# pityka/lamp

Measured on AMD Instinct MI355X. Metric: training-step samples/sec, higher is better.
Workload: dtype bf16; 1 GPU; example-cifar100 Cnn.resnet(100) training step (fwd+backprop+AdamW), synthetic CIFAR batch; per_gpu_batch=2048, global_batch=2048, parallelism=single, optimizer=AdamW lr 1e-3 wd 0 beta2 0.95 mixedPrecision

## Files before the change

### include/lamp_hip.h

```cpp
#ifndef LAMP_HIP_H
#define LAMP_HIP_H

#include <stddef.h>
#include <stdint.h>

#ifdef __cplusplus
extern "C" {
#endif

#define LAMP_MAX_DIMS 8

typedef struct lamp_tensor lamp_tensor;
typedef struct lamp_stream lamp_stream;
typedef struct lamp_comm lamp_comm;
typedef struct lamp_graph lamp_graph;

#define LAMP_U8 0
#define LAMP_I8 1
#define LAMP_I16 2
#define LAMP_I32 3
#define LAMP_I64 4
#define LAMP_F16 5
#define LAMP_F32 6
#define LAMP_F64 7
// ... 263 lines not shown
                      const lamp_tensor* inRowptr, const lamp_tensor* inPerm, const lamp_tensor* outRowptr, const lamp_tensor* outPerm);
int lamp_gat_long_row(int64_t* out);

int lamp_convolution(lamp_tensor** out, const lamp_tensor* x, const lamp_tensor* w, const lamp_tensor* bias_or_null,
                     const int64_t* stride, const int64_t* padding, const int64_t* dilation, int nspatial,
                     int transposed, const int64_t* output_padding, int64_t groups);
int lamp_convolution_backward(lamp_tensor* out3[3], const lamp_tensor* grad_out, const lamp_tensor* x,
                              const lamp_tensor* w, const int64_t* stride, const int64_t* padding,
                              const int64_t* dilation, int nspatial, int transposed,
                              const int64_t* output_padding, int64_t groups, const uint8_t mask[3]);
int lamp_convolution_backward_input_add(lamp_tensor** out, const lamp_tensor* grad_out, const lamp_tensor* x,
                                        const lamp_tensor* w, const int64_t* stride, const int64_t* padding,
                                        const int64_t* dilation, int nspatial, const int64_t* output_padding,
                                        int64_t groups, const lamp_tensor* addend);
int lamp_convolution_backward_input_pair(lamp_tensor** out, const lamp_tensor* x, const lamp_tensor* grad_out_a, const lamp_tensor* w_a,
                                         const int64_t* stride_a, const int64_t* padding_a, const int64_t* dilation_a,
                                         const lamp_tensor* grad_out_b, const lamp_tensor* w_b, const int64_t* stride_b,
                                         const int64_t* padding_b, const int64_t* dilation_b, int nspatial, int64_t groups,
                                         const lamp_tensor* addend_or_null);
int lamp_convolution_backward_weight_pair(lamp_tensor* out2[2], const lamp_tensor* x, const lamp_tensor* grad_out_a, const lamp_tensor* w_a,
                                          const int64_t* stride_a, const int64_t* padding_a, const int64_t* dilation_a,
                                          const lamp_tensor* grad_out_b, const lamp_tensor* w_b, const int64_t* stride_b,
                                          const int64_t* padding_b, const int64_t* dilation_b, int nspatial, int64_t groups);
int lamp_convolution_pair(lamp_tensor* out2[2], const lamp_tensor* x, const lamp_tensor* w_a, const lamp_tensor* bias_a_or_null,
                          const int64_t* stride_a, const int64_t* padding_a, const int64_t* dilation_a, const lamp_tensor* w_b,
                          const lamp_tensor* bias_b_or_null, const int64_t* stride_b, const int64_t* padding_b,
                          const int64_t* dilation_b, int nspatial, int64_t groups);
int lamp_convolution_chain_pair(lamp_tensor* out3[3], const lamp_tensor* x, const lamp_tensor* w, const lamp_tensor* bias_or_null,
                                const int64_t* stride, const int64_t* padding, const int64_t* dilation, const lamp_tensor* w_a,
                                const lamp_tensor* bias_a_or_null, const int64_t* stride_a, const int64_t* padding_a,
                                const int64_t* dilation_a, const lamp_tensor* w_b, const lamp_tensor* bias_b_or_null,
                                const int64_t* stride_b, const int64_t* padding_b, const int64_t* dilation_b, int nspatial,
                                int64_t groups);
int lamp_avg_pool2d(lamp_tensor** out, const lamp_tensor* x, int64_t kernel, int64_t stride, int64_t padding,
                    int ceil_mode, int count_include_pad);
int lamp_avg_pool2d_backward(lamp_tensor** out, const lamp_tensor* grad_out, const lamp_tensor* x, int64_t kernel,
                             int64_t stride, int64_t padding, int ceil_mode, int count_include_pad);
int lamp_max_pool2d_with_indices(lamp_tensor** out, lamp_tensor** indices, const lamp_tensor* x, int64_t kernel,
                                 int64_t stride, int64_t padding, int64_t dilation, int ceil_mode);
int lamp_max_pool2d_with_indices_backward(lamp_tensor** out, const lamp_tensor* grad_out, const lamp_tensor* x,
                                          int64_t kernel, int64_t stride, int64_t padding, int64_t dilation,
                                          int ceil_mode, const lamp_tensor* indices);
int lamp_max_pool1d_with_indices(lamp_tensor** out, lamp_tensor** indices, const lamp_tensor* x, int64_t kernel,
                                 int64_t stride, int64_t padding, int64_t dilation, int ceil_mode);
int lamp_max_pool1d_with_indices_backward(lamp_tensor** out, const lamp_tensor* grad_out, const lamp_tensor* x,
                                          int64_t kernel, int64_t stride, int64_t padding, int64_t dilation,
                                          int ceil_mode, const lamp_tensor* indices);

int lamp_native_batch_norm(lamp_tensor* out3[3] , const lamp_tensor* x,
                           const lamp_tensor* weight_or_null, const lamp_tensor* bias_or_null,
                           lamp_tensor* running_mean_or_null, lamp_tensor* running_var_or_null, int training,
                           double momentum, double eps);
int lamp_native_batch_norm_backward(lamp_tensor* out3[3] , const lamp_tensor* grad_out,
                                    const lamp_tensor* x, const lamp_tensor* weight_or_null,
                                    const lamp_tensor* running_mean_or_null, const lamp_tensor* running_var_or_null,
                                    const lamp_tensor* save_mean_or_null, const lamp_tensor* save_invstd_or_null,
                                    int training, double eps, const uint8_t mask[3]);
int lamp_native_batch_norm_relu(lamp_tensor* out3[3] , const lamp_tensor* x,
                                const lamp_tensor* weight_or_null, const lamp_tensor* bias_or_null,
                                lamp_tensor* running_mean_or_null, lamp_tensor* running_var_or_null, int training,
                                double momentum, double eps);
int lamp_native_batch_norm_relu_backward(lamp_tensor* out3[3] , const lamp_tensor* grad_out,
                                         const lamp_tensor* x, const lamp_tensor* weight_or_null, const lamp_tensor* bias_or_null,
                                         const lamp_tensor* running_mean_or_null, const lamp_tensor* running_var_or_null,
                                         const lamp_tensor* save_mean_or_null, const lamp_tensor* save_invstd_or_null,
                                         int training, double eps, const uint8_t mask[3]);
// ... 185 lines not shown
```

### jni/LampNative.java

```java
package aten;

public final class LampNative {
  static { System.loadLibrary("lampjni"); }
  private LampNative() {}
  public static native String lamp_last_error();
  public static native String lamp_version();
  public static native void lamp_tensor_release_all(long[] tensors);
  public static native byte[] lamp_comm_get_unique_id();
  public static native long lamp_comm_init_rank(int nranks, byte[] id, int rank);
  public static native long[] lamp_tensors_from_file(String path, long offset, long length, boolean pin, long[] types, long[] offsets, long[] lengths);
  public static native long[] lamp_tensor_trace_list();
  public static native long[] lamp_tensor_sizes(long t);
  public static native long[] lamp_tensor_strides(long t);
  public static native boolean copyFromDoubleArray(long t, double[] a);
  public static native boolean copyToDoubleArray(long t, double[] a);
  public static native boolean copyFromFloatArray(long t, float[] a);
  public static native boolean copyToFloatArray(long t, float[] a);
  public static native boolean copyFromLongArray(long t, long[] a);
  public static native boolean copyToLongArray(long t, long[] a);
  public static native boolean copyFromIntArray(long t, int[] a);
  public static native boolean copyToIntArray(long t, int[] a);
  public static native boolean copyFromShortArray(long t, short[] a);
  public static native boolean copyToShortArray(long t, short[] a);
  public static native boolean copyFromByteArray(long t, byte[] a);
// ... 196 lines not shown
  public static native long lamp_bmm(long a, long b);
  public static native void lamp_bmm_out(long out, long a, long b);
  public static native long lamp_matmul(long a, long b);
  public static native long lamp_addmm(long self, long a, long b, double beta, double alpha);
  public static native void lamp_addmm_out(long out, long self, long a, long b, double beta, double alpha);
  public static native long lamp_baddbmm(long self, long a, long b, double beta, double alpha);
  public static native void lamp_addmm_out_transposed1(long out, long self, long a, long b, double beta, double alpha);
  public static native void lamp_addmm_out_transposed2(long out, long self, long a, long b, double beta, double alpha);
  public static native void lamp_baddbmm_out_transposed1(long out, long self, long a, long b, double beta, double alpha);
  public static native void lamp_baddbmm_out_transposed2(long out, long self, long a, long b, double beta, double alpha);
  public static native long lamp_linear_bias(long x, long w, long bias_or_null);
  public static native void lamp_lstm_cell_forward(long gates, long c_prev, long h_out, long c_out);
  public static native void lamp_lstm_cell_backward(long dgates, long dc_prev, long gates, long c_prev, long c, long dout_or_null, long dh_or_null, long dc_or_null);
  public static native void lamp_gru_gates_forward(long gates, long h_prev, long rh_out);
  public static native void lamp_gru_output_forward(long gates, long h_prev, long h_out);
  public static native void lamp_gru_output_backward(long dgates, long dh_prev, long gates, long h_prev, long dout_or_null, long dh_or_null);
  public static native void lamp_gru_gates_backward(long dgates, long dh_prev, long gates, long h_prev, long drh);
  public static native void lamp_rnn_cell_forward(long gates, long h_out);
  public static native void lamp_rnn_cell_backward(long dgates, long h, long dout_or_null, long dh_or_null);
  public static native long[] lamp_gcn_adjacency(long edgeI, long edgeJ, long numNodes, int dtype);
  public static native long lamp_gcn_aggregate(long x, long rowptr, long col, long dinv);
  public static native long lamp_gcn_long_row();
  public static native long[] lamp_graph_edge_csr(long index, long numNodes);
  public static native long[] lamp_gat_forward(long score, long value, long edgeI, long inRowptr, long inPerm);
  public static native long[] lamp_gat_backward(long dout, long out, long lse, long score, long value, long edgeI, long edgeJ, long inRowptr, long inPerm, long outRowptr, long outPerm);
  public static native long lamp_gat_long_row();
  public static native long lamp_convolution(long x, long w, long bias_or_null, long[] stride, long[] padding, long[] dilation, int transposed, long[] output_padding, long groups);
  public static native long[] lamp_convolution_backward(long grad_out, long x, long w, long[] stride, long[] padding, long[] dilation, int transposed, long[] output_padding, long groups, boolean[] mask);
  public static native long lamp_convolution_backward_input_add(long grad_out, long x, long w, long[] stride, long[] padding, long[] dilation, long[] output_padding, long groups, long addend);
  public static native long lamp_convolution_backward_input_pair(long x, long grad_out_a, long w_a, long[] stride_a, long[] padding_a, long[] dilation_a, long grad_out_b, long w_b, long[] stride_b, long[] padding_b, long[] dilation_b, long groups, long addend_or_null);
  public static native long[] lamp_convolution_backward_weight_pair(long x, long grad_out_a, long w_a, long[] stride_a, long[] padding_a, long[] dilation_a, long grad_out_b, long w_b, long[] stride_b, long[] padding_b, long[] dilation_b, long groups);
  public static native long[] lamp_convolution_pair(long x, long w_a, long bias_a_or_null, long[] stride_a, long[] padding_a, long[] dilation_a, long w_b, long bias_b_or_null, long[] stride_b, long[] padding_b, long[] dilation_b, long groups);
  public static native long[] lamp_convolution_chain_pair(long x, long w, long bias_or_null, long[] stride, long[] padding, long[] dilation, long w_a, long bias_a_or_null, long[] stride_a, long[] padding_a, long[] dilation_a, long w_b, long bias_b_or_null, long[] stride_b, long[] padding_b, long[] dilation_b, long groups);
  public static native long lamp_avg_pool2d(long x, long kernel, long stride, long padding, int ceil_mode, int count_include_pad);
  public static native long lamp_avg_pool2d_backward(long grad_out, long x, long kernel, long stride, long padding, int ceil_mode, int count_include_pad);
  public static native long[] lamp_max_pool2d_with_indices(long x, long kernel, long stride, long padding, long dilation, int ceil_mode);
  public static native long lamp_max_pool2d_with_indices_backward(long grad_out, long x, long kernel, long stride, long padding, long dilation, int ceil_mode, long indices);
  public static native long[] lamp_max_pool1d_with_indices(long x, long kernel, long stride, long padding, long dilation, int ceil_mode);
  public static native long lamp_max_pool1d_with_indices_backward(long grad_out, long x, long kernel, long stride, long padding, long dilation, int ceil_mode, long indices);
  public static native long[] lamp_native_batch_norm(long x, long weight_or_null, long bias_or_null, long running_mean_or_null, long running_var_or_null, int training, double momentum, double eps);
  public static native long[] lamp_native_batch_norm_backward(long grad_out, long x, long weight_or_null, long running_mean_or_null, long running_var_or_null, long save_mean_or_null, long save_invstd_or_null, int training, double eps, boolean[] mask);
  public static native long[] lamp_native_batch_norm_relu(long x, long weight_or_null, long bias_or_null, long running_mean_or_null, long running_var_or_null, int training, double momentum, double eps);
  public static native long[] lamp_native_batch_norm_relu_backward(long grad_out, long x, long weight_or_null, long bias_or_null, long running_mean_or_null, long running_var_or_null, long save_mean_or_null, long save_invstd_or_null, int training, double eps, boolean[] mask);
  public static native long[] lamp_native_batch_norm_add_relu(long x, long addend, long weight_or_null, long bias_or_null, long running_mean_or_null, long running_var_or_null, int training, double momentum, double eps);
  public static native long[] lamp_native_batch_norm_add_relu_backward(long grad_out, long x, long addend, long weight_or_null, long bias_or_null, long running_mean_or_null, long running_var_or_null, long save_mean_or_null, long save_invstd_or_null, int training, double eps, boolean[] mask);
  public static native long[] lamp_native_batch_norm2_add_relu(long x, long weight, long bias, long running_mean, long running_var, long x2, long weight2, long bias2, long running_mean2, long running_var2, double momentum, double momentum2, double eps, double eps2);
  public static native long[] lamp_native_batch_norm2_add_relu_pool_log_softmax(long x, long weight, long bias, long running_mean, long running_var, long x2, long weight2, long bias2, long running_mean2, long running_var2, double momentum, double momentum2, double eps, double eps2);
  public static native long[] lamp_native_batch_norm2_add_relu_backward(long grad_out, long x, long weight, long bias, long save_mean, long save_invstd, long x2, long weight2, long bias2, long save_mean2, long save_invstd2, double eps, double eps2, boolean[] mask);
  public static native long[] lamp_batch_norm_affine(long x, long weight, long bias, long running_mean, long running_var, double momentum, double eps);
  public static native int lamp_convolution_bn_relu_input_folds(long x, long w, long[] stride, long[] padding, long[] dilation, long groups);
  public static native long lamp_convolution_bn_relu_input(long x, long affine, long w, long bias_or_null, long[] stride, long[] padding, long[] dilation, long groups);
  public static native long[] lamp_convolution_bn_relu_input_backward(long grad_out, long x, long affine, long w, long[] stride, long[] padding, long[] dilation, long groups, boolean[] mask);
  public static native long[] lamp_native_layer_norm(long x, long[] normalized_shape, long weight_or_null, long bias_or_null, double eps);
  public static native long[] lamp_native_layer_norm_backward(long grad_out, long x, long[] normalized_shape, long mean, long rstd, long weight_or_null, long bias_or_null, boolean[] mask);
  public static native long lamp_log_softmax(long x, long dim);
  public static native long lamp_log_softmax_backward_data(long grad_out, long output, long dim);
  public static native long lamp_global_avg_pool_log_softmax(long x);
  public static native long lamp_global_avg_pool_log_softmax_backward(long grad, long output, long x);
  public static native long lamp_global_avg_pool_log_softmax_nll_backward(long grad_loss, long target, long weight_or_null, long reduction, long ignore_index, long total_weight, long output, long x);
  public static native long lamp_softmax(long x, long dim);
  public static native long[] lamp_nll_loss_forward(long x, long target, long weight_or_null, long reduction, long ignore_index);
  public static native long[] lamp_nll_loss_forward_accumulate_(long x, long target, long weight_or_null, long reduction, long ignore_index, long acc, double scale);
  public static native long[] lamp_nll_loss_forward_pooled_gradient_(long x, long target, long weight_or_null, long reduction, long ignore_index, long acc_or_null, double scale, long plane_elems);
  public static native long lamp_nll_loss_backward(long grad_out, long x, long target, long weight_or_null, long reduction, long ignore_index, long total_weight);
  public static native long lamp_mse_loss(long x, long target, long reduction);
  public static native long lamp_mse_loss_backward(long grad_out, long x, long target, long reduction);
// ... 77 lines not shown
```

### jni/aten_jni.c

```c
#ifdef LAMP_JNI_SYNTAX_CHECK
#include "jni_syntax_check.h"
#else
#include <jni.h>
#endif
#include <stdint.h>
#include <stddef.h>
#include "lamp_hip.h"

#define H(x) ((void*)(intptr_t)(x))

#define LAMP_JNI_MAX_OUTS 4096

static void lamp_throw(JNIEnv* env) {
  jclass ex = (*env)->FindClass(env, "java/lang/RuntimeException");
  if (ex) (*env)->ThrowNew(env, ex, lamp_last_error());
}
static void lamp_throw_msg(JNIEnv* env, const char* msg) {
  jclass ex = (*env)->FindClass(env, "java/lang/RuntimeException");
  if (ex) (*env)->ThrowNew(env, ex, msg);
}

#define COPY_NATIVES(JT, JNAME, GET, REL)                                                                                              \
  JNIEXPORT jboolean JNICALL Java_aten_LampNative_copyFrom##JNAME##Array(JNIEnv* env, jclass cls, jlong t, JT##Array a) {              \
    (void)cls;                                                                                                                         \
// ... 1980 lines not shown
  (void)stride_a_n;
  jsize padding_a_n = (*env)->GetArrayLength(env, padding_a);
  jlong* padding_a_e = (*env)->GetLongArrayElements(env, padding_a, NULL);
  (void)padding_a_n;
  jsize dilation_a_n = (*env)->GetArrayLength(env, dilation_a);
  jlong* dilation_a_e = (*env)->GetLongArrayElements(env, dilation_a, NULL);
  (void)dilation_a_n;
  jsize stride_b_n = (*env)->GetArrayLength(env, stride_b);
  jlong* stride_b_e = (*env)->GetLongArrayElements(env, stride_b, NULL);
  (void)stride_b_n;
  jsize padding_b_n = (*env)->GetArrayLength(env, padding_b);
  jlong* padding_b_e = (*env)->GetLongArrayElements(env, padding_b, NULL);
  (void)padding_b_n;
  jsize dilation_b_n = (*env)->GetArrayLength(env, dilation_b);
  jlong* dilation_b_e = (*env)->GetLongArrayElements(env, dilation_b, NULL);
  void* out3_o[3] = {0};
  const int rc_ = lamp_convolution_chain_pair((void*)out3_o, H(x), H(w), H(bias_or_null), (const int64_t*)stride_e, (const int64_t*)padding_e, (const int64_t*)dilation_e, H(w_a), H(bias_a_or_null), (const int64_t*)stride_a_e, (const int64_t*)padding_a_e, (const int64_t*)dilation_a_e, H(w_b), H(bias_b_or_null), (const int64_t*)stride_b_e, (const int64_t*)padding_b_e, (const int64_t*)dilation_b_e, (int)dilation_b_n, (int64_t)groups);
  (*env)->ReleaseLongArrayElements(env, stride, stride_e, JNI_ABORT);
  (*env)->ReleaseLongArrayElements(env, padding, padding_e, JNI_ABORT);
  (*env)->ReleaseLongArrayElements(env, dilation, dilation_e, JNI_ABORT);
  (*env)->ReleaseLongArrayElements(env, stride_a, stride_a_e, JNI_ABORT);
  (*env)->ReleaseLongArrayElements(env, padding_a, padding_a_e, JNI_ABORT);
  (*env)->ReleaseLongArrayElements(env, dilation_a, dilation_a_e, JNI_ABORT);
  (*env)->ReleaseLongArrayElements(env, stride_b, stride_b_e, JNI_ABORT);
  (*env)->ReleaseLongArrayElements(env, padding_b, padding_b_e, JNI_ABORT);
  (*env)->ReleaseLongArrayElements(env, dilation_b, dilation_b_e, JNI_ABORT);
  if (rc_ != 0) { lamp_throw(env); return NULL; }
  jlong r_[3] = {(jlong)(intptr_t)out3_o[0], (jlong)(intptr_t)out3_o[1], (jlong)(intptr_t)out3_o[2]};
  jlongArray a_ = (*env)->NewLongArray(env, 3);
  if (a_) (*env)->SetLongArrayRegion(env, a_, 0, 3, r_);
  return a_;
}

JNIEXPORT jlong JNICALL Java_aten_LampNative_lamp_1avg_1pool2d(JNIEnv* env, jclass cls, jlong x, jlong kernel, jlong stride, jlong padding, jint ceil_mode, jint count_include_pad) {
  (void)cls;
  void* out_o = NULL;
  const int rc_ = lamp_avg_pool2d((void*)&out_o, H(x), (int64_t)kernel, (int64_t)stride, (int64_t)padding, (int)ceil_mode, (int)count_include_pad);
  if (rc_ != 0) { lamp_throw(env); return 0; }
  return (jlong)(intptr_t)out_o;
}

JNIEXPORT jlong JNICALL Java_aten_LampNative_lamp_1avg_1pool2d_1backward(JNIEnv* env, jclass cls, jlong grad_out, jlong x, jlong kernel, jlong stride, jlong padding, jint ceil_mode, jint count_include_pad) {
  (void)cls;
  void* out_o = NULL;
  const int rc_ = lamp_avg_pool2d_backward((void*)&out_o, H(grad_out), H(x), (int64_t)kernel, (int64_t)stride, (int64_t)padding, (int)ceil_mode, (int)count_include_pad);
  if (rc_ != 0) { lamp_throw(env); return 0; }
  return (jlong)(intptr_t)out_o;
}

JNIEXPORT jlongArray JNICALL Java_aten_LampNative_lamp_1max_1pool2d_1with_1indices(JNIEnv* env, jclass cls, jlong x, jlong kernel, jlong stride, jlong padding, jlong dilation, jint ceil_mode) {
  (void)cls;
  void* out_o = NULL;
  void* indices_o = NULL;
  const int rc_ = lamp_max_pool2d_with_indices((void*)&out_o, (void*)&indices_o, H(x), (int64_t)kernel, (int64_t)stride, (int64_t)padding, (int64_t)dilation, (int)ceil_mode);
  if (rc_ != 0) { lamp_throw(env); return NULL; }
  jlong r_[2] = {(jlong)(intptr_t)out_o, (jlong)(intptr_t)indices_o};
  jlongArray a_ = (*env)->NewLongArray(env, 2);
  if (a_) (*env)->SetLongArrayRegion(env, a_, 0, 2, r_);
  return a_;
}

JNIEXPORT jlong JNICALL Java_aten_LampNative_lamp_1max_1pool2d_1with_1indices_1backward(JNIEnv* env, jclass cls, jlong grad_out, jlong x, jlong kernel, jlong stride, jlong padding, jlong dilation, jint ceil_mode, jlong indices) {
  (void)cls;
  void* out_o = NULL;
  const int rc_ = lamp_max_pool2d_with_indices_backward((void*)&out_o, H(grad_out), H(x), (int64_t)kernel, (int64_t)stride, (int64_t)padding, (int64_t)dilation, (int)ceil_mode, H(indices));
  if (rc_ != 0) { lamp_throw(env); return 0; }
// ... 1078 lines not shown
```

### lamp_amd/csrc/core/host_staging.cpp

```cpp
#include "host_staging.h"

namespace S = lamp::staging;

extern "C" {

int lamp_abs__dev(lamp_tensor** out, const lamp_tensor* a);
int lamp_abs(lamp_tensor** out, const lamp_tensor* a) { return S::call(lamp_abs__dev, S::Out{out}, S::In{a}); }
int lamp_abs___dev(lamp_tensor* a);
int lamp_abs_(lamp_tensor* a) { return S::call(lamp_abs___dev, S::InOut{a}); }
int lamp_acos__dev(lamp_tensor** out, const lamp_tensor* a);
int lamp_acos(lamp_tensor** out, const lamp_tensor* a) { return S::call(lamp_acos__dev, S::Out{out}, S::In{a}); }
int lamp_acos___dev(lamp_tensor* a);
int lamp_acos_(lamp_tensor* a) { return S::call(lamp_acos___dev, S::InOut{a}); }
int lamp_adamw_step___dev(lamp_tensor* const* params, lamp_tensor* const* grads, lamp_tensor* const* m, lamp_tensor* const* v, lamp_tensor* const* master_or_null, int n, const double* lr, const double* weight_decay, const double* beta1, const double* beta2, double eps, double schedule_factor, int64_t step_count, int debias);
int lamp_adamw_step_(lamp_tensor* const* params, lamp_tensor* const* grads, lamp_tensor* const* m, lamp_tensor* const* v, lamp_tensor* const* master_or_null, int n, const double* lr, const double* weight_decay, const double* beta1, const double* beta2, double eps, double schedule_factor, int64_t step_count, int debias) { return S::call(lamp_adamw_step___dev, S::Arr{params, n, false}, S::Arr{grads, n, true}, S::Arr{m, n, false}, S::Arr{v, n, false}, S::Arr{master_or_null, n, false}, n, lr, weight_decay, beta1, beta2, eps, schedule_factor, step_count, debias); }
int lamp_add__dev(lamp_tensor** out, const lamp_tensor* a, const lamp_tensor* b, double alpha);
int lamp_add(lamp_tensor** out, const lamp_tensor* a, const lamp_tensor* b, double alpha) { return S::call(lamp_add__dev, S::Out{out}, S::In{a}, S::In{b}, alpha); }
int lamp_add___dev(lamp_tensor* self, const lamp_tensor* b, double alpha);
int lamp_add_(lamp_tensor* self, const lamp_tensor* b, double alpha) { return S::call(lamp_add___dev, S::InOut{self}, S::In{b}, alpha); }
int lamp_add_out__dev(lamp_tensor* out, const lamp_tensor* a, const lamp_tensor* b, double alpha);
int lamp_add_out(lamp_tensor* out, const lamp_tensor* a, const lamp_tensor* b, double alpha) { return S::call(lamp_add_out__dev, S::InOut{out}, S::In{a}, S::In{b}, alpha); }
int lamp_add_scalar__dev(lamp_tensor** out, const lamp_tensor* a, double b, double alpha);
int lamp_add_scalar(lamp_tensor** out, const lamp_tensor* a, double b, double alpha) { return S::call(lamp_add_scalar__dev, S::Out{out}, S::In{a}, b, alpha); }
int lamp_add_scalar___dev(lamp_tensor* self, double b, double alpha);
// ... 26 lines not shown
int lamp_atan2(lamp_tensor** out, const lamp_tensor* a, const lamp_tensor* b) { return S::call(lamp_atan2__dev, S::Out{out}, S::In{a}, S::In{b}); }
int lamp_atan___dev(lamp_tensor* a);
int lamp_atan_(lamp_tensor* a) { return S::call(lamp_atan___dev, S::InOut{a}); }
int lamp_avg_pool2d__dev(lamp_tensor** out, const lamp_tensor* x, int64_t kernel, int64_t stride, int64_t padding, int ceil_mode, int count_include_pad);
int lamp_avg_pool2d(lamp_tensor** out, const lamp_tensor* x, int64_t kernel, int64_t stride, int64_t padding, int ceil_mode, int count_include_pad) { return S::call(lamp_avg_pool2d__dev, S::Out{out}, S::In{x}, kernel, stride, padding, ceil_mode, count_include_pad); }
int lamp_avg_pool2d_backward__dev(lamp_tensor** out, const lamp_tensor* grad_out, const lamp_tensor* x, int64_t kernel, int64_t stride, int64_t padding, int ceil_mode, int count_include_pad);
int lamp_avg_pool2d_backward(lamp_tensor** out, const lamp_tensor* grad_out, const lamp_tensor* x, int64_t kernel, int64_t stride, int64_t padding, int ceil_mode, int count_include_pad) { return S::call(lamp_avg_pool2d_backward__dev, S::Out{out}, S::In{grad_out}, S::In{x}, kernel, stride, padding, ceil_mode, count_include_pad); }
int lamp_baddbmm__dev(lamp_tensor** out, const lamp_tensor* self, const lamp_tensor* a, const lamp_tensor* b, double beta, double alpha);
int lamp_baddbmm(lamp_tensor** out, const lamp_tensor* self, const lamp_tensor* a, const lamp_tensor* b, double beta, double alpha) { return S::call(lamp_baddbmm__dev, S::Out{out}, S::In{self}, S::In{a}, S::In{b}, beta, alpha); }
int lamp_baddbmm_out_transposed1__dev(lamp_tensor* out, const lamp_tensor* self, const lamp_tensor* a, const lamp_tensor* b, double beta, double alpha);
int lamp_baddbmm_out_transposed1(lamp_tensor* out, const lamp_tensor* self, const lamp_tensor* a, const lamp_tensor* b, double beta, double alpha) { return S::call(lamp_baddbmm_out_transposed1__dev, S::InOut{out}, S::In{self}, S::In{a}, S::In{b}, beta, alpha); }
int lamp_baddbmm_out_transposed2__dev(lamp_tensor* out, const lamp_tensor* self, const lamp_tensor* a, const lamp_tensor* b, double beta, double alpha);
int lamp_baddbmm_out_transposed2(lamp_tensor* out, const lamp_tensor* self, const lamp_tensor* a, const lamp_tensor* b, double beta, double alpha) { return S::call(lamp_baddbmm_out_transposed2__dev, S::InOut{out}, S::In{self}, S::In{a}, S::In{b}, beta, alpha); }
int lamp_batch_norm_affine__dev(lamp_tensor* out3[3], const lamp_tensor* x, const lamp_tensor* weight, const lamp_tensor* bias, lamp_tensor* running_mean, lamp_tensor* running_var, double momentum, double eps);
int lamp_batch_norm_affine(lamp_tensor* out3[3], const lamp_tensor* x, const lamp_tensor* weight, const lamp_tensor* bias, lamp_tensor* running_mean, lamp_tensor* running_var, double momentum, double eps) { return S::call(lamp_batch_norm_affine__dev, S::OutK<3>{out3}, S::In{x}, S::In{weight}, S::In{bias}, S::InOut{running_mean}, S::InOut{running_var}, momentum, eps); }
int lamp_binary_cross_entropy_with_logits__dev(lamp_tensor** out, const lamp_tensor* x, const lamp_tensor* target, const lamp_tensor* pos_weight_or_null, int64_t reduction);
int lamp_binary_cross_entropy_with_logits(lamp_tensor** out, const lamp_tensor* x, const lamp_tensor* target, const lamp_tensor* pos_weight_or_null, int64_t reduction) { return S::call(lamp_binary_cross_entropy_with_logits__dev, S::Out{out}, S::In{x}, S::In{target}, S::In{pos_weight_or_null}, reduction); }
int lamp_bincount__dev(lamp_tensor** out, const lamp_tensor* a, const lamp_tensor* weights_or_null, int64_t minlength);
int lamp_bincount(lamp_tensor** out, const lamp_tensor* a, const lamp_tensor* weights_or_null, int64_t minlength) { return S::call(lamp_bincount__dev, S::Out{out}, S::In{a}, S::In{weights_or_null}, minlength); }
int lamp_bmm__dev(lamp_tensor** out, const lamp_tensor* a, const lamp_tensor* b);
int lamp_bmm(lamp_tensor** out, const lamp_tensor* a, const lamp_tensor* b) { return S::call(lamp_bmm__dev, S::Out{out}, S::In{a}, S::In{b}); }
int lamp_bmm_out__dev(lamp_tensor* out, const lamp_tensor* a, const lamp_tensor* b);
int lamp_bmm_out(lamp_tensor* out, const lamp_tensor* a, const lamp_tensor* b) { return S::call(lamp_bmm_out__dev, S::InOut{out}, S::In{a}, S::In{b}); }
int lamp_cartesian_prod__dev(lamp_tensor** out, lamp_tensor* const* tensors, int n);
int lamp_cartesian_prod(lamp_tensor** out, lamp_tensor* const* tensors, int n) { return S::call(lamp_cartesian_prod__dev, S::Out{out}, S::Arr{tensors, n, false}, n); }
int lamp_ceil__dev(lamp_tensor** out, const lamp_tensor* a);
int lamp_ceil(lamp_tensor** out, const lamp_tensor* a) { return S::call(lamp_ceil__dev, S::Out{out}, S::In{a}); }
int lamp_ceil___dev(lamp_tensor* a);
int lamp_ceil_(lamp_tensor* a) { return S::call(lamp_ceil___dev, S::InOut{a}); }
int lamp_convolution__dev(lamp_tensor** out, const lamp_tensor* x, const lamp_tensor* w, const lamp_tensor* bias_or_null, const int64_t* stride, const int64_t* padding, const int64_t* dilation, int nspatial, int transposed, const int64_t* output_padding, int64_t groups);
int lamp_convolution(lamp_tensor** out, const lamp_tensor* x, const lamp_tensor* w, const lamp_tensor* bias_or_null, const int64_t* stride, const int64_t* padding, const int64_t* dilation, int nspatial, int transposed, const int64_t* output_padding, int64_t groups) { return S::call(lamp_convolution__dev, S::Out{out}, S::In{x}, S::In{w}, S::In{bias_or_null}, stride, padding, dilation, nspatial, transposed, output_padding, groups); }
int lamp_convolution_backward__dev(lamp_tensor* out3[3], const lamp_tensor* grad_out, const lamp_tensor* x, const lamp_tensor* w, const int64_t* stride, const int64_t* padding, const int64_t* dilation, int nspatial, int transposed, const int64_t* output_padding, int64_t groups, const uint8_t mask[3]);
int lamp_convolution_backward(lamp_tensor* out3[3], const lamp_tensor* grad_out, const lamp_tensor* x, const lamp_tensor* w, const int64_t* stride, const int64_t* padding, const int64_t* dilation, int nspatial, int transposed, const int64_t* output_padding, int64_t groups, const uint8_t mask[3]) { return S::call(lamp_convolution_backward__dev, S::OutK<3>{out3}, S::In{grad_out}, S::In{x}, S::In{w}, stride, padding, dilation, nspatial, transposed, output_padding, groups, mask); }
int lamp_convolution_backward_input_add__dev(lamp_tensor** out, const lamp_tensor* grad_out, const lamp_tensor* x, const lamp_tensor* w, const int64_t* stride, const int64_t* padding, const int64_t* dilation, int nspatial, const int64_t* output_padding, int64_t groups, const lamp_tensor* addend);
int lamp_convolution_backward_input_add(lamp_tensor** out, const lamp_tensor* grad_out, const lamp_tensor* x, const lamp_tensor* w, const int64_t* stride, const int64_t* padding, const int64_t* dilation, int nspatial, const int64_t* output_padding, int64_t groups, const lamp_tensor* addend) { return S::call(lamp_convolution_backward_input_add__dev, S::Out{out}, S::In{grad_out}, S::In{x}, S::In{w}, stride, padding, dilation, nspatial, output_padding, groups, S::In{addend}); }
int lamp_convolution_backward_input_pair__dev(lamp_tensor** out, const lamp_tensor* x, const lamp_tensor* grad_out_a, const lamp_tensor* w_a, const int64_t* stride_a, const int64_t* padding_a, const int64_t* dilation_a, const lamp_tensor* grad_out_b, const lamp_tensor* w_b, const int64_t* stride_b, const int64_t* padding_b, const int64_t* dilation_b, int nspatial, int64_t groups, const lamp_tensor* addend_or_null);
int lamp_convolution_backward_input_pair(lamp_tensor** out, const lamp_tensor* x, const lamp_tensor* grad_out_a, const lamp_tensor* w_a, const int64_t* stride_a, const int64_t* padding_a, const int64_t* dilation_a, const lamp_tensor* grad_out_b, const lamp_tensor* w_b, const int64_t* stride_b, const int64_t* padding_b, const int64_t* dilation_b, int nspatial, int64_t groups, const lamp_tensor* addend_or_null) { return S::call(lamp_convolution_backward_input_pair__dev, S::Out{out}, S::In{x}, S::In{grad_out_a}, S::In{w_a}, stride_a, padding_a, dilation_a, S::In{grad_out_b}, S::In{w_b}, stride_b, padding_b, dilation_b, nspatial, groups, S::In{addend_or_null}); }
int lamp_convolution_backward_weight_pair__dev(lamp_tensor* out2[2], const lamp_tensor* x, const lamp_tensor* grad_out_a, const lamp_tensor* w_a, const int64_t* stride_a, const int64_t* padding_a, const int64_t* dilation_a, const lamp_tensor* grad_out_b, const lamp_tensor* w_b, const int64_t* stride_b, const int64_t* padding_b, const int64_t* dilation_b, int nspatial, int64_t groups);
int lamp_convolution_backward_weight_pair(lamp_tensor* out2[2], const lamp_tensor* x, const lamp_tensor* grad_out_a, const lamp_tensor* w_a, const int64_t* stride_a, const int64_t* padding_a, const int64_t* dilation_a, const lamp_tensor* grad_out_b, const lamp_tensor* w_b, const int64_t* stride_b, const int64_t* padding_b, const int64_t* dilation_b, int nspatial, int64_t groups) { return S::call(lamp_convolution_backward_weight_pair__dev, S::OutK<2>{out2}, S::In{x}, S::In{grad_out_a}, S::In{w_a}, stride_a, padding_a, dilation_a, S::In{grad_out_b}, S::In{w_b}, stride_b, padding_b, dilation_b, nspatial, groups); }
int lamp_convolution_bn_relu_input__dev(lamp_tensor** out, const lamp_tensor* x, const lamp_tensor* affine, const lamp_tensor* w, const lamp_tensor* bias_or_null, const int64_t* stride, const int64_t* padding, const int64_t* dilation, int nspatial, int64_t groups);
int lamp_convolution_bn_relu_input(lamp_tensor** out, const lamp_tensor* x, const lamp_tensor* affine, const lamp_tensor* w, const lamp_tensor* bias_or_null, const int64_t* stride, const int64_t* padding, const int64_t* dilation, int nspatial, int64_t groups) { return S::call(lamp_convolution_bn_relu_input__dev, S::Out{out}, S::In{x}, S::In{affine}, S::In{w}, S::In{bias_or_null}, stride, padding, dilation, nspatial, groups); }
int lamp_convolution_bn_relu_input_backward__dev(lamp_tensor* out3[3], const lamp_tensor* grad_out, const lamp_tensor* x, const lamp_tensor* affine, const lamp_tensor* w, const int64_t* stride, const int64_t* padding, const int64_t* dilation, int nspatial, int64_t groups, const uint8_t mask[3]);
int lamp_convolution_bn_relu_input_backward(lamp_tensor* out3[3], const lamp_tensor* grad_out, const lamp_tensor* x, const lamp_tensor* affine, const lamp_tensor* w, const int64_t* stride, const int64_t* padding, const int64_t* dilation, int nspatial, int64_t groups, const uint8_t mask[3]) { return S::call(lamp_convolution_bn_relu_input_backward__dev, S::OutK<3>{out3}, S::In{grad_out}, S::In{x}, S::In{affine}, S::In{w}, stride, padding, dilation, nspatial, groups, mask); }
int lamp_convolution_bn_relu_input_folds__dev(int* out, const lamp_tensor* x, const lamp_tensor* w, const int64_t* stride, const int64_t* padding, const int64_t* dilation, int nspatial, int64_t groups);
int lamp_convolution_bn_relu_input_folds(int* out, const lamp_tensor* x, const lamp_tensor* w, const int64_t* stride, const int64_t* padding, const int64_t* dilation, int nspatial, int64_t groups) { return S::call(lamp_convolution_bn_relu_input_folds__dev, out, S::In{x}, S::In{w}, stride, padding, dilation, nspatial, groups); }
int lamp_convolution_chain_pair__dev(lamp_tensor* out3[3], const lamp_tensor* x, const lamp_tensor* w, const lamp_tensor* bias_or_null, const int64_t* stride, const int64_t* padding, const int64_t* dilation, const lamp_tensor* w_a, const lamp_tensor* bias_a_or_null, const int64_t* stride_a, const int64_t* padding_a, const int64_t* dilation_a, const lamp_tensor* w_b, const lamp_tensor* bias_b_or_null, const int64_t* stride_b, const int64_t* padding_b, const int64_t* dilation_b, int nspatial, int64_t groups);
int lamp_convolution_chain_pair(lamp_tensor* out3[3], const lamp_tensor* x, const lamp_tensor* w, const lamp_tensor* bias_or_null, const int64_t* stride, const int64_t* padding, const int64_t* dilation, const lamp_tensor* w_a, const lamp_tensor* bias_a_or_null, const int64_t* stride_a, const int64_t* padding_a, const int64_t* dilation_a, const lamp_tensor* w_b, const lamp_tensor* bias_b_or_null, const int64_t* stride_b, const int64_t* padding_b, const int64_t* dilation_b, int nspatial, int64_t groups) { return S::call(lamp_convolution_chain_pair__dev, S::OutK<3>{out3}, S::In{x}, S::In{w}, S::In{bias_or_null}, stride, padding, dilation, S::In{w_a}, S::In{bias_a_or_null}, stride_a, padding_a, dilation_a, S::In{w_b}, S::In{bias_b_or_null}, stride_b, padding_b, dilation_b, nspatial, groups); }
int lamp_convolution_pair__dev(lamp_tensor* out2[2], const lamp_tensor* x, const lamp_tensor* w_a, const lamp_tensor* bias_a_or_null, const int64_t* stride_a, const int64_t* padding_a, const int64_t* dilation_a, const lamp_tensor* w_b, const lamp_tensor* bias_b_or_null, const int64_t* stride_b, const int64_t* padding_b, const int64_t* dilation_b, int nspatial, int64_t groups);
int lamp_convolution_pair(lamp_tensor* out2[2], const lamp_tensor* x, const lamp_tensor* w_a, const lamp_tensor* bias_a_or_null, const int64_t* stride_a, const int64_t* padding_a, const int64_t* dilation_a, const lamp_tensor* w_b, const lamp_tensor* bias_b_or_null, const int64_t* stride_b, const int64_t* padding_b, const int64_t* dilation_b, int nspatial, int64_t groups) { return S::call(lamp_convolution_pair__dev, S::OutK<2>{out2}, S::In{x}, S::In{w_a}, S::In{bias_a_or_null}, stride_a, padding_a, dilation_a, S::In{w_b}, S::In{bias_b_or_null}, stride_b, padding_b, dilation_b, nspatial, groups); }
int lamp_cos__dev(lamp_tensor** out, const lamp_tensor* a);
int lamp_cos(lamp_tensor** out, const lamp_tensor* a) { return S::call(lamp_cos__dev, S::Out{out}, S::In{a}); }
int lamp_cos___dev(lamp_tensor* a);
int lamp_cos_(lamp_tensor* a) { return S::call(lamp_cos___dev, S::InOut{a}); }
int lamp_count_ne__dev(lamp_tensor** out, const lamp_tensor* a, const lamp_tensor* b);
int lamp_count_ne(lamp_tensor** out, const lamp_tensor* a, const lamp_tensor* b) { return S::call(lamp_count_ne__dev, S::Out{out}, S::In{a}, S::In{b}); }
int lamp_cross__dev(lamp_tensor** out, const lamp_tensor* a, const lamp_tensor* b, int64_t dim);
int lamp_cross(lamp_tensor** out, const lamp_tensor* a, const lamp_tensor* b, int64_t dim) { return S::call(lamp_cross__dev, S::Out{out}, S::In{a}, S::In{b}, dim); }
int lamp_diag__dev(lamp_tensor** out, const lamp_tensor* a, int64_t diagonal);
int lamp_diag(lamp_tensor** out, const lamp_tensor* a, int64_t diagonal) { return S::call(lamp_diag__dev, S::Out{out}, S::In{a}, diagonal); }
int lamp_diagonal__dev(lamp_tensor** out, const lamp_tensor* a, int64_t offset, int64_t dim1, int64_t dim2);
int lamp_diagonal(lamp_tensor** out, const lamp_tensor* a, int64_t offset, int64_t dim1, int64_t dim2) { return S::call(lamp_diagonal__dev, S::Out{out}, S::In{a}, offset, dim1, dim2); }
int lamp_div__dev(lamp_tensor** out, const lamp_tensor* a, const lamp_tensor* b);
int lamp_div(lamp_tensor** out, const lamp_tensor* a, const lamp_tensor* b) { return S::call(lamp_div__dev, S::Out{out}, S::In{a}, S::In{b}); }
int lamp_div___dev(lamp_tensor* self, const lamp_tensor* b);
int lamp_div_(lamp_tensor* self, const lamp_tensor* b) { return S::call(lamp_div___dev, S::InOut{self}, S::In{b}); }
int lamp_div_out__dev(lamp_tensor* out, const lamp_tensor* a, const lamp_tensor* b);
// ... 379 lines not shown
```

### lamp_amd/csrc/core/switches.h

```cpp
#pragma once
#include <cstdint>

namespace lamp {

constexpr int64_t SW_NO_CLAMP = INT64_MIN;

#define LAMP_SWITCHES_ONCE(X)                                                                                                             \
                                                        \
  X(conv_sibling, "LAMP_CONV_SIBLING", BOOL, 1, 0, "a residual block's 3x3 and its sibling 1x1 of the same input as one forward launch") \
  X(conv_chain, "LAMP_CONV_CHAIN", BOOL, 1, 0, "a convolution directly in front of a residual block and the block's 3x3 + 1x1 as one forward call (0: two)") \
  X(fuse_bn_pair, "LAMP_FUSE_BN_PAIR", BOOL, 1, 0, "relu(bn(right) + bn(left)) at a block's end as one op (0: the chain)")                \
  X(fuse_pool_logsoftmax, "LAMP_FUSE_POOL_LOGSOFTMAX", BOOL, 1, 0, "average pool -> flatten -> log-softmax tail as one node")             \
  X(fuse_block_tail, "LAMP_FUSE_BLOCK_TAIL", BOOL, 1, 0, "the last residual block and the pooled log-softmax tail as one node")          \
  X(fuse_bn_conv, "LAMP_FUSE_BN_CONV", BOOL, 1, 0, "batch norm -> relu -> convolution: the convolution applies the norm while staging")  \
  X(fuse_loss_accumulate, "LAMP_FUSE_LOSS_ACCUMULATE", BOOL, 1, 0, "acc += n * loss inside the NLL loss kernel")                          \
  X(fuse_loss_backward, "LAMP_FUSE_LOSS_BACKWARD", BOOL, 1, 0, "the NLL loss backward goes straight to the pooled log-softmax node's input in one launch")                      \
  X(fuse_loss_tail, "LAMP_FUSE_LOSS_TAIL", BOOL, 1, 0, "the loss launch also writes the pooled log-softmax's input gradient per plane")  \
  X(conv_dgrad_accumulate, "LAMP_CONV_DGRAD_ACCUMULATE", BOOL, 1, 0, "a convolution's input gradient adds into the existing one in its epilogue") \
  X(conv_dgrad_pair, "LAMP_CONV_DGRAD_PAIR", BOOL, 1, 0, "input gradients of a block's 3x3 and sibling 1x1 from one launch")             \
  X(conv_wgrad_pair, "LAMP_CONV_WGRAD_PAIR", BOOL, 1, 0, "weight gradients of a block's 3x3 and sibling 1x1 from one launch")            \
  X(linear_bias_fused, "LAMP_LINEAR_BIAS_FUSED", BOOL, 1, 0, "a linear layer's bias in the GEMM epilogue (0: mm then add)")               \
  X(mult_add_fused, "LAMP_MULT_ADD_FUSED", BOOL, 1, 0, "x * scale + residual in one pass (0: mult then add)")                             \
  X(attention_as_written_for_cuda, "LAMP_ATTENTION_AS_WRITTEN_FOR_CUDA", BOOL, 0, 0, "multi-head attention as the reference's op chain instead of the fused kernels") \
  X(recurrent_fused, "LAMP_RECURRENT_FUSED", BOOL, 1, 0, "RNN / GRU / LSTM as one node per sequence with fused cell kernels (0: the fold over time steps)") \
  X(fuse_qkv, "LAMP_FUSE_QKV", BOOL, 1, 0, "self-attention's three projections as one product (0: three)")                                \
  X(host_stream_side, "LAMP_HOST_STREAM_SIDE", BOOL, 0, 0, "batch streams gather on a side stream instead of the consumer's")             \
                                                                           \
  X(pinned_cache_mb, "LAMP_PINNED_CACHE_MB", INT, 2048, 0, "upper bound of the cache of freed pinned host buffers, MiB")                  \
  X(pinned_gather_wgs, "LAMP_PINNED_GATHER_WGS", INT, 48, 1, "workgroups of a gather that reads pinned host memory")                      \
                                                                                                    \
  X(flash_attention, "LAMP_FLASH_ATTENTION", BOOL, 1, 0, "the flash attention kernels, forward and backward")                             \
  X(small_attention, "LAMP_SMALL_ATTENTION", BOOL, 1, 0, "the short-sequence attention kernels")                                          \
  X(knn_fused, "LAMP_KNN_FUSED", BOOL, 1, 0, "the fused distance + top-k nearest-neighbour kernel")                                       \
  X(knn_split, "LAMP_KNN_SPLIT", INT, -1, SW_NO_CLAMP, "f16-plane k-NN filter: 0 off, 1 where it pays, 2 forced; negative: the mode set through the API") \
  X(knn_split_planes, "LAMP_KNN_SPLIT_PLANES", INT, 0, SW_NO_CLAMP, "f16 planes per coordinate of that filter: 3, anything else 2")      \
  X(umap_pairs2, "LAMP_UMAP_PAIRS2", BOOL, 1, 0, "the UMAP loss's two-dimensional pair kernel")                                            \
                                                                                                             \
  X(gemm_shape_tags, "LAMP_GEMM_SHAPE_TAGS", BOOL, 0, 0, "profiling aid: one kernel-timer class per GEMM shape and layout")               \
  X(gemm_splitk, "LAMP_GEMM_SPLITK", BOOL, 1, 0, "split-K for products with few output tiles (bf16 and f32 / f64)")                       \
  X(gemm_tail_split, "LAMP_GEMM_TAIL_SPLIT", BOOL, 1, 0, "an almost empty last round of 256 x 256 tiles becomes a second, split-K product") \
  X(gemm_fp_split_wgs, "LAMP_GEMM_FP_SPLIT_WGS", INT, 512, 1, "workgroups an f32 / f64 split-K product aims at")                          \
                                                                                              \
  X(bn_fused_bwd, "LAMP_BN_FUSED_BWD", BOOL, 1, 0, "one-pass batch-norm backward (workgroups exchange their sums) where no mode is set through the API") \
// ... 45 lines not shown
```

### lamp_amd/csrc/host/autograd.h

```cpp
#pragma once
#include <cmath>
#include <functional>
#include <memory>
#include <string>
#include <vector>

#include "../core/tensor.h"

namespace lamp {
namespace host {

struct Box {
  lamp_tensor* h;
  explicit Box(lamp_tensor* h_) : h(h_) {}
  ~Box() { if (h) lamp_tensor_release(h); }
  Box(const Box&) = delete;
  Box& operator=(const Box&) = delete;
};
struct Ten {
  std::shared_ptr<Box> b;
  Ten() = default;
  explicit Ten(lamp_tensor* h) : b(h ? std::make_shared<Box>(h) : nullptr) {}
  lamp_tensor* h() const { return b ? b->h : nullptr; }
  bool defined() const { return b && b->h; }
// ... 64 lines not shown
inline Ten view(const Ten& a, const std::vector<int64_t>& s) { lamp_tensor* o = nullptr; HCALL(lamp_view(&o, a.h(), s.data(), (int)s.size())); return Ten(o); }
inline Ten reshape(const Ten& a, const std::vector<int64_t>& s) { lamp_tensor* o = nullptr; HCALL(lamp_reshape(&o, a.h(), s.data(), (int)s.size())); return Ten(o); }
inline Ten flatten(const Ten& a, int64_t s, int64_t e) { lamp_tensor* o = nullptr; HCALL(lamp_flatten(&o, a.h(), s, e)); return Ten(o); }
inline Ten transpose(const Ten& a, int64_t d0, int64_t d1) { lamp_tensor* o = nullptr; HCALL(lamp_transpose(&o, a.h(), d0, d1)); return Ten(o); }
inline Ten slice(const Ten& a, int64_t d, int64_t s, int64_t e, int64_t st) { lamp_tensor* o = nullptr; HCALL(lamp_slice(&o, a.h(), d, s, e, st)); return Ten(o); }
inline Ten select(const Ten& a, int64_t d, int64_t i) { lamp_tensor* o = nullptr; HCALL(lamp_select(&o, a.h(), d, i)); return Ten(o); }
inline Ten unbroadcast(const Ten& p, const std::vector<int64_t>& s) { lamp_tensor* o = nullptr; HCALL(lamp_unbroadcast(&o, p.h(), s.data(), (int)s.size())); return Ten(o); }
inline Ten sum_dims(const Ten& a, const std::vector<int64_t>& d, bool keep) { lamp_tensor* o = nullptr; HCALL(lamp_sum_dims(&o, a.h(), d.data(), (int)d.size(), keep)); return Ten(o); }
inline Ten mean_dims(const Ten& a, const std::vector<int64_t>& d, bool keep) { lamp_tensor* o = nullptr; HCALL(lamp_mean_dims(&o, a.h(), d.data(), (int)d.size(), keep)); return Ten(o); }
inline Ten norm2_dims(const Ten& a, const std::vector<int64_t>& d, bool keep) { lamp_tensor* o = nullptr; HCALL(lamp_norm2_dims(&o, a.h(), d.data(), (int)d.size(), keep)); return Ten(o); }
inline Ten zeros(const std::vector<int64_t>& s, int dtype, int device) { lamp_tensor* o = nullptr; HCALL(lamp_zeros(&o, s.data(), (int)s.size(), dtype, device)); return Ten(o); }
inline Ten ones(const std::vector<int64_t>& s, int dtype, int device) { lamp_tensor* o = nullptr; HCALL(lamp_ones(&o, s.data(), (int)s.size(), dtype, device)); return Ten(o); }
inline Ten scalar(double v, int dtype, int device) { lamp_tensor* o = nullptr; HCALL(lamp_scalar_tensor(&o, v, dtype, device)); return Ten(o); }
inline Ten normal(double mean, double std, const std::vector<int64_t>& s, int dtype, int device) { lamp_tensor* o = nullptr; HCALL(lamp_normal(&o, mean, std, s.data(), (int)s.size(), dtype, device)); return Ten(o); }
inline Ten cast(const Ten& a, int dtype) { lamp_tensor* o = nullptr; HCALL(lamp_cast(&o, a.h(), dtype)); return Ten(o); }
inline Ten index_select(const Ten& a, int64_t d, const Ten& idx) { lamp_tensor* o = nullptr; HCALL(lamp_index_select(&o, a.h(), d, idx.h())); return Ten(o); }
inline Ten index_add(const Ten& a, int64_t d, const Ten& idx, const Ten& src) { lamp_tensor* o = nullptr; HCALL(lamp_index_add(&o, a.h(), d, idx.h(), src.h())); return Ten(o); }
inline Ten where(const Ten& c, const Ten& a, const Ten& b) { lamp_tensor* o = nullptr; HCALL(lamp_where(&o, c.h(), a.h(), b.h())); return Ten(o); }
inline Ten lt_scalar(const Ten& a, double s) { lamp_tensor* o = nullptr; HCALL(lamp_lt_scalar(&o, a.h(), s)); return Ten(o); }
inline Ten le_scalar(const Ten& a, double s) { lamp_tensor* o = nullptr; HCALL(lamp_le_scalar(&o, a.h(), s)); return Ten(o); }
inline Ten cat(const std::vector<Ten>& ts, int64_t dim) {
  std::vector<lamp_tensor*> hs;
  for (auto& t : ts) hs.push_back(t.h());
  lamp_tensor* o = nullptr;
  HCALL(lamp_cat(&o, hs.data(), (int)hs.size(), dim));
  return Ten(o);
}
}

struct Variable;
using Var = std::shared_ptr<Variable>;
using Backward = std::function<void(const Ten& p, Variable& out)>;

struct Op {
  virtual ~Op() = default;
  std::vector<std::pair<Var, Backward>> params;
  const char* name = "op";
  std::function<void()> reset;
  std::function<void(const Ten& plane_grad)> pooled_input_grad;
};

struct Variable {
  std::shared_ptr<Op> op;
  Ten value;
  bool wants_grad = false;
  Ten grad;
  bool grad_shared = false;
  std::vector<std::function<void()>> pending;
  bool needsGrad() const { return wants_grad; }
  std::vector<int64_t> shape() const { return value.shape(); }
  void zeroGrad() { grad = Ten(); grad_shared = false; }
  Ten grad_tensor() {
    if (!wants_grad) return Ten();
    if (!grad.defined()) { grad = ops::zeros_like(value); grad_shared = false; }
    return grad;
  }
  Ten grad_inplace() {
    if (!grad.defined()) { grad = ops::zeros_like(value); grad_shared = false; }
    else if (grad_shared) { grad = ops::clone(grad); grad_shared = false; }
    return grad;
  }
  void accumulate(const Ten& t, bool fresh) {
    if (!grad.defined()) { grad = t; grad_shared = !fresh; return; }
    if (grad_shared) { grad = ops::add(grad, t); grad_shared = false; return; }
    ops::add_(grad, t);
  }
  void accumulate_scaled(const Ten& t, double alpha) {
    if (!grad.defined()) { grad = ops::mul_scalar(t, alpha); grad_shared = false; return; }
    if (grad_shared) { grad = ops::add(grad, t, alpha); grad_shared = false; return; }
    ops::add_(grad, t, alpha);
  }
  void subtract(const Ten& t) { accumulate_scaled(t, -1.0); }
// ... 26 lines not shown
```

### lamp_amd/csrc/host/ops.cpp

```cpp
#include "ops.h"
#include "../core/switches.h"
#include <cstring>
#include <map>
#include <tuple>

#include <unordered_set>

namespace lamp {
namespace host {

Var make_const(const Ten& t) {
  auto v = std::make_shared<Variable>();
  v->value = t;
  return v;
}
Var make_param(const Ten& t) {
  auto v = std::make_shared<Variable>();
  v->value = t;
  v->wants_grad = true;
  return v;
}
Var make_result(const std::shared_ptr<Op>& op, const Ten& value) {
  auto v = std::make_shared<Variable>();
  v->op = op;
// ... 628 lines not shown
        lamp_tensor* r3[3] = {nullptr, nullptr, nullptr};
        HCALL(lamp_scaled_dot_product_attention_bias_backward(r3, p.h(), qv.h(), kv.h(), vv.h(), out.h(), lse.h(), attentionBias.defined() ? attentionBias.h() : nullptr,
                                                              isCausal, 0.0));
        for (int i = 0; i < 3; i++) cache->g[i] = Ten(r3[i]);
        cache->p = p;
      }
      acc.accumulate(cache->g[which], true);
      cache->g[which] = Ten();
      if (!cache->g[0].defined() && !cache->g[1].defined() && !cache->g[2].defined()) cache->p = Ten();
    };
  };
  op->params.push_back({query, back(0)});
  op->params.push_back({key, back(1)});
  op->params.push_back({value, back(2)});
  return make_result(op, out);
}

struct ConvPairGrad {
  struct Side { Ten w; std::vector<int64_t> stride, padding, dilation; Ten p; Ten pw; Variable* wout = nullptr; };
  Side side[2];
  int64_t groups = 1;
  int waiting = -1;
  int wwaiting = -1;
};
static Var convolution_node(const Var& input, const Var& weight, const Var& bias, const std::vector<int64_t>& stride,
                            const std::vector<int64_t>& padding, const std::vector<int64_t>& dilation, bool transposed,
                            const std::vector<int64_t>& outputPadding, int64_t groups, const Ten* computed,
                            const std::shared_ptr<ConvPairGrad>& pair = nullptr, int pair_side = 0) {
  auto op = new_op("Convolution");
  const int ns = (int)stride.size();
  Ten iv = input->value, wv = weight->value;
  const bool fuse_accumulate = sw().conv_dgrad_accumulate;
  const bool fuse_pair = sw().conv_dgrad_pair;
  auto back = [=](int which) {
    std::function<void(const Ten&, Variable&)> single;
    single = [=](const Ten& p, Variable& out) {
      if (which == 0 && !transposed && fuse_accumulate && out.has_grad() && out.grad.h()->is_device() && p.h()->is_device() && out.grad.dtype() == p.dtype()) {
        lamp_tensor* r = nullptr;
        HCALL(lamp_convolution_backward_input_add(&r, p.h(), iv.h(), wv.h(), stride.data(), padding.data(), dilation.data(), ns,
                                                  outputPadding.data(), groups, out.grad.h()));
        out.grad = Ten(r);
        out.grad_shared = false;
        return;
      }
      lamp_tensor* o3[3] = {nullptr, nullptr, nullptr};
      uint8_t mask[3] = {(uint8_t)(which == 0), (uint8_t)(which == 1), (uint8_t)(which == 2)};
      HCALL(lamp_convolution_backward(o3, p.h(), iv.h(), wv.h(), stride.data(), padding.data(), dilation.data(), ns, transposed,
                                      outputPadding.data(), groups, mask));
      out.accumulate(Ten(o3[which]), true);
    };
    const bool fuse_wpair = sw().conv_wgrad_pair;
    if (which == 1 && pair && fuse_wpair && !transposed) {
      Variable* inp = input.get();
      return Backward([=](const Ten& p, Variable& out) {
        if (!p.h()->is_device() || tls_backprop_hooked || out.op) { single(p, out); return; }
        ConvPairGrad& st = *pair;
        if (st.wwaiting < 0) {
          st.wwaiting = pair_side;
          st.side[pair_side].pw = p;
          st.side[pair_side].wout = &out;
          inp->pending.push_back([=] {
            ConvPairGrad& s2 = *pair;
            if (s2.wwaiting != pair_side) return;
            const Ten held = s2.side[pair_side].pw;
            Variable* wo = s2.side[pair_side].wout;
            s2.side[pair_side].pw = Ten(); s2.side[pair_side].wout = nullptr; s2.wwaiting = -1;
// ... 8 lines not shown
        st.side[other].pw = Ten(); st.side[other].wout = nullptr; st.wwaiting = -1;
        const Ten& pa = pair_side == 0 ? p : po;
        const Ten& pb = pair_side == 0 ? po : p;
        lamp_tensor* o2[2] = {nullptr, nullptr};
        HCALL(lamp_convolution_backward_weight_pair(o2, iv.h(), pa.h(), st.side[0].w.h(), st.side[0].stride.data(), st.side[0].padding.data(),
                                                    st.side[0].dilation.data(), pb.h(), st.side[1].w.h(), st.side[1].stride.data(),
                                                    st.side[1].padding.data(), st.side[1].dilation.data(), ns, st.groups));
        const Ten da(o2[0]), db(o2[1]);
        (pair_side == 0 ? out : *wo).accumulate(da, true);
        (pair_side == 0 ? *wo : out).accumulate(db, true);
      });
    }
    if (which != 0 || !pair || !fuse_pair || transposed) return Backward(single);
    return Backward([=](const Ten& p, Variable& out) {
      if (!(p.h()->is_device() && fuse_accumulate)) { single(p, out); return; }
      ConvPairGrad& st = *pair;
      if (st.waiting < 0) {
        st.waiting = pair_side;
        st.side[pair_side].p = p;
        Variable* outp = &out;
        out.pending.push_back([=] {
          ConvPairGrad& s2 = *pair;
          if (s2.waiting != pair_side) return;
          const Ten held = s2.side[pair_side].p;
          s2.side[pair_side].p = Ten(); s2.waiting = -1;
          single(held, *outp);
        });
        return;
      }
      if (st.waiting == pair_side) { single(p, out); return; }
      const int other = st.waiting;
      const Ten po = st.side[other].p;
      st.side[other].p = Ten(); st.waiting = -1;
      const Ten& pa = pair_side == 0 ? p : po;
      const Ten& pb = pair_side == 0 ? po : p;
      const bool have = out.has_grad() && out.grad.h()->is_device() && out.grad.dtype() == p.dtype();
      if (out.has_grad() && !have) { single(po, out); single(p, out); return; }
      lamp_tensor* r = nullptr;
      HCALL(lamp_convolution_backward_input_pair(&r, iv.h(), pa.h(), st.side[0].w.h(), st.side[0].stride.data(), st.side[0].padding.data(),
                                                 st.side[0].dilation.data(), pb.h(), st.side[1].w.h(), st.side[1].stride.data(),
                                                 st.side[1].padding.data(), st.side[1].dilation.data(), ns, st.groups, have ? out.grad.h() : nullptr));
      out.grad = Ten(r);
      out.grad_shared = false;
    });
  };
  op->params.push_back({input, back(0)});
  op->params.push_back({weight, back(1)});
  op->params.push_back({bias, back(2)});
  if (pair) op->reset = [pair] {
    pair->waiting = pair->wwaiting = -1;
    for (auto& sd : pair->side) { sd.p = Ten(); sd.pw = Ten(); sd.wout = nullptr; }
  };
  if (computed) return make_result(op, *computed);
  lamp_tensor* o = nullptr;
  HCALL(lamp_convolution(&o, iv.h(), wv.h(), bias->value.h(), stride.data(), padding.data(), dilation.data(), ns, transposed,
                         outputPadding.data(), groups));
  return make_result(op, Ten(o));
}
Var convolution(const Var& input, const Var& weight, const Var& bias, const std::vector<int64_t>& stride,
                const std::vector<int64_t>& padding, const std::vector<int64_t>& dilation, bool transposed,
                const std::vector<int64_t>& outputPadding, int64_t groups) {
  return convolution_node(input, weight, bias, stride, padding, dilation, transposed, outputPadding, groups, nullptr);
}
static std::pair<Var, Var> convolution_pair_nodes(const Var& input, const Var& weight_a, const Var& bias_a, const std::vector<int64_t>& stride_a,
                                                  const std::vector<int64_t>& padding_a, const std::vector<int64_t>& dilation_a, const Var& weight_b,
                                                  const Var& bias_b, const std::vector<int64_t>& stride_b, const std::vector<int64_t>& padding_b,
                                                  const std::vector<int64_t>& dilation_b, int64_t groups, const Ten& ya, const Ten& yb);
std::pair<Var, Var> convolution_pair(const Var& input, const Var& weight_a, const Var& bias_a, const std::vector<int64_t>& stride_a,
                                     const std::vector<int64_t>& padding_a, const std::vector<int64_t>& dilation_a, const Var& weight_b,
                                     const Var& bias_b, const std::vector<int64_t>& stride_b, const std::vector<int64_t>& padding_b,
                                     const std::vector<int64_t>& dilation_b, int64_t groups) {
  const int ns = (int)stride_a.size();
  LAMP_CHECK(ns == (int)stride_b.size(), "convolution_pair: the two convolutions have different numbers of spatial dimensions");
  lamp_tensor* o2[2] = {nullptr, nullptr};
  HCALL(lamp_convolution_pair(o2, input->value.h(), weight_a->value.h(), bias_a->value.h(), stride_a.data(), padding_a.data(), dilation_a.data(),
                              weight_b->value.h(), bias_b->value.h(), stride_b.data(), padding_b.data(), dilation_b.data(), ns, groups));
  return convolution_pair_nodes(input, weight_a, bias_a, stride_a, padding_a, dilation_a, weight_b, bias_b, stride_b, padding_b, dilation_b, groups, Ten(o2[0]),
                                Ten(o2[1]));
}
static std::pair<Var, Var> convolution_pair_nodes(const Var& input, const Var& weight_a, const Var& bias_a, const std::vector<int64_t>& stride_a,
                                                  const std::vector<int64_t>& padding_a, const std::vector<int64_t>& dilation_a, const Var& weight_b,
// ... 418 lines not shown
```

### lamp_amd/csrc/kernels/abi_dev_names.h

```cpp
#pragma once
#define lamp_abs lamp_abs__dev
#define lamp_abs_ lamp_abs___dev
#define lamp_acos lamp_acos__dev
#define lamp_acos_ lamp_acos___dev
#define lamp_adamw_step_ lamp_adamw_step___dev
#define lamp_add lamp_add__dev
#define lamp_add_ lamp_add___dev
#define lamp_add_out lamp_add_out__dev
#define lamp_add_scalar lamp_add_scalar__dev
#define lamp_add_scalar_ lamp_add_scalar___dev
#define lamp_add_scaled_mixed_ lamp_add_scaled_mixed___dev
#define lamp_addcdiv_out lamp_addcdiv_out__dev
#define lamp_addcmul_out lamp_addcmul_out__dev
#define lamp_addmm lamp_addmm__dev
#define lamp_addmm_out lamp_addmm_out__dev
#define lamp_addmm_out_transposed1 lamp_addmm_out_transposed1__dev
#define lamp_addmm_out_transposed2 lamp_addmm_out_transposed2__dev
#define lamp_argmax lamp_argmax__dev
#define lamp_argsort lamp_argsort__dev
#define lamp_asin lamp_asin__dev
#define lamp_asin_ lamp_asin___dev
#define lamp_atan lamp_atan__dev
#define lamp_atan2 lamp_atan2__dev
#define lamp_atan_ lamp_atan___dev
#define lamp_avg_pool2d lamp_avg_pool2d__dev
#define lamp_avg_pool2d_backward lamp_avg_pool2d_backward__dev
#define lamp_baddbmm lamp_baddbmm__dev
#define lamp_baddbmm_out_transposed1 lamp_baddbmm_out_transposed1__dev
#define lamp_baddbmm_out_transposed2 lamp_baddbmm_out_transposed2__dev
#define lamp_batch_norm_affine lamp_batch_norm_affine__dev
#define lamp_binary_cross_entropy_with_logits lamp_binary_cross_entropy_with_logits__dev
#define lamp_bincount lamp_bincount__dev
#define lamp_bmm lamp_bmm__dev
#define lamp_bmm_out lamp_bmm_out__dev
#define lamp_cartesian_prod lamp_cartesian_prod__dev
#define lamp_ceil lamp_ceil__dev
#define lamp_ceil_ lamp_ceil___dev
#define lamp_convolution lamp_convolution__dev
#define lamp_convolution_backward lamp_convolution_backward__dev
#define lamp_convolution_backward_input_add lamp_convolution_backward_input_add__dev
#define lamp_convolution_backward_input_pair lamp_convolution_backward_input_pair__dev
#define lamp_convolution_backward_weight_pair lamp_convolution_backward_weight_pair__dev
#define lamp_convolution_bn_relu_input lamp_convolution_bn_relu_input__dev
#define lamp_convolution_bn_relu_input_backward lamp_convolution_bn_relu_input_backward__dev
#define lamp_convolution_bn_relu_input_folds lamp_convolution_bn_relu_input_folds__dev
#define lamp_convolution_chain_pair lamp_convolution_chain_pair__dev
#define lamp_convolution_pair lamp_convolution_pair__dev
#define lamp_cos lamp_cos__dev
#define lamp_cos_ lamp_cos___dev
#define lamp_count_ne lamp_count_ne__dev
#define lamp_cross lamp_cross__dev
#define lamp_diag lamp_diag__dev
#define lamp_diagonal lamp_diagonal__dev
#define lamp_div lamp_div__dev
#define lamp_div_ lamp_div___dev
#define lamp_div_out lamp_div_out__dev
#define lamp_div_scalar lamp_div_scalar__dev
#define lamp_dropout_ lamp_dropout___dev
#define lamp_embedding lamp_embedding__dev
#define lamp_embedding_backward lamp_embedding_backward__dev
#define lamp_eq lamp_eq__dev
#define lamp_eq_scalar lamp_eq_scalar__dev
#define lamp_exp lamp_exp__dev
#define lamp_exp_ lamp_exp___dev
#define lamp_expm1 lamp_expm1__dev
#define lamp_flatten_into_ lamp_flatten_into___dev
#define lamp_floor lamp_floor__dev
#define lamp_floor_ lamp_floor___dev
#define lamp_gat_backward lamp_gat_backward__dev
#define lamp_gat_forward lamp_gat_forward__dev
#define lamp_gather lamp_gather__dev
#define lamp_gcn_adjacency lamp_gcn_adjacency__dev
// ... 173 lines not shown
```

### lamp_amd/csrc/kernels/conv.hip

```cpp
#include "device_utils.h"
#include "../core/strided.h"
#include "../core/switches.h"
#include "conv_geom.h"
#include "conv_backends.h"

namespace lamp {

template <class T>
__global__ __launch_bounds__(256) void conv_fwd_direct_kernel(const T* __restrict__ x, const T* __restrict__ w, const T* __restrict__ bias,
                                                              T* __restrict__ y, ConvGeom g) {
  using A = acc_t<T>;
  const int64_t total = g.N * g.Cout * g.Ho * g.Wo;
  const int cin_g = (int)(g.Cin / g.groups), cout_g = (int)(g.Cout / g.groups);
  for (int64_t e = blockIdx.x * (int64_t)blockDim.x + threadIdx.x; e < total; e += (int64_t)gridDim.x * blockDim.x) {
    const int wo = (int)(e % g.Wo);
    const int ho = (int)((e / g.Wo) % g.Ho);
    const int co = (int)((e / (g.Wo * g.Ho)) % g.Cout);
    const int64_t n = e / (g.Wo * g.Ho * g.Cout);
    const int grp = co / cout_g;
    A acc = bias ? load_as<A>(bias[co]) : A(0);
    const T* wp = w + (int64_t)co * cin_g * g.kh * g.kw;
    for (int cl = 0; cl < cin_g; cl++) {
      const T* xp = x + ((n * g.Cin + grp * cin_g + cl) * g.H) * g.W;
      for (int r = 0; r < g.kh; r++) {
// ... 547 lines not shown
    LAMP_CHECK(gy->ndim == x->ndim && gy->sizes[0] == g.N && gy->sizes[1] == g.Cout && gy->sizes[gy->ndim - 1] == g.Wo && (nspatial == 1 || gy->sizes[2] == g.Ho),
               "convolution_backward_input_pair: the " << which << " grad_out " << gy->describe() << " does not match its forward output shape");
  };
  check_grad(grad_out_a, ga, "first"); check_grad(grad_out_b, gb, "second");
  if (x->dtype == kBF16 && nspatial == 2) {
    Hold wa(contiguous_filter(w_a)), wb(contiguous_filter(w_b)), gya(contiguous(grad_out_a)), gyb(contiguous(grad_out_b)), ac(addend ? contiguous(addend) : nullptr);
    hipStream_t st = current_stream(x->device());
    Hold dx(new_tensor(std::vector<int64_t>(x->sizes, x->sizes + x->ndim), x->dtype, x->device()));
    bool fused = false;
    if (narrow_conv_dgrad_pair(gya.get(), wa.get(), ga, gyb.get(), wb.get(), gb, dx.get(), st, ac.get(), &fused) ||
        igemm_conv_dgrad_pair(gya.get(), wa.get(), ga, gyb.get(), wb.get(), gb, dx.get(), st, ac.get(), &fused)) {
      if (ac.get() && !fused) {
        lamp_tensor* sum = nullptr;
        if (lamp_add(&sum, ac.get(), dx.get(), 1.0) != 0) throw Error(lamp_last_error());
        *out = sum;
      } else *out = dx.take();
      return 0;
    }
  }
  const uint8_t m3[3] = {1, 0, 0};
  lamp_tensor* part = nullptr;
  if (addend) {
    if (lamp_convolution_backward_input_add(&part, grad_out_b, x, w_b, stride_b, padding_b, dilation_b, nspatial, zero2, groups, addend) != 0) throw Error(lamp_last_error());
  } else {
    lamp_tensor* r3[3] = {nullptr, nullptr, nullptr};
    if (lamp_convolution_backward(r3, grad_out_b, x, w_b, stride_b, padding_b, dilation_b, nspatial, 0, zero2, groups, m3) != 0) throw Error(lamp_last_error());
    part = r3[0];
  }
  Hold ph(part);
  if (lamp_convolution_backward_input_add(out, grad_out_a, x, w_a, stride_a, padding_a, dilation_a, nspatial, zero2, groups, ph.get()) != 0) throw Error(lamp_last_error());
  LAMP_API_END
}

int lamp_convolution_backward_weight_pair(lamp_tensor* out2[2], const lamp_tensor* x, const lamp_tensor* grad_out_a, const lamp_tensor* w_a,
                                          const int64_t* stride_a, const int64_t* padding_a, const int64_t* dilation_a,
                                          const lamp_tensor* grad_out_b, const lamp_tensor* w_b, const int64_t* stride_b,
                                          const int64_t* padding_b, const int64_t* dilation_b, int nspatial, int64_t groups) {
  LAMP_API_BEGIN
  check_device_tensor(x, "input"); check_device_tensor(w_a, "first weight"); check_device_tensor(grad_out_a, "first grad_out");
  check_device_tensor(w_b, "second weight"); check_device_tensor(grad_out_b, "second grad_out");
  LAMP_CHECK(x->dtype == w_a->dtype && x->dtype == w_b->dtype && grad_out_a->dtype == x->dtype && grad_out_b->dtype == x->dtype,
             "convolution_backward_weight_pair: dtype mismatch");
  LAMP_CHECK(nspatial >= 1 && nspatial <= 2, "convolution_backward_weight_pair: 1 or 2 spatial dimensions");
  const int64_t zero2[2] = {0, 0};
  ConvGeom ga = make_geom(x, w_a, stride_a, padding_a, dilation_a, nspatial, 0, zero2, groups);
  ConvGeom gb = make_geom(x, w_b, stride_b, padding_b, dilation_b, nspatial, 0, zero2, groups);
  auto check_grad = [&](const lamp_tensor* gy, const ConvGeom& g, const char* which) {
    LAMP_CHECK(gy->ndim == x->ndim && gy->sizes[0] == g.N && gy->sizes[1] == g.Cout && gy->sizes[gy->ndim - 1] == g.Wo && (nspatial == 1 || gy->sizes[2] == g.Ho),
               "convolution_backward_weight_pair: the " << which << " grad_out " << gy->describe() << " does not match its forward output shape");
  };
  check_grad(grad_out_a, ga, "first"); check_grad(grad_out_b, gb, "second");
  if (x->dtype == kBF16 && nspatial == 2) {
    Hold xc(contiguous(x)), wa(contiguous_filter(w_a)), wb(contiguous_filter(w_b)), gya(contiguous(grad_out_a)), gyb(contiguous(grad_out_b));
    hipStream_t st = current_stream(x->device());
    Hold dwa(new_like(wa.get())), dwb(new_like(wb.get()));
    if (narrow_conv_wgrad_pair(gya.get(), gyb.get(), xc.get(), dwa.get(), dwb.get(), ga, gb, st) ||
        igemm_conv_wgrad_pair(gya.get(), gyb.get(), xc.get(), dwa.get(), dwb.get(), ga, gb, st)) {
      out2[0] = dwa.take(); out2[1] = dwb.take();
      return 0;
    }
  }
  const uint8_t m3[3] = {0, 1, 0};
  lamp_tensor* ra[3] = {nullptr, nullptr, nullptr};
  if (lamp_convolution_backward(ra, grad_out_a, x, w_a, stride_a, padding_a, dilation_a, nspatial, 0, zero2, groups, m3) != 0) throw Error(lamp_last_error());
  Hold ha(ra[1]);
  lamp_tensor* rb[3] = {nullptr, nullptr, nullptr};
// ... 7 lines not shown
```

### lamp_amd/csrc/kernels/conv_backends.h

```cpp
#pragma once
#include "../core/tensor.h"
#include "conv_geom.h"

namespace lamp {
struct NcvPackMany;

bool igemm_conv_fwd(const Tensor* x, const Tensor* w, const Tensor* bias, Tensor* y, const ConvGeom& g, hipStream_t st);
bool igemm_conv_fwd_pair(const Tensor* x, const Tensor* w, const Tensor* bias, Tensor* y, const ConvGeom& g, const Tensor* w1, const Tensor* bias1,
                         Tensor* y1, const ConvGeom& g1, hipStream_t st);
bool igemm_conv_dgrad(const Tensor* dy, const Tensor* w, Tensor* dx, const ConvGeom& g, hipStream_t st, const Tensor* addend = nullptr,
                      bool* addend_fused = nullptr);
bool igemm_conv_dgrad_pair(const Tensor* dy, const Tensor* w, const ConvGeom& g, const Tensor* dy1, const Tensor* w1, const ConvGeom& g1, Tensor* dx,
                           hipStream_t st, const Tensor* addend, bool* addend_fused);
bool igemm_conv_wgrad(const Tensor* dy, const Tensor* x, Tensor* dw, const ConvGeom& g, hipStream_t st, const Tensor* affine = nullptr);
bool igemm_conv_wgrad_pair(const Tensor* dy, const Tensor* dy1, const Tensor* x, Tensor* dw, Tensor* dw1, const ConvGeom& g, const ConvGeom& g1, hipStream_t st);
bool igemm_conv_folds_affine(const ConvGeom& g, int dtype);
bool igemm_conv_fwd_affine(const Tensor* x, const Tensor* affine, const Tensor* w, const Tensor* bias, Tensor* y, const ConvGeom& g, hipStream_t st);

bool igemm32_conv_fwd(const Tensor* x, const Tensor* w, const Tensor* bias, Tensor* y, const ConvGeom& g, hipStream_t st);
bool igemm32_conv_dgrad(const Tensor* dy, const Tensor* w, Tensor* dx, const ConvGeom& g, hipStream_t st, const Tensor* addend = nullptr,
                        bool* addend_fused = nullptr);
bool igemm32_conv_wgrad(const Tensor* dy, const Tensor* x, Tensor* dw, const ConvGeom& g, hipStream_t st);

bool narrow_conv_fwd(const Tensor* x, const Tensor* w, const Tensor* bias, Tensor* y, const ConvGeom& g, hipStream_t st);
bool narrow_conv_fwd_pair(const Tensor* x, const Tensor* w, const Tensor* bias, Tensor* y, const ConvGeom& g, const Tensor* w1, const Tensor* bias1,
                          Tensor* y1, const ConvGeom& g1, hipStream_t st);
bool narrow_conv_chain_pair(const Tensor* x, const Tensor* w0, const Tensor* bias0, Tensor* s, const ConvGeom& g0, const Tensor* w, const Tensor* bias,
                            Tensor* y, const ConvGeom& g, const Tensor* w1, const Tensor* bias1, Tensor* y1, const ConvGeom& g1, hipStream_t st);
bool narrow_conv_dgrad(const Tensor* dy, const Tensor* w, Tensor* dx, const ConvGeom& g, hipStream_t st, const Tensor* addend = nullptr,
                       bool* addend_fused = nullptr);
bool narrow_conv_dgrad_pair(const Tensor* dy, const Tensor* w, const ConvGeom& g, const Tensor* dy1, const Tensor* w1, const ConvGeom& g1, Tensor* dx,
                            hipStream_t st, const Tensor* addend, bool* addend_fused);
bool narrow_conv_wgrad(const Tensor* dy, const Tensor* x, Tensor* dw, const ConvGeom& g, hipStream_t st);
bool narrow_conv_wgrad_pair(const Tensor* dy, const Tensor* dy1, const Tensor* x, Tensor* dw, Tensor* dw1, const ConvGeom& g, const ConvGeom& g1, hipStream_t st);

bool small_conv_fwd(const Tensor* x, const Tensor* w, const Tensor* bias, Tensor* y, const ConvGeom& g, hipStream_t st);
bool small_conv_dgrad(const Tensor* dy, const Tensor* w, Tensor* dx, const ConvGeom& g, hipStream_t st, const Tensor* addend = nullptr,
                      bool* addend_fused = nullptr);
bool small_conv_wgrad(const Tensor* dy, const Tensor* x, Tensor* dw, const ConvGeom& g, hipStream_t st);

void conv_repack_cached(lamp_tensor* const* params, int n, hipStream_t st);
void igemm_repack_cached(lamp_tensor* const* params, int n, hipStream_t st);
void igemm32_repack_cached(lamp_tensor* const* params, int n, hipStream_t st);
void small_repack_cached(lamp_tensor* const* params, int n, hipStream_t st);
void narrow_repack_cached(lamp_tensor* const* params, int n, hipStream_t st, NcvPackMany* fill, int* fill_cnt);
void narrow_pack_launch(const NcvPackMany& a, int cnt, hipStream_t st);

}
```

### lamp_amd/csrc/kernels/conv_narrow.hip

```cpp
#include "device_utils.h"
#include "conv_geom.h"
#include "conv_backends.h"
#include "../core/pack_cache.h"
#include "wgrad_reduce.h"
#include <type_traits>
#include <vector>
#include "conv_narrow_pack.h"
#include "../core/switches.h"

namespace lamp {

typedef nv_s8 __attribute__((aligned(2))) nv_s8_u;
typedef float nv_f4 __attribute__((ext_vector_type(4)));

struct NcvGeom {
  int N, C, CO;
  int H, W;
  int Hs, Ws;
  int top, left, dil;
  int Ho, Wo;
  int sh, sw, wx;
  int kh;
  int kh_inv;
  int pf;
// ... 159 lines not shown
      }
    }
    koff[ks] = (c * q.Hs + r) * q.Ws * 2;
  });
}
struct NcvStatAcc { nv_f4 st1, st2; int tiles; };
__device__ __forceinline__ void ncv_stats_take(NcvStatAcc& s, unsigned a, unsigned b, unsigned c, unsigned d) {
  typedef unsigned int nv_u4 __attribute__((ext_vector_type(4)));
  const unsigned ones2 = 0x3f803f80u;
  const nv_bf8 ones = __builtin_bit_cast(nv_bf8, nv_u4{ones2, ones2, ones2, ones2});
  const nv_bf8 y = __builtin_bit_cast(nv_bf8, nv_u4{a, b, c, d});
  s.st1 = __builtin_amdgcn_mfma_f32_16x16x32_bf16(ones, y, s.st1, 0, 0, 0);
  s.st2 = __builtin_amdgcn_mfma_f32_16x16x32_bf16(y, y, s.st2, 0, 0, 0);
}
template <int VPT>
__device__ __forceinline__ void ncv_stats_leave(NcvStatAcc& s, float (*sst)[16][3], int lane, int wid) {
  const int j = lane & 15, r = j & 3;
  const float sq = r == 0 ? s.st2[0] : r == 1 ? s.st2[1] : r == 2 ? s.st2[2] : s.st2[3];
  if ((lane >> 4) == (j >> 2)) { sst[wid][j][0] = (float)(s.tiles * VPT); sst[wid][j][1] = s.st1[0]; sst[wid][j][2] = sq; }
  s.st1 = nv_f4{0.f, 0.f, 0.f, 0.f}; s.st2 = nv_f4{0.f, 0.f, 0.f, 0.f}; s.tiles = 0;
}
template <int NS>
__device__ __forceinline__ void ncv_stats_flush(float (*sst)[16][3], int lane, int wid, int nwaves, int CO, int co_a, float* __restrict__ stats,
                                                float* __restrict__ stats2, int part, int nparts) {
  if (wid == 0 && lane < (NS == 2 ? 8 : 16) && lane < CO) {
    float cnt = 0.f, sy = 0.f, sq = 0.f;
    for (int h = 0; h < NS; h++)
      for (int k = 0; k < nwaves; k++) { cnt += sst[k][lane + 8 * h][0]; sy += sst[k][lane + 8 * h][1]; sq += sst[k][lane + 8 * h][2]; }
    const float mean = sy / cnt;
    float* o = lane < co_a ? stats + ((int64_t)lane * nparts + part) * 3 : stats2 + ((int64_t)(lane - co_a) * nparts + part) * 3;
    o[0] = cnt; o[1] = mean; o[2] = fmaxf(sq - sy * mean, 0.f);
  }
}
template <int NK, int SW, int PH0, int NS, bool ADD, bool STATS, bool PAR, bool MIRROR>
__device__ __forceinline__ void ncv_super_tiles(const char* smem, const NcvGeom& q, const nv_bf8 (&wfr)[NK], const int (&koff)[NK], int a_off, float bv, int co,
                                                bf16_t* yc, const bf16_t* ap, NcvStatAcc& sa, unsigned short* mc, int mws, int lane, int wid, int nwaves) {
  constexpr int P = 8 / SW;
  constexpr int ND = P / NS;
  constexpr int NSEG = (PH0 + (ND - 1) * NS * SW + 7) < 16 ? 2 : 3;
  static_assert(!MIRROR || (P == 8 && !PAR), "the LDS copy takes whole 16-byte packets of plain tiles");
  const int ncg = q.Wo / P, TR = 16 / ncg;
  const int nsuper = q.Ho / TR;
  for (int st = wid; st < nsuper; st += nwaves) {
    constexpr int RS = PAR ? 2 : 1;
    const int h0 = PAR ? (st >> 1) * (2 * TR) + (st & 1) : st * TR;
    const char* base = smem + a_off + h0 * q.sh * q.Ws * 2;
    nv_f4 acc[ND];
#pragma unroll
    for (int d = 0; d < ND; d++) acc[d] = nv_f4{0.f, 0.f, 0.f, 0.f};
#ifdef NCV_SKIP
    if (NCV_SKIP & 1) { acc[0][0] = (float)lane; }
    else
#endif
    {
    auto kstep = [&](auto ksc) {
      constexpr int ks = decltype(ksc)::value;
      unsigned int sg[NSEG * 4 + 1];
#pragma unroll
      for (int e = 0; e < NSEG; e++) {
        const uint4 v = *reinterpret_cast<const uint4*>(base + koff[ks] + e * 16);
        sg[e * 4 + 0] = v.x; sg[e * 4 + 1] = v.y; sg[e * 4 + 2] = v.z; sg[e * 4 + 3] = v.w;
      }
      sg[NSEG * 4] = 0;
#pragma unroll
      for (int d = 0; d < ND; d++) {
        const int o = PH0 + d * NS * SW;
        const int dq = o >> 1;
        unsigned int f[4];
#pragma unroll
        for (int j = 0; j < 4; j++) f[j] = (o & 1) ? __builtin_amdgcn_alignbit(sg[dq + j + 1], sg[dq + j], 16) : sg[dq + j];
        typedef unsigned int u4v __attribute__((ext_vector_type(4)));
        const u4v fv = {f[0], f[1], f[2], f[3]};
        acc[d] = __builtin_amdgcn_mfma_f32_16x16x32_bf16(__builtin_bit_cast(nv_bf8, fv), wfr[ks], acc[d], 0, 0, 0);
// ... 10 lines not shown
    if (ADD && co < q.CO) {
#pragma unroll
      for (int k = 0; k < NROW; k++) {
        const int i = row0 + k, tr = i / ncg, cg = i - tr * ncg;
        const bf16_t* a = ap + (h0 + RS * tr) * q.Wo + cg * P;
        if (P == 8) addv[k] = *reinterpret_cast<const uint4*>(a);
        else { const uint2 t = *reinterpret_cast<const uint2*>(a); addv[k] = make_uint4(t.x, t.y, 0, 0); }
      }
    }
    if (STATS) sa.tiles++;
    if (NS == 1) {
      unsigned int prev[P / 2];
#pragma unroll
      for (int rr = 0; rr < 4; rr++) {
        const int i = (lane >> 4) * 4 + rr;
        const int tr = i / ncg, cg = i - tr * ncg;
        bf16_t* o = yc + (h0 + RS * tr) * q.Wo + cg * P;
        unsigned int pk[P / 2];
#pragma unroll
        for (int d = 0; d < P; d += 2) {
          const bf16_t lo(acc[d % ND][rr] + bv), hi(acc[(d + 1) % ND][rr] + bv);
          pk[d >> 1] = (unsigned)lo.bits | ((unsigned)hi.bits << 16);
        }
        if (ADD) {
#pragma unroll
          for (int j = 0; j < P / 2; j++) pk[j] = add_bf16x2(pk[j], (&addv[rr % NROW].x)[j]);
        }
        if (STATS) {
          if (P == 8) ncv_stats_take(sa, pk[0], pk[1], pk[2 % (P / 2)], pk[3 % (P / 2)]);
          else if (rr & 1) ncv_stats_take(sa, prev[0], prev[1], pk[0], pk[1]);
          else { prev[0] = pk[0]; prev[1] = pk[1]; }
        }
        if (co < q.CO NCV_STORE_COND) {
          if (P == 8) *reinterpret_cast<uint4*>(o) = make_uint4(pk[0], pk[1], pk[2 % (P / 2)], pk[3 % (P / 2)]);
          else *reinterpret_cast<uint2*>(o) = make_uint2(pk[0], pk[1]);
          if constexpr (MIRROR) *reinterpret_cast<uint4*>(mc + (h0 + tr) * mws + cg * 8) = make_uint4(pk[0], pk[1], pk[2 % (P / 2)], pk[3 % (P / 2)]);
        }
      }
    } else {
      const int sft = (lane >> 3) & 1;
      unsigned int keep[2][ND], got[2][ND];
#pragma unroll
      for (int h = 0; h < 2; h++)
#pragma unroll
        for (int d = 0; d < ND; d++) {
          const bf16_t mine(acc[d][sft * 2 + h] + bv), theirs(acc[d][(1 - sft) * 2 + h] + bv);
          keep[h][d] = mine.bits;
          got[h][d] = (unsigned)__shfl_xor((int)theirs.bits, 8, 64);
        }
      unsigned int prev[ND];
#pragma unroll
      for (int h = 0; h < 2; h++) {
        const int i = (lane >> 4) * 4 + sft * 2 + h;
        const int tr = i / ncg, cg = i - tr * ncg;
        bf16_t* o = yc + (h0 + RS * tr) * q.Wo + cg * P;
        unsigned int pk[ND];
#pragma unroll
        for (int d = 0; d < ND; d++) {
          const unsigned int even = sft ? got[h][d] : keep[h][d], odd = sft ? keep[h][d] : got[h][d];
          pk[d] = even | (odd << 16);
        }
        if (ADD) {
#pragma unroll
          for (int d = 0; d < ND; d++) pk[d] = add_bf16x2(pk[d], (&addv[h % NROW].x)[d]);
        }
        if (STATS) {
          if (P == 8) ncv_stats_take(sa, pk[0], pk[1], pk[2 % ND], pk[3 % ND]);
          else if (h) ncv_stats_take(sa, prev[0], prev[1], pk[0], pk[1]);
          else { prev[0] = pk[0]; prev[1] = pk[1]; }
        }
        if (co < q.CO NCV_STORE_COND) {
          if (P == 8) *reinterpret_cast<uint4*>(o) = make_uint4(pk[0], pk[1], pk[2 % ND], pk[3 % ND]);
          else *reinterpret_cast<uint2*>(o) = make_uint2(pk[0], pk[1]);
          if constexpr (MIRROR) *reinterpret_cast<uint4*>(mc + (h0 + tr) * mws + cg * 8) = make_uint4(pk[0], pk[1], pk[2 % ND], pk[3 % ND]);
        }
      }
    }
  }
}

template <int NK, int SW, int PH0, int NS, bool ADD, bool STATS, bool PAR = false>
__global__ __launch_bounds__(256, (STATS && NK <= 5) ? 3 : 1) void ncv_fwd2_kernel(const bf16_t* __restrict__ src, const nv_bf8* __restrict__ wpk, const bf16_t* __restrict__ bias,
                                                       bf16_t* dst, NcvGeom q, const bf16_t* add, bf16_t* dst2, const bf16_t* __restrict__ bias2, int co_a,
                                                       float* __restrict__ stats, float* __restrict__ stats2, int stats_per_wg,
                                                       const bf16_t* __restrict__ src2) {
  __shared__ float sst[STATS ? 2 : 1][4][16][3];
  extern __shared__ __attribute__((aligned(16))) char smem[];
  unsigned short* xs = reinterpret_cast<unsigned short*>(smem);
  NCV_STAMP_AT(0);
  constexpr int P = 8 / SW;
  const int tid = threadIdx.x, lane = tid & 63, wid = tid >> 6, nthreads = blockDim.x, nwaves = nthreads >> 6;
  const int co = NS == 2 ? (lane & 7) : (lane & 15);
  const int ncg = q.Wo / P;
  const int64_t img_in = (int64_t)q.C1 * q.H * q.W, img_in2 = (int64_t)(q.C - q.C1) * q.H * q.W;
  NcvPre pre;
  const NcvPlan plan = ncv_stage_plan(q, tid, nthreads);
  if (q.pf && (int)blockIdx.x < q.N) ncv_stage_load(pre, plan, src + blockIdx.x * img_in, src2 + blockIdx.x * img_in2);
  nv_bf8 wfr[NK];
  int koff[NK];
  ncv_frag_setup<NK, PAR>(q, wpk, lane, wfr, koff);
  const float bv = co < co_a ? (bias ? (float)bias[co] : 0.f) : ((bias2 && co < q.CO) ? (float)bias2[co - co_a] : 0.f);
#ifdef NCV_STAMP
  __builtin_amdgcn_s_waitcnt(0);
  NCV_STAMP_AT(1);
#endif
  const int HoWo = q.Ho * q.Wo;
  const int img_elems = q.C * q.Hs * q.Ws;
  for (int o = tid * 8; o < img_elems; o += nthreads * 8) *reinterpret_cast<uint4*>(xs + o) = make_uint4(0, 0, 0, 0);
  const int a_tr = (lane & 15) / ncg, a_cg = (lane & 15) - a_tr * ncg;
  const int a_off = ((PAR ? 2 : 1) * a_tr * q.sh * q.Ws + a_cg * 8 + (q.wx - PH0)) * 2;
  constexpr int VPT = 16 * P / NS;
  NcvStatAcc sa{nv_f4{0.f, 0.f, 0.f, 0.f}, nv_f4{0.f, 0.f, 0.f, 0.f}, 0};
  int it = 0;
  for (int n = blockIdx.x; n < q.N; n += gridDim.x, it++) {
    __syncthreads();
    NCV_STAMP_ONCE(2);
    if (STATS && !stats_per_wg && it > 0) ncv_stats_flush<NS>(sst[(it - 1) & 1], lane, wid, nwaves, q.CO, co_a, stats, stats2, n - (int)gridDim.x, q.N);
#if defined(NCV_SKIP) && (NCV_SKIP & 4)
    if (n < 0)
#endif
    {
    if (q.pf) ncv_stage_store(xs, pre, plan, q.dil);
    else ncv_stage(xs, src + n * img_in, q, tid, nthreads);
    }
    __syncthreads();
    NCV_STAMP_ONCE(3);
#if defined(NCV_SKIP) && (NCV_SKIP & 4)
    if (n < 0)
#endif
    if (q.pf && n + (int)gridDim.x < q.N)
      ncv_stage_load(pre, plan, src + (n + (int)gridDim.x) * img_in, src2 + (n + (int)gridDim.x) * img_in2);
    bf16_t* yc = co < co_a ? dst + ((int64_t)n * co_a + co) * HoWo : dst2 + ((int64_t)n * (q.CO - co_a) + (co - co_a)) * HoWo;
    const bf16_t* ap = ADD ? add + (int64_t)n * q.CO * HoWo + co * HoWo : nullptr;
    ncv_super_tiles<NK, SW, PH0, NS, ADD, STATS, PAR, false>(smem, q, wfr, koff, a_off, bv, co, yc, ap, sa, nullptr, 0, lane, wid, nwaves);
    if (STATS && !stats_per_wg) ncv_stats_leave<VPT>(sa, sst[it & 1], lane, wid);
    NCV_STAMP_ONCE(4);
  }
  if (STATS && it > 0) {
    if (stats_per_wg) ncv_stats_leave<VPT>(sa, sst[0], lane, wid);
    __syncthreads();
    if (stats_per_wg) ncv_stats_flush<NS>(sst[0], lane, wid, nwaves, q.CO, co_a, stats, stats2, (int)blockIdx.x, (int)gridDim.x);
    else ncv_stats_flush<NS>(sst[(it - 1) & 1], lane, wid, nwaves, q.CO, co_a, stats, stats2, (int)blockIdx.x + (it - 1) * (int)gridDim.x, q.N);
  }
#ifdef NCV_STAMP
  NCV_STAMP_AT(5);
  __builtin_amdgcn_s_waitcnt(0);
  NCV_STAMP_AT(6);
#endif
}

constexpr int NCV_CHAIN_PF = 2;
template <int NK0, int PH00, int NK1, int PH01, bool STATS>
__global__ __launch_bounds__(256, NK1 <= 5 ? 3 : 1) void ncv_chain_kernel(const bf16_t* __restrict__ x, const nv_bf8* __restrict__ wpk0, const bf16_t* __restrict__ bias0,
                                                                          bf16_t* s, NcvGeom q0, const nv_bf8* __restrict__ wpk1, const bf16_t* __restrict__ bias1,
                                                                          const bf16_t* __restrict__ bias1b, bf16_t* ya, bf16_t* yb, int co_a, NcvGeom q1,
                                                                          float* __restrict__ stats, float* __restrict__ stats2, int stats_per_wg) {
  __shared__ float sst[STATS ? 2 : 1][4][16][3];
  extern __shared__ __attribute__((aligned(16))) char smem[];
  const int img0 = q0.C * q0.Hs * q0.Ws, img1 = q1.C * q1.Hs * q1.Ws;
  unsigned short* xs0 = reinterpret_cast<unsigned short*>(smem);
  unsigned short* xs1 = xs0 + img0;
  const int tid = threadIdx.x, lane = tid & 63, wid = tid >> 6;
  const int co0 = lane & 7, co1 = lane & 15;
  const int64_t img_in = (int64_t)q0.C * q0.H * q0.W;
  NcvPreT<NCV_CHAIN_PF> pre;
  const NcvPlanT<NCV_CHAIN_PF> plan = ncv_stage_plan<NCV_CHAIN_PF>(q0, tid, 256);
  if ((int)blockIdx.x < q0.N) ncv_stage_load(pre, plan, x + blockIdx.x * img_in, x);
  nv_bf8 wfr1[NK1];
  int koff1[NK1];
  ncv_frag_setup<NK1, false>(q1, wpk1, lane, wfr1, koff1);
  const float bv0 = (bias0 && co0 < q0.CO) ? (float)bias0[co0] : 0.f;
  const float bv1 = co1 < co_a ? (bias1 ? (float)bias1[co1] : 0.f) : ((bias1b && co1 < q1.CO) ? (float)bias1b[co1 - co_a] : 0.f);
  for (int o = tid * 8; o < img0 + img1; o += 256 * 8) *reinterpret_cast<uint4*>(xs0 + o) = make_uint4(0, 0, 0, 0);
  const int ncg0 = q0.Wo / 8, ncg1 = q1.Wo / 4;
  const int a_tr0 = (lane & 15) / ncg0, a_cg0 = (lane & 15) - a_tr0 * ncg0;
  const int a_off0 = (a_tr0 * q0.sh * q0.Ws + a_cg0 * 8 + (q0.wx - PH00)) * 2;
  const int a_tr1 = (lane & 15) / ncg1, a_cg1 = (lane & 15) - a_tr1 * ncg1;
  const int a_off1 = (a_tr1 * q1.sh * q1.Ws + a_cg1 * 8 + (q1.wx - PH01)) * 2;
  const int HoWo0 = q0.Ho * q0.Wo, HoWo1 = q1.Ho * q1.Wo;
  unsigned short* mc = xs1 + (co0 * q1.Hs + q1.top) * q1.Ws + q1.left;
  constexpr int VPT = 16 * 4;
  NcvStatAcc sa{nv_f4{0.f, 0.f, 0.f, 0.f}, nv_f4{0.f, 0.f, 0.f, 0.f}, 0}, none = sa;
  int it = 0;
  for (int n = blockIdx.x; n < q0.N; n += gridDim.x, it++) {
    __syncthreads();
    if (STATS && !stats_per_wg && it > 0) ncv_stats_flush<1>(sst[(it - 1) & 1], lane, wid, 4, q1.CO, co_a, stats, stats2, n - (int)gridDim.x, q1.N);
    ncv_stage_store(xs0, pre, plan, 1);
    __syncthreads();
    if (n + (int)gridDim.x < q0.N) ncv_stage_load(pre, plan, x + (n + (int)gridDim.x) * img_in, x);
    nv_bf8 wfr0[NK0];
    int koff0[NK0];
    int lane0 = lane;
    asm volatile("" : "+v"(lane0));
    ncv_frag_setup<NK0, false>(q0, wpk0, lane0, wfr0, koff0);
    ncv_super_tiles<NK0, 1, PH00, 2, false, false, false, true>(smem, q0, wfr0, koff0, a_off0, bv0, co0, s + ((int64_t)n * q0.CO + co0) * HoWo0, nullptr, none,
                                                                mc, q1.Ws, lane, wid, 4);
    __syncthreads();
    bf16_t* yc = co1 < co_a ? ya + ((int64_t)n * co_a + co1) * HoWo1 : yb + ((int64_t)n * (q1.CO - co_a) + (co1 - co_a)) * HoWo1;
    ncv_super_tiles<NK1, 2, PH01, 1, false, STATS, false, false>(reinterpret_cast<const char*>(xs1), q1, wfr1, koff1, a_off1, bv1, co1, yc, nullptr, sa, nullptr, 0,
                                                                 lane, wid, 4);
    if (STATS && !stats_per_wg) ncv_stats_leave<VPT>(sa, sst[it & 1], lane, wid);
  }
  if (STATS && it > 0) {
    if (stats_per_wg) ncv_stats_leave<VPT>(sa, sst[0], lane, wid);
    __syncthreads();
    if (stats_per_wg) ncv_stats_flush<1>(sst[0], lane, wid, 4, q1.CO, co_a, stats, stats2, (int)blockIdx.x, (int)gridDim.x);
    else ncv_stats_flush<1>(sst[(it - 1) & 1], lane, wid, 4, q1.CO, co_a, stats, stats2, (int)blockIdx.x + (it - 1) * (int)gridDim.x, q1.N);
  }
}
#ifdef NCV_STAMP
extern "C" int lamp_debug_ncv_stamps(unsigned long long* out) { return hipMemcpyFromSymbol(out, HIP_SYMBOL(ncv_stamps), sizeof(ncv_stamps)) == hipSuccess ? 0 : 1; }
#endif

struct NcvWGeom {
  int N, Cin, Cout, H, W, Ho, Wo;
  int kh, kw, ph, pw;
  int Hs, Ws;
  int ncol;
  int IG;
  int Cout2;
};
constexpr int NCV_OFF2 = 4;

template <int NT, int SW>
__global__ __launch_bounds__(256) void ncv_wgrad_kernel(const bf16_t* __restrict__ dy, const bf16_t* __restrict__ x, float* __restrict__ partial, NcvWGeom q,
                                                        int images_per_block) {
  extern __shared__ __attribute__((aligned(16))) char smem[];
  const int tid = threadIdx.x, lane = tid & 63, wid = tid >> 6;
  const int HoWo = q.Ho * q.Wo;
  const int ximg = q.Cin * q.Hs * q.Ws * (SW == 2 ? 2 : 1);
  unsigned short* xs = reinterpret_cast<unsigned short*>(smem);
  unsigned short* ds = xs + q.IG * ximg;
// ... 49 lines not shown
    __syncthreads();
    const int nchunks = ig * chunks_per_img;
    for (int ch = wid; ch < nchunks; ch += 4) {
      const int pg = ch * 32 + (lane >> 4) * 8;
      const int im = pg / HoWo, pp = pg - im * HoWo;
      const int ho = pp / q.Wo, wo0 = pp - ho * q.Wo;
      const nv_s8 a = *reinterpret_cast<const nv_s8*>(ds + (im * 16 + (lane & 15)) * HoWo + pp);
      const char* xb = reinterpret_cast<const char*>(xs + im * ximg) +
                       (SW == 1 ? (ho * q.Ws + wo0) * 2 : ((ho * 2) * 2 * q.Ws + wo0) * 2);
#pragma unroll
      for (int nt = 0; nt < NT; nt++) {
        const nv_s8 b = *reinterpret_cast<const nv_s8_u*>(xb + coff[nt]);
        acc[nt] = __builtin_amdgcn_mfma_f32_16x16x32_bf16(__builtin_bit_cast(nv_bf8, a), __builtin_bit_cast(nv_bf8, b), acc[nt], 0, 0, 0);
      }
    }
  }
#pragma unroll
  for (int nt = 0; nt < NT; nt++)
#pragma unroll
    for (int rr = 0; rr < 4; rr++) red[(wid * 16 + (lane >> 4) * 4 + rr) * (NT * 16) + nt * 16 + (lane & 15)] = acc[nt][rr];
  __syncthreads();
  const int O = q.Cout * q.ncol;
  for (int i = tid; i < O; i += 256) {
    const int co = i / q.ncol, cidx = i - co * q.ncol;
    float a = 0.f;
#pragma unroll
    for (int w = 0; w < 4; w++) a += red[(w * 16 + co) * (NT * 16) + cidx];
    partial[(int64_t)blockIdx.x * O + i] = a;
  }
}

constexpr int NCV_OFFA = 8;
constexpr int NCV_WPF = 6;
template <int KW, int PW, int SW, int NPT>
__global__ __launch_bounds__(256) void ncv_wgrad2_kernel(const bf16_t* __restrict__ dy, const bf16_t* __restrict__ x, float* __restrict__ partial, NcvWGeom q,
                                                         int images_per_block, const bf16_t* __restrict__ dy2, float* __restrict__ partial2) {
  extern __shared__ __attribute__((aligned(16))) char smem[];
  const int tid = threadIdx.x, lane = tid & 63, wid = tid >> 6;
  const int HoWo = q.Ho * q.Wo;
  const int ximg = q.Cin * q.Hs * q.Ws * (SW == 2 ? 2 : 1);
  unsigned short* xs = reinterpret_cast<unsigned short*>(smem);
  unsigned short* ds = xs + q.IG * ximg;
  constexpr int NCOLT = NPT * KW * 16;
  float* red = reinterpret_cast<float*>(ds + q.IG * 16 * HoWo);
  {
    const int tot = q.IG * (ximg + 16 * HoWo);
    for (int o = tid * 8; o < tot; o += 256 * 8) *reinterpret_cast<uint4*>(xs + o) = make_uint4(0, 0, 0, 0);
  }
  const int npairs = q.Cin * q.kh;
  int poff[NPT];
#pragma unroll
  for (int pt = 0; pt < NPT; pt++) {
    int pair = pt * 16 + (lane & 15);
    if (pair >= npairs) pair = 0;
    const int ci = pair / q.kh, r = pair - ci * q.kh;
    poff[pt] = (SW == 1 ? (ci * q.Hs + r) * q.Ws : (ci * q.Hs + r) * 2 * q.Ws) * 2;
  }
  nv_f4 acc[NPT][KW];
#pragma unroll
  for (int pt = 0; pt < NPT; pt++)
#pragma unroll
    for (int s = 0; s < KW; s++) acc[pt][s] = nv_f4{0.f, 0.f, 0.f, 0.f};

  const int64_t n0 = (int64_t)blockIdx.x * images_per_block, n1 = min<int64_t>(n0 + images_per_block, q.N);
  const int chunks_per_img = HoWo >> 5;
  const int xpk = (q.Cin * q.H * q.W) >> 3, dpk = (q.Cout * HoWo) >> 3, dpk2 = (q.Cout2 * HoWo) >> 3, per = xpk + dpk + dpk2;
  const int rc = q.W >> 3;
  const bool pf = q.IG * per <= NCV_WPF * 256;
  uint4 pre[NCV_WPF];
  int p_src[NCV_WPF], p_dst[NCV_WPF], p_im[NCV_WPF];
#pragma unroll
  for (int k = 0; k < NCV_WPF; k++) {
    const int idx = tid + k * 256;
    const int im = idx / per, j = idx - im * per;
    p_im[k] = (pf && im < q.IG) ? im : -1;
    if (j < xpk) {
      const int b = j % rc, a = (j / rc) % q.H, c = j / (rc * q.H);
      p_src[k] = im * q.Cin * q.H * q.W + j * 8;
      p_dst[k] = im * ximg + (SW == 1 ? (c * q.Hs + q.ph + a) * q.Ws + NCV_OFFA + b * 8 : ((c * q.Hs + q.ph + a) * 2) * q.Ws + NCV_OFFA + b * 4);
    } else if (j < xpk + dpk) {
      p_src[k] = -(im * q.Cout * HoWo + (j - xpk) * 8) - 1;
      p_dst[k] = q.IG * ximg + im * 16 * HoWo + (j - xpk) * 8;
    } else {
      p_src[k] = -(im * q.Cout2 * HoWo + (j - xpk - dpk) * 8) - 1 - (1 << 30);
      p_dst[k] = q.IG * ximg + im * 16 * HoWo + q.Cout * HoWo + (j - xpk - dpk) * 8;
    }
  }
  auto pre_load = [&](int64_t nb, int ig) {
    const bf16_t* xg = x + nb * q.Cin * q.H * q.W;
    const bf16_t* dg = dy + nb * q.Cout * HoWo;
    const bf16_t* dg2 = dy2 + nb * q.Cout2 * HoWo;
#pragma unroll
    for (int k = 0; k < NCV_WPF; k++)
      if (p_im[k] >= 0 && p_im[k] < ig) {
        const bf16_t* sp = p_src[k] >= 0 ? xg + p_src[k] : p_src[k] >= -(1 << 30) ? dg + (-p_src[k] - 1) : dg2 + (-p_src[k] - 1 - (1 << 30));
        pre[k] = *reinterpret_cast<const uint4*>(sp);
      }
  };
  auto stage_x = [&](unsigned short* dst, const uint4 v) {
    if (SW == 1) {
      *reinterpret_cast<uint4*>(dst) = v;
    } else {
      uint2 ev, od;
      ev.x = (v.x & 0xffffu) | (v.y << 16); ev.y = (v.z & 0xffffu) | (v.w << 16);
      od.x = (v.x >> 16) | (v.y & 0xffff0000u); od.y = (v.z >> 16) | (v.w & 0xffff0000u);
      *reinterpret_cast<uint2*>(dst) = ev;
      *reinterpret_cast<uint2*>(dst + q.Ws) = od;
    }
  };
  auto pre_store = [&](int ig) {
#pragma unroll
    for (int k = 0; k < NCV_WPF; k++) {
      if (p_im[k] < 0 || p_im[k] >= ig) continue;
      const uint4 v = pre[k];
      if (SW == 1 || p_src[k] < 0) *reinterpret_cast<uint4*>(xs + p_dst[k]) = v;
      else stage_x(xs + p_dst[k], v);
    }
  };
  auto x_dst = [&](unsigned short* xi, int j) {
    const int b = j % rc, a = (j / rc) % q.H, c = j / (rc * q.H);
    return xi + (SW == 1 ? (c * q.Hs + q.ph + a) * q.Ws + NCV_OFFA + b * 8 : ((c * q.Hs + q.ph + a) * 2) * q.Ws + NCV_OFFA + b * 4);
  };

  if (pf && n0 < n1) pre_load(n0, (int)min<int64_t>(q.IG, n1 - n0));
  for (int64_t nb = n0; nb < n1; nb += q.IG) {
    const int ig = (int)min<int64_t>(q.IG, n1 - nb);
    __syncthreads();
#if defined(NCV_WSKIP) && (NCV_WSKIP & 4)
    if (nb < 0)
#endif
    if (pf) pre_store(ig);
    else for (int im = 0; im < ig; im++) {
      const bf16_t* xp = x + (nb + im) * q.Cin * q.H * q.W;
      unsigned short* xi = xs + im * ximg;
      for (int i = tid; i < xpk; i += 256) stage_x(x_dst(xi, i), *reinterpret_cast<const uint4*>(xp + i * 8));
      const bf16_t* dp = dy + (nb + im) * q.Cout * HoWo;
      unsigned short* di = ds + im * 16 * HoWo;
      for (int i = tid; i < dpk; i += 256) *reinterpret_cast<uint4*>(di + i * 8) = *reinterpret_cast<const uint4*>(dp + i * 8);
      const bf16_t* dp2 = dy2 + (nb + im) * q.Cout2 * HoWo;
      for (int i = tid; i < dpk2; i += 256) *reinterpret_cast<uint4*>(di + q.Cout * HoWo + i * 8) = *reinterpret_cast<const uint4*>(dp2 + i * 8);
    }
    __syncthreads();
#if defined(NCV_WSKIP) && (NCV_WSKIP & 4)
    if (nb < 0)
#endif
    if (pf && nb + q.IG < n1) pre_load(nb + q.IG, (int)min<int64_t>(q.IG, n1 - nb - q.IG));
    const int nchunks = ig * chunks_per_img;
#if defined(NCV_WSKIP) && (NCV_WSKIP & 1)
    if (nb < 0)
#endif
    for (int ch = wid; ch < nchunks; ch += 4) {
      const int pg = ch * 32 + (lane >> 4) * 8;
      const int im = pg / HoWo, pp = pg - im * HoWo;
      const int ho = pp / q.Wo, wo0 = pp - ho * q.Wo;
      const nv_s8 a = *reinterpret_cast<const nv_s8*>(ds + (im * 16 + (lane & 15)) * HoWo + pp);
      const nv_bf8 af = __builtin_bit_cast(nv_bf8, a);
      const char* xb = reinterpret_cast<const char*>(xs + im * ximg) +
                       (SW == 1 ? (ho * q.Ws + wo0 + NCV_OFFA - 8) * 2 : ((ho * 2) * 2 * q.Ws + wo0 + NCV_OFFA - 8) * 2);
#pragma unroll
      for (int pt = 0; pt < NPT; pt++) {
        const char* rowp = xb + poff[pt];
        if (SW == 1) {
          constexpr bool need_m = PW > 0, need_p = (KW - 1 - PW) > 0;
          unsigned int sg[13];
          const uint4 z = make_uint4(0, 0, 0, 0);
          const uint4 v0 = need_m ? *reinterpret_cast<const uint4*>(rowp) : z;
          const uint4 v1 = *reinterpret_cast<const uint4*>(rowp + 16);
          const uint4 v2 = need_p ? *reinterpret_cast<const uint4*>(rowp + 32) : z;
          sg[0] = v0.x; sg[1] = v0.y; sg[2] = v0.z; sg[3] = v0.w; sg[4] = v1.x; sg[5] = v1.y; sg[6] = v1.z; sg[7] = v1.w;
          sg[8] = v2.x; sg[9] = v2.y; sg[10] = v2.z; sg[11] = v2.w; sg[12] = 0;
#pragma unroll
          for (int s = 0; s < KW; s++) {
            const int o = 8 + s - PW;
            const int dq = o >> 1;
            typedef unsigned int u4v __attribute__((ext_vector_type(4)));
            u4v f;
#pragma unroll
            for (int j = 0; j < 4; j++) f[j] = (o & 1) ? __builtin_amdgcn_alignbit(sg[dq + j + 1], sg[dq + j], 16) : sg[dq + j];
            acc[pt][s] = __builtin_amdgcn_mfma_f32_16x16x32_bf16(af, __builtin_bit_cast(nv_bf8, f), acc[pt][s], 0, 0, 0);
          }
        } else {
          unsigned int sg[2][9];
#pragma unroll
          for (int par = 0; par < 2; par++) {
            const uint4 v0 = *reinterpret_cast<const uint4*>(rowp + par * q.Ws * 2);
            const uint4 v1 = *reinterpret_cast<const uint4*>(rowp + par * q.Ws * 2 + 16);
            sg[par][0] = v0.x; sg[par][1] = v0.y; sg[par][2] = v0.z; sg[par][3] = v0.w;
            sg[par][4] = v1.x; sg[par][5] = v1.y; sg[par][6] = v1.z; sg[par][7] = v1.w; sg[par][8] = 0;
          }
#pragma unroll
          for (int s = 0; s < KW; s++) {
            const int t = s - PW, par = t & 1, half = (t - par) >> 1;
            const int o = 8 + half, dq = o >> 1;
            typedef unsigned int u4v __attribute__((ext_vector_type(4)));
            u4v f;
#pragma unroll
            for (int j = 0; j < 4; j++) f[j] = (o & 1) ? __builtin_amdgcn_alignbit(sg[par][dq + j + 1], sg[par][dq + j], 16) : sg[par][dq + j];
            acc[pt][s] = __builtin_amdgcn_mfma_f32_16x16x32_bf16(af, __builtin_bit_cast(nv_bf8, f), acc[pt][s], 0, 0, 0);
          }
        }
      }
    }
  }
#pragma unroll
  for (int pt = 0; pt < NPT; pt++)
#pragma unroll
    for (int s = 0; s < KW; s++)
#pragma unroll
      for (int rr = 0; rr < 4; rr++) red[(wid * 16 + (lane >> 4) * 4 + rr) * NCOLT + (pt * KW + s) * 16 + (lane & 15)] = acc[pt][s][rr];
  __syncthreads();
  const int O = q.Cout * q.ncol;
  for (int i = tid; i < O; i += 256) {
    const int co = i / q.ncol, cidx = i - co * q.ncol;
    const int pair = cidx / KW, s = cidx - pair * KW;
    const int col = ((pair >> 4) * KW + s) * 16 + (pair & 15);
    float a = 0.f;
#pragma unroll
    for (int w = 0; w < 4; w++) a += red[(w * 16 + co) * NCOLT + col];
    partial[(int64_t)blockIdx.x * O + i] = a;
  }
  const int O2 = q.Cout2 * q.Cin;
  for (int i = tid; i < O2; i += 256) {
    const int co2 = i / q.Cin, ci = i - co2 * q.Cin;
    const int pair = ci * q.kh + (q.kh >> 1), s = KW >> 1;
    const int col = ((pair >> 4) * KW + s) * 16 + (pair & 15);
    float a = 0.f;
#pragma unroll
    for (int w = 0; w < 4; w++) a += red[(w * 16 + q.Cout + co2) * NCOLT + col];
    partial2[(int64_t)blockIdx.x * O2 + i] = a;
  }
}


static inline int round_up(int v, int m) { return (v + m - 1) / m * m; }

static bool ncv_common(const ConvGeom& g, int dtype) {
  if (dtype != kBF16) return false;
  if (g.groups != 1 || g.transposed || g.dh != 1 || g.dw != 1) return false;
  if (g.Cin > 16 || g.Cout > 16 || g.N < 1) return false;
  if (g.sh != g.sw || g.sh < 1 || g.sh > 2) return false;
  if (g.kw > 8 || g.ph > g.kh - 1 || g.pw > g.kw - 1 || g.pw > 8) return false;
  return true;
}

template <int NK>
static void ncv_launch(const bf16_t* src, const nv_bf8* wpk, const bf16_t* bias, bf16_t* dst, const NcvGeom& q, int blocks, size_t lds, hipStream_t st) {
  hipLaunchKernelGGL((ncv_fwd_kernel<NK>), dim3(blocks), dim3(256), lds, st, src, wpk, bias, dst, q);
}

static PackCache g_ncv_packs;
constexpr int64_t NCV_PACK_ELEMS = (int64_t)NCV_NKMAX * 64 * 8;
enum { NCV_T_COUT, NCV_T_CIN, NCV_T_KH, NCV_T_KW, NCV_T_DGRAD, NCV_T_NS, NCV_T_SW, NCV_T_COUT2 };

void narrow_pack_launch(const NcvPackMany& a, int cnt, hipStream_t st) {
  hipLaunchKernelGGL(ncv_pack_kernel, dim3((NCV_NKMAX * 64 + 255) / 256, (unsigned)cnt), dim3(256), 0, st, a);
  LAMP_LAUNCH_CHECK();
}

static Tensor* ncv_packed_weights(const Tensor* w, const NcvW& wq, hipStream_t st, const Tensor* w2 = nullptr) {
  const bool cacheable = PackCache::cacheable(w, w2);
  const PackKey key{w->st->uid, w->offset, {wq.Cout, wq.Cin, wq.kh, wq.kw, wq.dgrad, wq.ns + 16 * wq.nke, wq.sw, w2 ? wq.Cout2 : 0}, st,
                    w2 ? w2->st->uid : 0, w2 ? w2->offset : 0};
  const uint64_t ver = PackCache::version_of(w), ver2 = PackCache::version_of(w2);
// ... 311 lines not shown
    bf16_t* y1p = y1->ptr<bf16_t>();
    int co_a = (int)g.Cout;
    void* args[] = {(void*)&xp, (void*)&wpk0, (void*)&b0p, (void*)&sp, (void*)&q0, (void*)&wpk1, (void*)&bp, (void*)&b1p, (void*)&yp, (void*)&y1p,
                    (void*)&co_a, (void*)&q1, (void*)&statp, (void*)&stat2p, (void*)&stats_per_wg};
    HIP_CHECK(hipLaunchKernel(kfn, dim3(blocks), dim3(256), args, lds, st));
    LAMP_LAUNCH_CHECK();
  }
  if (statt.get()) conv_stats_publish(y, statt.get(), parts, 0);
  if (statt2.get()) conv_stats_publish(y1, statt2.get(), parts);
  return true;
}
bool narrow_conv_dgrad(const Tensor* dy, const Tensor* w, Tensor* dx, const ConvGeom& g, hipStream_t st, const Tensor* addend, bool* addend_fused) {
  return ncv_run(dy, w, nullptr, dx, g, true, st, addend, addend_fused);
}
bool narrow_conv_dgrad_pair(const Tensor* dy, const Tensor* w, const ConvGeom& g, const Tensor* dy1, const Tensor* w1, const ConvGeom& g1, Tensor* dx,
                            hipStream_t st, const Tensor* addend, bool* addend_fused) {
  if (addend_fused) *addend_fused = false;
  const bool on = sw().conv_dgrad_pair;
  if (!on || dy->dtype != kBF16 || dy1->dtype != kBF16) return false;
  if (g.kh != 3 || g.kw != 3 || g.ph != 1 || g.pw != 1 || g1.kh != 1 || g1.kw != 1 || g1.ph != 0 || g1.pw != 0) return false;
  if (g.sh != g1.sh || g.sw != g1.sw || g.Ho != g1.Ho || g.Wo != g1.Wo || g.H != g1.H || g.W != g1.W || g.Cin != g1.Cin || g.N != g1.N) return false;
  if (g.groups != 1 || g1.groups != 1 || g.dh != 1 || g.dw != 1 || g1.dh != 1 || g1.dw != 1 || g1.Cout > 16) return false;
  const NcvSecondGrad sg{dy1, w1};
  return ncv_run(dy, w, nullptr, dx, g, true, st, addend, addend_fused, nullptr, &sg);
}

template <int NT, int SW>
static void ncv_wg_launch(const bf16_t* dy, const bf16_t* x, float* partial, const NcvWGeom& q, int ipb, int blocks, size_t lds, hipStream_t st) {
  static bool attr = false;
  allow_big_lds((const void*)ncv_wgrad_kernel<NT, SW>);
  hipLaunchKernelGGL((ncv_wgrad_kernel<NT, SW>), dim3(blocks), dim3(256), lds, st, dy, x, partial, q, ipb);
}

struct NcvSecondWgrad { const Tensor* dy; Tensor* dw; };
static bool ncv_wgrad_run(const Tensor* dy, const Tensor* x, Tensor* dw, const ConvGeom& g, hipStream_t st, const NcvSecondWgrad* second) {
  if (!ncv_common(g, x->dtype)) return false;
  if (g.W % 8 != 0 || g.Wo % 8 != 0 || (g.Ho * g.Wo) % 32 != 0) return false;
  const int cout2 = second ? (int)second->dy->sizes[1] : 0;
  if (second && (g.Cout + cout2 > 16 || g.kh != 3 || g.kw != 3 || g.ph != 1 || g.pw != 1)) return false;
  NcvWGeom q;
  q.N = (int)g.N; q.Cin = (int)g.Cin; q.Cout = (int)g.Cout; q.H = (int)g.H; q.W = (int)g.W; q.Ho = (int)g.Ho; q.Wo = (int)g.Wo;
  q.kh = g.kh; q.kw = g.kw; q.ph = g.ph; q.pw = g.pw; q.Cout2 = cout2;
  q.ncol = (int)g.Cin * g.kh * g.kw;
  const int SW = g.sh;
  q.Hs = std::max((int)g.H + 2 * g.ph, ((int)g.Ho - 1) * g.sh + g.kh);
  if (SW == 1) q.Ws = round_up(std::max(NCV_LEFT + (int)g.W, (int)g.Wo - 1 + g.kw - 1 - g.pw + NCV_LEFT + 1), 8);
  else {
    const int half_max = (g.kw - 1 - g.pw) >> 1;
    q.Ws = round_up(std::max((int)g.W / 2, (int)g.Wo + half_max) + NCV_OFF2 + 1, 8);
  }
  const int HoWo = (int)(g.Ho * g.Wo);
  q.IG = std::max(1, 256 / HoWo);
  const int npt = (int)((g.Cin * g.kh + 15) / 16);
  const bool aligned = g.kh == g.kw && npt <= 3 &&
                       ((g.kw == 5 && g.pw == 2 && SW == 1) || (g.kw == 3 && g.pw == 1) || (g.kw == 1 && g.pw == 0));
  if (aligned) {
    if (SW == 1) q.Ws = round_up(NCV_OFFA + std::max((int)g.W, (int)g.Wo + 8) + 8, 8);
    else q.Ws = round_up(NCV_OFFA + std::max((int)g.W / 2, (int)g.Wo) + 8, 8);
    const int ximg2 = q.Cin * q.Hs * q.Ws * (SW == 2 ? 2 : 1);
    const int ncolt = npt * g.kw * 16;
    const size_t lds2 = (size_t)q.IG * (ximg2 + 16 * HoWo) * 2 + (size_t)4 * 16 * ncolt * 4;
    if (lds2 <= 150 * 1024) {
      const int O = q.Cout * q.ncol;
      const void* kfn = nullptr;
#define NCV_WG2(KWv, PWv, SWv, NPTv) kfn = (const void*)ncv_wgrad2_kernel<KWv, PWv, SWv, NPTv>
#define NCV_WG2_NPT(KWv, PWv, SWv) do { if (npt == 1) NCV_WG2(KWv, PWv, SWv, 1); else if (npt == 2) NCV_WG2(KWv, PWv, SWv, 2); else NCV_WG2(KWv, PWv, SWv, 3); } while (0)
      if (g.kw == 5) NCV_WG2_NPT(5, 2, 1);
      else if (g.kw == 3 && SW == 1) NCV_WG2_NPT(3, 1, 1);
      else if (g.kw == 3) NCV_WG2_NPT(3, 1, 2);
      else if (SW == 1) NCV_WG2_NPT(1, 0, 1);
      else NCV_WG2_NPT(1, 0, 2);
#undef NCV_WG2_NPT
#undef NCV_WG2
      allow_big_lds(kfn);
      const int per_cu = std::min((int)std::max<size_t>(1, std::min<size_t>(4, (size_t)(150 * 1024) / lds2)), kernel_occupancy(kfn, 256, lds2));
      const int64_t rounds = (g.N + q.IG - 1) / q.IG;
      const int nb = (int)std::min<int64_t>(rounds, (int64_t)num_cus() * per_cu);
      const int ipb = (int)((rounds + nb - 1) / nb) * q.IG;
      const int nblocks = (int)((g.N + ipb - 1) / ipb);
      int64_t ps[1] = {(int64_t)nblocks * O};
      Hold partial(new_tensor(ps, 1, kF32, dy->device()));
      const int O2 = cout2 * q.Cin;
      Hold partial2;
      if (second) { int64_t ps2[1] = {(int64_t)nblocks * O2}; partial2 = Hold(new_tensor(ps2, 1, kF32, dy->device())); }
      {
        const double sec_fl = second ? 2.0 * (double)g.N * cout2 * (double)g.Ho * g.Wo * (double)g.Cin : 0.0;
        const double sec_by = second ? ((double)g.N * cout2 * g.Ho * g.Wo + (double)cout2 * g.Cin) * 2.0 : 0.0;
        KernelTimer kt("conv_wgrad_narrow", conv_flops(g) + sec_fl, conv_bytes(g, 2) + sec_by, st);
        const bf16_t* dp = dy->ptr<bf16_t>(); const bf16_t* xp = x->ptr<bf16_t>(); float* pp = partial->ptr<float>();
        const bf16_t* dp2 = second ? second->dy->ptr<bf16_t>() : (const bf16_t*)nullptr;
        float* pp2 = second ? partial2->ptr<float>() : (float*)nullptr;
        int ipb_arg = ipb;
        void* args[] = {(void*)&dp, (void*)&xp, (void*)&pp, (void*)&q, (void*)&ipb_arg, (void*)&dp2, (void*)&pp2};
        HIP_CHECK(hipLaunchKernel(kfn, dim3(nblocks), dim3(256), args, lds2, st));
        LAMP_LAUNCH_CHECK();
      }
      WgradReduceArgs ra{};
      ra.kind = 1; ra.O = O; ra.nsplit = nblocks; ra.blocks = (int)(((int64_t)O * 64 + 255) / 256);
      wgrad_reduce_enqueue(ra, partial.get(), dw, st);
      if (second) {
        WgradReduceArgs rb{};
        rb.kind = 1; rb.O = O2; rb.nsplit = nblocks; rb.blocks = (int)(((int64_t)O2 * 64 + 255) / 256);
        wgrad_reduce_enqueue(rb, partial2.get(), second->dw, st);
      }
      return true;
    }
    if (second) return false;
    if (SW == 1) q.Ws = round_up(std::max(NCV_LEFT + (int)g.W, (int)g.Wo - 1 + g.kw - 1 - g.pw + NCV_LEFT + 1), 8);
    else { const int half_max = (g.kw - 1 - g.pw) >> 1; q.Ws = round_up(std::max((int)g.W / 2, (int)g.Wo + half_max) + NCV_OFF2 + 1, 8); }
  }
  if (second) return false;
  const int nt_real = (q.ncol + 15) / 16;
  static const int nt_opts[] = {1, 2, 4, 5, 9};
  int NT = 0;
  for (int o : nt_opts) if (o >= nt_real) { NT = o; break; }
  if (!NT) return false;
  const int ximg = q.Cin * q.Hs * q.Ws * (SW == 2 ? 2 : 1);
  if ((q.IG * (ximg + 16 * HoWo)) % 8 != 0) return false;
  const size_t lds = (size_t)q.IG * (ximg + 16 * HoWo) * 2 + (size_t)4 * 16 * NT * 16 * 4;
  if (lds > 150 * 1024) return false;
  const int O = q.Cout * q.ncol;
  const int per_cu = (int)std::max<size_t>(1, std::min<size_t>(4, (size_t)(150 * 1024) / lds));
  const int64_t rounds = (g.N + q.IG - 1) / q.IG;
  const int nb = (int)std::min<int64_t>(rounds, (int64_t)num_cus() * per_cu);
  const int ipb = (int)((rounds + nb - 1) / nb) * q.IG;
  const int nblocks = (int)((g.N + ipb - 1) / ipb);
  int64_t ps[1] = {(int64_t)nblocks * O};
  Hold partial(new_tensor(ps, 1, kF32, dy->device()));
  {
    KernelTimer kt("conv_wgrad_narrow", conv_flops(g), conv_bytes(g, 2), st);
    const bf16_t* dp = dy->ptr<bf16_t>(); const bf16_t* xp = x->ptr<bf16_t>(); float* pp = partial->ptr<float>();
#define NCV_WG(NTv)                                                                                          \
  do {                                                                                                       \
    if (SW == 1) ncv_wg_launch<NTv, 1>(dp, xp, pp, q, ipb, nblocks, lds, st);                                \
    else ncv_wg_launch<NTv, 2>(dp, xp, pp, q, ipb, nblocks, lds, st);                                        \
  } while (0)
    switch (NT) {
      case 1: NCV_WG(1); break;
      case 2: NCV_WG(2); break;
      case 4: NCV_WG(4); break;
      case 5: NCV_WG(5); break;
      default: NCV_WG(9); break;
    }
#undef NCV_WG
    LAMP_LAUNCH_CHECK();
  }
  WgradReduceArgs ra{};
  ra.kind = 1; ra.O = O; ra.nsplit = nblocks; ra.blocks = (int)(((int64_t)O * 64 + 255) / 256);
  wgrad_reduce_enqueue(ra, partial.get(), dw, st);
  return true;
}

bool narrow_conv_wgrad(const Tensor* dy, const Tensor* x, Tensor* dw, const ConvGeom& g, hipStream_t st) { return ncv_wgrad_run(dy, x, dw, g, st, nullptr); }
bool narrow_conv_wgrad_pair(const Tensor* dy, const Tensor* dy1, const Tensor* x, Tensor* dw, Tensor* dw1, const ConvGeom& g, const ConvGeom& g1, hipStream_t st) {
  const bool on = sw().conv_wgrad_pair;
  if (!on || x->dtype != kBF16 || dy->dtype != kBF16 || dy1->dtype != kBF16) return false;
  if (g1.kh != 1 || g1.kw != 1 || g1.ph != 0 || g1.pw != 0) return false;
  if (g.sh != g1.sh || g.sw != g1.sw || g.Ho != g1.Ho || g.Wo != g1.Wo || g.H != g1.H || g.W != g1.W || g.Cin != g1.Cin || g.N != g1.N) return false;
  if (g.groups != 1 || g1.groups != 1 || g.dh != 1 || g.dw != 1 || g1.dh != 1 || g1.dw != 1) return false;
  const NcvSecondWgrad sw{dy1, dw1};
  return ncv_wgrad_run(dy, x, dw, g, st, &sw);
}

}
```

Baseline: 2.239 million samples/s.

## Fuse block's paired input gradient with preceding conv's weight gradient in one kernel

```diff
diff --git a/include/lamp_hip.h b/include/lamp_hip.h
--- a/include/lamp_hip.h
+++ b/include/lamp_hip.h
@@ -319,6 +319,12 @@
                                 const int64_t* dilation_a, const lamp_tensor* w_b, const lamp_tensor* bias_b_or_null,
                                 const int64_t* stride_b, const int64_t* padding_b, const int64_t* dilation_b, int nspatial,
                                 int64_t groups);
+int lamp_convolution_backward_chain_pair(lamp_tensor** out_dw0, const lamp_tensor* x, const lamp_tensor* w, const int64_t* stride,
+                                         const int64_t* padding, const int64_t* dilation, const lamp_tensor* grad_a,
+                                         const lamp_tensor* w_a, const int64_t* stride_a, const int64_t* padding_a,
+                                         const int64_t* dilation_a, const lamp_tensor* grad_b, const lamp_tensor* w_b,
+                                         const int64_t* stride_b, const int64_t* padding_b, const int64_t* dilation_b, int nspatial,
+                                         int64_t groups);
 int lamp_avg_pool2d(lamp_tensor** out, const lamp_tensor* x, int64_t kernel, int64_t stride, int64_t padding,
                     int ceil_mode, int count_include_pad);
 int lamp_avg_pool2d_backward(lamp_tensor** out, const lamp_tensor* grad_out, const lamp_tensor* x, int64_t kernel,
diff --git a/jni/LampNative.java b/jni/LampNative.java
--- a/jni/LampNative.java
+++ b/jni/LampNative.java
@@ -252,6 +252,7 @@
   public static native long[] lamp_convolution_backward_weight_pair(long x, long grad_out_a, long w_a, long[] stride_a, long[] padding_a, long[] dilation_a, long grad_out_b, long w_b, long[] stride_b, long[] padding_b, long[] dilation_b, long groups);
   public static native long[] lamp_convolution_pair(long x, long w_a, long bias_a_or_null, long[] stride_a, long[] padding_a, long[] dilation_a, long w_b, long bias_b_or_null, long[] stride_b, long[] padding_b, long[] dilation_b, long groups);
   public static native long[] lamp_convolution_chain_pair(long x, long w, long bias_or_null, long[] stride, long[] padding, long[] dilation, long w_a, long bias_a_or_null, long[] stride_a, long[] padding_a, long[] dilation_a, long w_b, long bias_b_or_null, long[] stride_b, long[] padding_b, long[] dilation_b, long groups);
+  public static native long lamp_convolution_backward_chain_pair(long x, long w, long[] stride, long[] padding, long[] dilation, long grad_a, long w_a, long[] stride_a, long[] padding_a, long[] dilation_a, long grad_b, long w_b, long[] stride_b, long[] padding_b, long[] dilation_b, long groups);
   public static native long lamp_avg_pool2d(long x, long kernel, long stride, long padding, int ceil_mode, int count_include_pad);
   public static native long lamp_avg_pool2d_backward(long grad_out, long x, long kernel, long stride, long padding, int ceil_mode, int count_include_pad);
   public static native long[] lamp_max_pool2d_with_indices(long x, long kernel, long stride, long padding, long dilation, int ceil_mode);
diff --git a/jni/aten_jni.c b/jni/aten_jni.c
--- a/jni/aten_jni.c
+++ b/jni/aten_jni.c
@@ -2036,6 +2036,49 @@
   return a_;
 }
 
+JNIEXPORT jlong JNICALL Java_aten_LampNative_lamp_1convolution_1backward_1chain_1pair(JNIEnv* env, jclass cls, jlong x, jlong w, jlongArray stride, jlongArray padding, jlongArray dilation, jlong grad_a, jlong w_a, jlongArray stride_a, jlongArray padding_a, jlongArray dilation_a, jlong grad_b, jlong w_b, jlongArray stride_b, jlongArray padding_b, jlongArray dilation_b, jlong groups) {
+  (void)cls;
+  jsize stride_n = (*env)->GetArrayLength(env, stride);
+  jlong* stride_e = (*env)->GetLongArrayElements(env, stride, NULL);
+  (void)stride_n;
+  jsize padding_n = (*env)->GetArrayLength(env, padding);
+  jlong* padding_e = (*env)->GetLongArrayElements(env, padding, NULL);
+  (void)padding_n;
+  jsize dilation_n = (*env)->GetArrayLength(env, dilation);
+  jlong* dilation_e = (*env)->GetLongArrayElements(env, dilation, NULL);
+  (void)dilation_n;
+  jsize stride_a_n = (*env)->GetArrayLength(env, stride_a);
+  jlong* stride_a_e = (*env)->GetLongArrayElements(env, stride_a, NULL);
+  (void)stride_a_n;
+  jsize padding_a_n = (*env)->GetArrayLength(env, padding_a);
+  jlong* padding_a_e = (*env)->GetLongArrayElements(env, padding_a, NULL);
+  (void)padding_a_n;
+  jsize dilation_a_n = (*env)->GetArrayLength(env, dilation_a);
+  jlong* dilation_a_e = (*env)->GetLongArrayElements(env, dilation_a, NULL);
+  (void)dilation_a_n;
+  jsize stride_b_n = (*env)->GetArrayLength(env, stride_b);
+  jlong* stride_b_e = (*env)->GetLongArrayElements(env, stride_b, NULL);
+  (void)stride_b_n;
+  jsize padding_b_n = (*env)->GetArrayLength(env, padding_b);
+  jlong* padding_b_e = (*env)->GetLongArrayElements(env, padding_b, NULL);
+  (void)padding_b_n;
+  jsize dilation_b_n = (*env)->GetArrayLength(env, dilation_b);
+  jlong* dilation_b_e = (*env)->GetLongArrayElements(env, dilation_b, NULL);
+  void* out_dw0_o = NULL;
+  const int rc_ = lamp_convolution_backward_chain_pair((void*)&out_dw0_o, H(x), H(w), (const int64_t*)stride_e, (const int64_t*)padding_e, (const int64_t*)dilation_e, H(grad_a), H(w_a), (const int64_t*)stride_a_e, (const int64_t*)padding_a_e, (const int64_t*)dilation_a_e, H(grad_b), H(w_b), (const int64_t*)stride_b_e, (const int64_t*)padding_b_e, (const int64_t*)dilation_b_e, (int)dilation_b_n, (int64_t)groups);
+  (*env)->ReleaseLongArrayElements(env, stride, stride_e, JNI_ABORT);
+  (*env)->ReleaseLongArrayElements(env, padding, padding_e, JNI_ABORT);
+  (*env)->ReleaseLongArrayElements(env, dilation, dilation_e, JNI_ABORT);
+  (*env)->ReleaseLongArrayElements(env, stride_a, stride_a_e, JNI_ABORT);
+  (*env)->ReleaseLongArrayElements(env, padding_a, padding_a_e, JNI_ABORT);
+  (*env)->ReleaseLongArrayElements(env, dilation_a, dilation_a_e, JNI_ABORT);
+  (*env)->ReleaseLongArrayElements(env, stride_b, stride_b_e, JNI_ABORT);
+  (*env)->ReleaseLongArrayElements(env, padding_b, padding_b_e, JNI_ABORT);
+  (*env)->ReleaseLongArrayElements(env, dilation_b, dilation_b_e, JNI_ABORT);
+  if (rc_ != 0) { lamp_throw(env); return 0; }
+  return (jlong)(intptr_t)out_dw0_o;
+}
+
 JNIEXPORT jlong JNICALL Java_aten_LampNative_lamp_1avg_1pool2d(JNIEnv* env, jclass cls, jlong x, jlong kernel, jlong stride, jlong padding, jint ceil_mode, jint count_include_pad) {
   (void)cls;
   void* out_o = NULL;
diff --git a/lamp_amd/csrc/core/host_staging.cpp b/lamp_amd/csrc/core/host_staging.cpp
--- a/lamp_amd/csrc/core/host_staging.cpp
+++ b/lamp_amd/csrc/core/host_staging.cpp
@@ -82,6 +82,8 @@
 int lamp_convolution(lamp_tensor** out, const lamp_tensor* x, const lamp_tensor* w, const lamp_tensor* bias_or_null, const int64_t* stride, const int64_t* padding, const int64_t* dilation, int nspatial, int transposed, const int64_t* output_padding, int64_t groups) { return S::call(lamp_convolution__dev, S::Out{out}, S::In{x}, S::In{w}, S::In{bias_or_null}, stride, padding, dilation, nspatial, transposed, output_padding, groups); }
 int lamp_convolution_backward__dev(lamp_tensor* out3[3], const lamp_tensor* grad_out, const lamp_tensor* x, const lamp_tensor* w, const int64_t* stride, const int64_t* padding, const int64_t* dilation, int nspatial, int transposed, const int64_t* output_padding, int64_t groups, const uint8_t mask[3]);
 int lamp_convolution_backward(lamp_tensor* out3[3], const lamp_tensor* grad_out, const lamp_tensor* x, const lamp_tensor* w, const int64_t* stride, const int64_t* padding, const int64_t* dilation, int nspatial, int transposed, const int64_t* output_padding, int64_t groups, const uint8_t mask[3]) { return S::call(lamp_convolution_backward__dev, S::OutK<3>{out3}, S::In{grad_out}, S::In{x}, S::In{w}, stride, padding, dilation, nspatial, transposed, output_padding, groups, mask); }
+int lamp_convolution_backward_chain_pair__dev(lamp_tensor** out_dw0, const lamp_tensor* x, const lamp_tensor* w, const int64_t* stride, const int64_t* padding, const int64_t* dilation, const lamp_tensor* grad_a, const lamp_tensor* w_a, const int64_t* stride_a, const int64_t* padding_a, const int64_t* dilation_a, const lamp_tensor* grad_b, const lamp_tensor* w_b, const int64_t* stride_b, const int64_t* padding_b, const int64_t* dilation_b, int nspatial, int64_t groups);
+int lamp_convolution_backward_chain_pair(lamp_tensor** out_dw0, const lamp_tensor* x, const lamp_tensor* w, const int64_t* stride, const int64_t* padding, const int64_t* dilation, const lamp_tensor* grad_a, const lamp_tensor* w_a, const int64_t* stride_a, const int64_t* padding_a, const int64_t* dilation_a, const lamp_tensor* grad_b, const lamp_tensor* w_b, const int64_t* stride_b, const int64_t* padding_b, const int64_t* dilation_b, int nspatial, int64_t groups) { return S::call(lamp_convolution_backward_chain_pair__dev, S::Out{out_dw0}, S::In{x}, S::In{w}, stride, padding, dilation, S::In{grad_a}, S::In{w_a}, stride_a, padding_a, dilation_a, S::In{grad_b}, S::In{w_b}, stride_b, padding_b, dilation_b, nspatial, groups); }
 int lamp_convolution_backward_input_add__dev(lamp_tensor** out, const lamp_tensor* grad_out, const lamp_tensor* x, const lamp_tensor* w, const int64_t* stride, const int64_t* padding, const int64_t* dilation, int nspatial, const int64_t* output_padding, int64_t groups, const lamp_tensor* addend);
 int lamp_convolution_backward_input_add(lamp_tensor** out, const lamp_tensor* grad_out, const lamp_tensor* x, const lamp_tensor* w, const int64_t* stride, const int64_t* padding, const int64_t* dilation, int nspatial, const int64_t* output_padding, int64_t groups, const lamp_tensor* addend) { return S::call(lamp_convolution_backward_input_add__dev, S::Out{out}, S::In{grad_out}, S::In{x}, S::In{w}, stride, padding, dilation, nspatial, output_padding, groups, S::In{addend}); }
 int lamp_convolution_backward_input_pair__dev(lamp_tensor** out, const lamp_tensor* x, const lamp_tensor* grad_out_a, const lamp_tensor* w_a, const int64_t* stride_a, const int64_t* padding_a, const int64_t* dilation_a, const lamp_tensor* grad_out_b, const lamp_tensor* w_b, const int64_t* stride_b, const int64_t* padding_b, const int64_t* dilation_b, int nspatial, int64_t groups, const lamp_tensor* addend_or_null);
diff --git a/lamp_amd/csrc/core/switches.h b/lamp_amd/csrc/core/switches.h
--- a/lamp_amd/csrc/core/switches.h
+++ b/lamp_amd/csrc/core/switches.h
@@ -9,6 +9,7 @@
                                                         \
   X(conv_sibling, "LAMP_CONV_SIBLING", BOOL, 1, 0, "a residual block's 3x3 and its sibling 1x1 of the same input as one forward launch") \
   X(conv_chain, "LAMP_CONV_CHAIN", BOOL, 1, 0, "a convolution directly in front of a residual block and the block's 3x3 + 1x1 as one forward call (0: two)") \
+  X(conv_chain_bwd, "LAMP_CONV_CHAIN_BWD", BOOL, 1, 0, "a block's paired input gradient and the weight gradient of the convolution in front of it as one call where nothing else needs the gradient between them (0: two)") \
   X(fuse_bn_pair, "LAMP_FUSE_BN_PAIR", BOOL, 1, 0, "relu(bn(right) + bn(left)) at a block's end as one op (0: the chain)")                \
   X(fuse_pool_logsoftmax, "LAMP_FUSE_POOL_LOGSOFTMAX", BOOL, 1, 0, "average pool -> flatten -> log-softmax tail as one node")             \
   X(fuse_block_tail, "LAMP_FUSE_BLOCK_TAIL", BOOL, 1, 0, "the last residual block and the pooled log-softmax tail as one node")          \
diff --git a/lamp_amd/csrc/host/autograd.h b/lamp_amd/csrc/host/autograd.h
--- a/lamp_amd/csrc/host/autograd.h
+++ b/lamp_amd/csrc/host/autograd.h
@@ -120,12 +120,18 @@
 using Var = std::shared_ptr<Variable>;
 using Backward = std::function<void(const Ten& p, Variable& out)>;
 
+struct PairOutputGrads {
+  Ten p[2], w[2];
+  std::vector<int64_t> stride[2], padding[2], dilation[2];
+  int64_t groups = 1;
+};
 struct Op {
   virtual ~Op() = default;
   std::vector<std::pair<Var, Backward>> params;
   const char* name = "op";
   std::function<void()> reset;
   std::function<void(const Ten& plane_grad)> pooled_input_grad;
+  std::function<bool(const PairOutputGrads& pair)> chain_pair_grad;
 };
 
 struct Variable {
diff --git a/lamp_amd/csrc/host/ops.cpp b/lamp_amd/csrc/host/ops.cpp
--- a/lamp_amd/csrc/host/ops.cpp
+++ b/lamp_amd/csrc/host/ops.cpp
@@ -684,6 +684,7 @@
   Ten iv = input->value, wv = weight->value;
   const bool fuse_accumulate = sw().conv_dgrad_accumulate;
   const bool fuse_pair = sw().conv_dgrad_pair;
+  const bool fuse_chain_bwd = sw().conv_chain_bwd && fuse_pair;
   auto back = [=](int which) {
     std::function<void(const Ten&, Variable&)> single;
     single = [=](const Ten& p, Variable& out) {
@@ -758,21 +759,53 @@
       const int other = st.waiting;
       const Ten po = st.side[other].p;
       st.side[other].p = Ten(); st.waiting = -1;
-      const Ten& pa = pair_side == 0 ? p : po;
-      const Ten& pb = pair_side == 0 ? po : p;
-      const bool have = out.has_grad() && out.grad.h()->is_device() && out.grad.dtype() == p.dtype();
-      if (out.has_grad() && !have) { single(po, out); single(p, out); return; }
-      lamp_tensor* r = nullptr;
-      HCALL(lamp_convolution_backward_input_pair(&r, iv.h(), pa.h(), st.side[0].w.h(), st.side[0].stride.data(), st.side[0].padding.data(),
-                                                 st.side[0].dilation.data(), pb.h(), st.side[1].w.h(), st.side[1].stride.data(),
-                                                 st.side[1].padding.data(), st.side[1].dilation.data(), ns, st.groups, have ? out.grad.h() : nullptr));
-      out.grad = Ten(r);
-      out.grad_shared = false;
+      auto both = [=](const Ten& p, const Ten& po, Variable& out) {
+        const ConvPairGrad& st = *pair;
+        const Ten& pa = pair_side == 0 ? p : po;
+        const Ten& pb = pair_side == 0 ? po : p;
+        const bool have = out.has_grad() && out.grad.h()->is_device() && out.grad.dtype() == p.dtype();
+        if (out.has_grad() && !have) { single(po, out); single(p, out); return; }
+        lamp_tensor* r = nullptr;
+        HCALL(lamp_convolution_backward_input_pair(&r, iv.h(), pa.h(), st.side[0].w.h(), st.side[0].stride.data(), st.side[0].padding.data(),
+                                                   st.side[0].dilation.data(), pb.h(), st.side[1].w.h(), st.side[1].stride.data(),
+                                                   st.side[1].padding.data(), st.side[1].dilation.data(), ns, st.groups, have ? out.grad.h() : nullptr));
+        out.grad = Ten(r);
+        out.grad_shared = false;
+      };
+      if (fuse_chain_bwd && out.op && out.op->chain_pair_grad) {
+        Variable* outp = &out;
+        out.pending.push_back([=] {
+          if (!outp->has_grad()) {
+            const ConvPairGrad& s2 = *pair;
+            PairOutputGrads g;
+            g.p[0] = pair_side == 0 ? p : po; g.p[1] = pair_side == 0 ? po : p;
+            for (int i = 0; i < 2; i++) { g.w[i] = s2.side[i].w; g.stride[i] = s2.side[i].stride; g.padding[i] = s2.side[i].padding; g.dilation[i] = s2.side[i].dilation; }
+            g.groups = s2.groups;
+            if (outp->op->chain_pair_grad(g)) return;
+          }
+          both(p, po, *outp);
+        });
+        return;
+      }
+      both(p, po, out);
     });
   };
   op->params.push_back({input, back(0)});
   op->params.push_back({weight, back(1)});
   op->params.push_back({bias, back(2)});
+  if (fuse_chain_bwd && !transposed && !input->needsGrad() && weight->needsGrad() && !weight->op && !bias->needsGrad() && iv.h()->is_device() &&
+      wv.h()->is_device() && iv.dtype() == kBF16 && wv.dtype() == kBF16) {
+    Variable* wvar = weight.get();
+    op->chain_pair_grad = [=](const PairOutputGrads& g) {
+      if (g.groups != groups || !g.p[0].h()->is_device() || !g.p[1].h()->is_device()) return false;
+      lamp_tensor* r = nullptr;
+      HCALL(lamp_convolution_backward_chain_pair(&r, iv.h(), wv.h(), stride.data(), padding.data(), dilation.data(), g.p[0].h(), g.w[0].h(), g.stride[0].data(),
+                                                 g.padding[0].data(), g.dilation[0].data(), g.p[1].h(), g.w[1].h(), g.stride[1].data(), g.padding[1].data(),
+                                                 g.dilation[1].data(), ns, groups));
+      wvar->accumulate(Ten(r), true);
+      return true;
+    };
+  }
   if (pair) op->reset = [pair] {
     pair->waiting = pair->wwaiting = -1;
     for (auto& sd : pair->side) { sd.p = Ten(); sd.pw = Ten(); sd.wout = nullptr; }
diff --git a/lamp_amd/csrc/kernels/abi_dev_names.h b/lamp_amd/csrc/kernels/abi_dev_names.h
--- a/lamp_amd/csrc/kernels/abi_dev_names.h
+++ b/lamp_amd/csrc/kernels/abi_dev_names.h
@@ -38,6 +38,7 @@
 #define lamp_ceil_ lamp_ceil___dev
 #define lamp_convolution lamp_convolution__dev
 #define lamp_convolution_backward lamp_convolution_backward__dev
+#define lamp_convolution_backward_chain_pair lamp_convolution_backward_chain_pair__dev
 #define lamp_convolution_backward_input_add lamp_convolution_backward_input_add__dev
 #define lamp_convolution_backward_input_pair lamp_convolution_backward_input_pair__dev
 #define lamp_convolution_backward_weight_pair lamp_convolution_backward_weight_pair__dev
diff --git a/lamp_amd/csrc/kernels/conv.hip b/lamp_amd/csrc/kernels/conv.hip
--- a/lamp_amd/csrc/kernels/conv.hip
+++ b/lamp_amd/csrc/kernels/conv.hip
@@ -603,6 +603,51 @@
   LAMP_API_END
 }
 
+int lamp_convolution_backward_chain_pair(lamp_tensor** out_dw0, const lamp_tensor* x, const lamp_tensor* w, const int64_t* stride, const int64_t* padding,
+                                         const int64_t* dilation, const lamp_tensor* grad_a, const lamp_tensor* w_a, const int64_t* stride_a,
+                                         const int64_t* padding_a, const int64_t* dilation_a, const lamp_tensor* grad_b, const lamp_tensor* w_b,
+                                         const int64_t* stride_b, const int64_t* padding_b, const int64_t* dilation_b, int nspatial, int64_t groups) {
+  LAMP_API_BEGIN
+  *out_dw0 = nullptr;
+  check_device_tensor(x, "input"); check_device_tensor(w, "weight"); check_device_tensor(grad_a, "first grad_out"); check_device_tensor(w_a, "first weight");
+  check_device_tensor(grad_b, "second grad_out"); check_device_tensor(w_b, "second weight");
+  const int64_t zero2[2] = {0, 0};
+  ConvGeom g0 = make_geom(x, w, stride, padding, dilation, nspatial, 0, zero2, groups);
+  LAMP_CHECK(g0.Ho > 0 && g0.Wo > 0, "convolution_backward_chain_pair: the first convolution has an empty output");
+  std::vector<int64_t> sshape = {g0.N, g0.Cout};
+  if (nspatial == 2) sshape.push_back(g0.Ho);
+  sshape.push_back(g0.Wo);
+  Hold s(new_tensor(sshape, x->dtype, x->device()));
+  if (nspatial == 2 && x->ndim == 4 && x->dtype == kBF16 && w->dtype == kBF16 && w_a->dtype == kBF16 && w_b->dtype == kBF16 && grad_a->dtype == kBF16 &&
+      grad_b->dtype == kBF16 && w_a->ndim == 4 && w_b->ndim == 4 && grad_a->ndim == 4 && grad_b->ndim == 4) {
+    if (w_a->sizes[1] * groups == g0.Cout && w_b->sizes[1] * groups == g0.Cout) {
+      ConvGeom ga = make_geom(s.get(), w_a, stride_a, padding_a, dilation_a, nspatial, 0, zero2, groups);
+      ConvGeom gb = make_geom(s.get(), w_b, stride_b, padding_b, dilation_b, nspatial, 0, zero2, groups);
+      auto grad_ok = [&](const lamp_tensor* gy, const ConvGeom& g) { return gy->sizes[0] == g.N && gy->sizes[1] == g.Cout && gy->sizes[2] == g.Ho && gy->sizes[3] == g.Wo; };
+      if (grad_ok(grad_a, ga) && grad_ok(grad_b, gb)) {
+        Hold xc(contiguous(x)), wa(contiguous_filter(w_a)), wb(contiguous_filter(w_b)), gya(contiguous(grad_a)), gyb(contiguous(grad_b));
+        Hold w0(contiguous_filter(w));
+        Hold dw(new_like(w0.get()));
+        hipStream_t st = current_stream(x->device());
+        if (narrow_conv_chain_bwd(xc.get(), g0, gya.get(), wa.get(), ga, gyb.get(), wb.get(), gb, dw.get(), st)) {
+          *out_dw0 = dw.take();
+          return 0;
+        }
+      }
+    }
+  }
+  lamp_tensor* ds = nullptr;
+  if (lamp_convolution_backward_input_pair(&ds, s.get(), grad_a, w_a, stride_a, padding_a, dilation_a, grad_b, w_b, stride_b, padding_b, dilation_b, nspatial, groups,
+                                           nullptr) != 0)
+    throw Error(lamp_last_error());
+  Hold hds(ds);
+  const uint8_t m3[3] = {0, 1, 0};
+  lamp_tensor* r3[3] = {nullptr, nullptr, nullptr};
+  if (lamp_convolution_backward(r3, hds.get(), x, w, stride, padding, dilation, nspatial, 0, zero2, groups, m3) != 0) throw Error(lamp_last_error());
+  *out_dw0 = r3[1];
+  LAMP_API_END
+}
+
 int lamp_convolution_backward_weight_pair(lamp_tensor* out2[2], const lamp_tensor* x, const lamp_tensor* grad_out_a, const lamp_tensor* w_a,
                                           const int64_t* stride_a, const int64_t* padding_a, const int64_t* dilation_a,
                                           const lamp_tensor* grad_out_b, const lamp_tensor* w_b, const int64_t* stride_b,
diff --git a/lamp_amd/csrc/kernels/conv_backends.h b/lamp_amd/csrc/kernels/conv_backends.h
--- a/lamp_amd/csrc/kernels/conv_backends.h
+++ b/lamp_amd/csrc/kernels/conv_backends.h
@@ -27,6 +27,8 @@
                           Tensor* y1, const ConvGeom& g1, hipStream_t st);
 bool narrow_conv_chain_pair(const Tensor* x, const Tensor* w0, const Tensor* bias0, Tensor* s, const ConvGeom& g0, const Tensor* w, const Tensor* bias,
                             Tensor* y, const ConvGeom& g, const Tensor* w1, const Tensor* bias1, Tensor* y1, const ConvGeom& g1, hipStream_t st);
+bool narrow_conv_chain_bwd(const Tensor* x, const ConvGeom& g0, const Tensor* dy, const Tensor* w, const ConvGeom& g, const Tensor* dy1, const Tensor* w1,
+                           const ConvGeom& g1, Tensor* dw0, hipStream_t st);
 bool narrow_conv_dgrad(const Tensor* dy, const Tensor* w, Tensor* dx, const ConvGeom& g, hipStream_t st, const Tensor* addend = nullptr,
                        bool* addend_fused = nullptr);
 bool narrow_conv_dgrad_pair(const Tensor* dy, const Tensor* w, const ConvGeom& g, const Tensor* dy1, const Tensor* w1, const ConvGeom& g1, Tensor* dx,
diff --git a/lamp_amd/csrc/kernels/conv_narrow.hip b/lamp_amd/csrc/kernels/conv_narrow.hip
--- a/lamp_amd/csrc/kernels/conv_narrow.hip
+++ b/lamp_amd/csrc/kernels/conv_narrow.hip
@@ -215,13 +215,13 @@
     o[0] = cnt; o[1] = mean; o[2] = fmaxf(sq - sy * mean, 0.f);
   }
 }
-template <int NK, int SW, int PH0, int NS, bool ADD, bool STATS, bool PAR, bool MIRROR>
+template <int NK, int SW, int PH0, int NS, bool ADD, bool STATS, bool PAR, int MIRROR>
 __device__ __forceinline__ void ncv_super_tiles(const char* smem, const NcvGeom& q, const nv_bf8 (&wfr)[NK], const int (&koff)[NK], int a_off, float bv, int co,
                                                 bf16_t* yc, const bf16_t* ap, NcvStatAcc& sa, unsigned short* mc, int mws, int lane, int wid, int nwaves) {
   constexpr int P = 8 / SW;
   constexpr int ND = P / NS;
   constexpr int NSEG = (PH0 + (ND - 1) * NS * SW + 7) < 16 ? 2 : 3;
-  static_assert(!MIRROR || (P == 8 && !PAR), "the LDS copy takes whole 16-byte packets of plain tiles");
+  static_assert(!MIRROR || P == 8, "the LDS copy takes whole 16-byte packets");
   const int ncg = q.Wo / P, TR = 16 / ncg;
   const int nsuper = q.Ho / TR;
   for (int st = wid; st < nsuper; st += nwaves) {
@@ -298,9 +298,11 @@
           else { prev[0] = pk[0]; prev[1] = pk[1]; }
         }
         if (co < q.CO NCV_STORE_COND) {
-          if (P == 8) *reinterpret_cast<uint4*>(o) = make_uint4(pk[0], pk[1], pk[2 % (P / 2)], pk[3 % (P / 2)]);
-          else *reinterpret_cast<uint2*>(o) = make_uint2(pk[0], pk[1]);
-          if constexpr (MIRROR) *reinterpret_cast<uint4*>(mc + (h0 + tr) * mws + cg * 8) = make_uint4(pk[0], pk[1], pk[2 % (P / 2)], pk[3 % (P / 2)]);
+          if constexpr (MIRROR != 2) {
+            if (P == 8) *reinterpret_cast<uint4*>(o) = make_uint4(pk[0], pk[1], pk[2 % (P / 2)], pk[3 % (P / 2)]);
+            else *reinterpret_cast<uint2*>(o) = make_uint2(pk[0], pk[1]);
+          }
+          if constexpr (MIRROR != 0) *reinterpret_cast<uint4*>(mc + (h0 + RS * tr) * mws + cg * 8) = make_uint4(pk[0], pk[1], pk[2 % (P / 2)], pk[3 % (P / 2)]);
         }
       }
     } else {
@@ -336,9 +338,11 @@
           else { prev[0] = pk[0]; prev[1] = pk[1]; }
         }
         if (co < q.CO NCV_STORE_COND) {
-          if (P == 8) *reinterpret_cast<uint4*>(o) = make_uint4(pk[0], pk[1], pk[2 % ND], pk[3 % ND]);
-          else *reinterpret_cast<uint2*>(o) = make_uint2(pk[0], pk[1]);
-          if constexpr (MIRROR) *reinterpret_cast<uint4*>(mc + (h0 + tr) * mws + cg * 8) = make_uint4(pk[0], pk[1], pk[2 % ND], pk[3 % ND]);
+          if constexpr (MIRROR != 2) {
+            if (P == 8) *reinterpret_cast<uint4*>(o) = make_uint4(pk[0], pk[1], pk[2 % ND], pk[3 % ND]);
+            else *reinterpret_cast<uint2*>(o) = make_uint2(pk[0], pk[1]);
+          }
+          if constexpr (MIRROR != 0) *reinterpret_cast<uint4*>(mc + (h0 + RS * tr) * mws + cg * 8) = make_uint4(pk[0], pk[1], pk[2 % ND], pk[3 % ND]);
         }
       }
     }
@@ -398,7 +402,7 @@
       ncv_stage_load(pre, plan, src + (n + (int)gridDim.x) * img_in, src2 + (n + (int)gridDim.x) * img_in2);
     bf16_t* yc = co < co_a ? dst + ((int64_t)n * co_a + co) * HoWo : dst2 + ((int64_t)n * (q.CO - co_a) + (co - co_a)) * HoWo;
     const bf16_t* ap = ADD ? add + (int64_t)n * q.CO * HoWo + co * HoWo : nullptr;
-    ncv_super_tiles<NK, SW, PH0, NS, ADD, STATS, PAR, false>(smem, q, wfr, koff, a_off, bv, co, yc, ap, sa, nullptr, 0, lane, wid, nwaves);
+    ncv_super_tiles<NK, SW, PH0, NS, ADD, STATS, PAR, 0>(smem, q, wfr, koff, a_off, bv, co, yc, ap, sa, nullptr, 0, lane, wid, nwaves);
     if (STATS && !stats_per_wg) ncv_stats_leave<VPT>(sa, sst[it & 1], lane, wid);
     NCV_STAMP_ONCE(4);
   }
@@ -459,11 +463,11 @@
     int lane0 = lane;
     asm volatile("" : "+v"(lane0));
     ncv_frag_setup<NK0, false>(q0, wpk0, lane0, wfr0, koff0);
-    ncv_super_tiles<NK0, 1, PH00, 2, false, false, false, true>(smem, q0, wfr0, koff0, a_off0, bv0, co0, s + ((int64_t)n * q0.CO + co0) * HoWo0, nullptr, none,
+    ncv_super_tiles<NK0, 1, PH00, 2, false, false, false, 1>(smem, q0, wfr0, koff0, a_off0, bv0, co0, s + ((int64_t)n * q0.CO + co0) * HoWo0, nullptr, none,
                                                                 mc, q1.Ws, lane, wid, 4);
     __syncthreads();
     bf16_t* yc = co1 < co_a ? ya + ((int64_t)n * co_a + co1) * HoWo1 : yb + ((int64_t)n * (q1.CO - co_a) + (co1 - co_a)) * HoWo1;
-    ncv_super_tiles<NK1, 2, PH01, 1, false, STATS, false, false>(reinterpret_cast<const char*>(xs1), q1, wfr1, koff1, a_off1, bv1, co1, yc, nullptr, sa, nullptr, 0,
+    ncv_super_tiles<NK1, 2, PH01, 1, false, STATS, false, 0>(reinterpret_cast<const char*>(xs1), q1, wfr1, koff1, a_off1, bv1, co1, yc, nullptr, sa, nullptr, 0,
                                                                  lane, wid, 4);
     if (STATS && !stats_per_wg) ncv_stats_leave<VPT>(sa, sst[it & 1], lane, wid);
   }
@@ -579,6 +583,113 @@
 
 constexpr int NCV_OFFA = 8;
 constexpr int NCV_WPF = 6;
+template <int SW>
+__device__ __forceinline__ int ncv_wg_x_dst(const NcvWGeom& q, int j) {
+  const int rc = q.W >> 3;
+  const int b = j % rc, a = (j / rc) % q.H, c = j / (rc * q.H);
+  return SW == 1 ? (c * q.Hs + q.ph + a) * q.Ws + NCV_OFFA + b * 8 : ((c * q.Hs + q.ph + a) * 2) * q.Ws + NCV_OFFA + b * 4;
+}
+template <int SW, int NPT>
+__device__ __forceinline__ void ncv_wg_pair_rows(const NcvWGeom& q, int lane, int (&poff)[NPT]) {
+  const int npairs = q.Cin * q.kh;
+#pragma unroll
+  for (int pt = 0; pt < NPT; pt++) {
+    int pair = pt * 16 + (lane & 15);
+    if (pair >= npairs) pair = 0;
+    const int ci = pair / q.kh, r = pair - ci * q.kh;
+    poff[pt] = (SW == 1 ? (ci * q.Hs + r) * q.Ws : (ci * q.Hs + r) * 2 * q.Ws) * 2;
+  }
+}
+template <int KW, int PW, int SW, int NPT>
+__device__ __forceinline__ void ncv_wg_chunks(const unsigned short* xs, int ximg, const unsigned short* arow, int a_img, const NcvWGeom& q, const int (&poff)[NPT],
+                                              nv_f4 (&acc)[NPT][KW], int nchunks, int lane, int wid) {
+  const int HoWo = q.Ho * q.Wo;
+  for (int ch = wid; ch < nchunks; ch += 4) {
+    const int pg = ch * 32 + (lane >> 4) * 8;
+    const int im = pg / HoWo, pp = pg - im * HoWo;
+    const int ho = pp / q.Wo, wo0 = pp - ho * q.Wo;
+    const nv_s8 a = *reinterpret_cast<const nv_s8*>(arow + im * a_img + pp);
+    const nv_bf8 af = __builtin_bit_cast(nv_bf8, a);
+    const char* xb = reinterpret_cast<const char*>(xs + im * ximg) +
+                     (SW == 1 ? (ho * q.Ws + wo0 + NCV_OFFA - 8) * 2 : ((ho * 2) * 2 * q.Ws + wo0 + NCV_OFFA - 8) * 2);
+#pragma unroll
+    for (int pt = 0; pt < NPT; pt++) {
+      const char* rowp = xb + poff[pt];
+      if (SW == 1) {
+        constexpr bool need_m = PW > 0, need_p = (KW - 1 - PW) > 0;
+        unsigned int sg[13];
+        const uint4 z = make_uint4(0, 0, 0, 0);
+        const uint4 v0 = need_m ? *reinterpret_cast<const uint4*>(rowp) : z;
+        const uint4 v1 = *reinterpret_cast<const uint4*>(rowp + 16);
+        const uint4 v2 = need_p ? *reinterpret_cast<const uint4*>(rowp + 32) : z;
+        sg[0] = v0.x; sg[1] = v0.y; sg[2] = v0.z; sg[3] = v0.w; sg[4] = v1.x; sg[5] = v1.y; sg[6] = v1.z; sg[7] = v1.w;
+        sg[8] = v2.x; sg[9] = v2.y; sg[10] = v2.z; sg[11] = v2.w; sg[12] = 0;
+#pragma unroll
+        for (int s = 0; s < KW; s++) {
+          const int o = 8 + s - PW;
+          const int dq = o >> 1;
+          typedef unsigned int u4v __attribute__((ext_vector_type(4)));
+          u4v f;
+#pragma unroll
+          for (int j = 0; j < 4; j++) f[j] = (o & 1) ? __builtin_amdgcn_alignbit(sg[dq + j + 1], sg[dq + j], 16) : sg[dq + j];
+          acc[pt][s] = __builtin_amdgcn_mfma_f32_16x16x32_bf16(af, __builtin_bit_cast(nv_bf8, f), acc[pt][s], 0, 0, 0);
+        }
+      } else {
+        unsigned int sg[2][9];
+#pragma unroll
+        for (int par = 0; par < 2; par++) {
+          const uint4 v0 = *reinterpret_cast<const uint4*>(rowp + par * q.Ws * 2);
+          const uint4 v1 = *reinterpret_cast<const uint4*>(rowp + par * q.Ws * 2 + 16);
+          sg[par][0] = v0.x; sg[par][1] = v0.y; sg[par][2] = v0.z; sg[par][3] = v0.w;
+          sg[par][4] = v1.x; sg[par][5] = v1.y; sg[par][6] = v1.z; sg[par][7] = v1.w; sg[par][8] = 0;
+        }
+#pragma unroll
+        for (int s = 0; s < KW; s++) {
+          const int t = s - PW, par = t & 1, half = (t - par) >> 1;
+          const int o = 8 + half, dq = o >> 1;
+          typedef unsigned int u4v __attribute__((ext_vector_type(4)));
+          u4v f;
+#pragma unroll
+          for (int j = 0; j < 4; j++) f[j] = (o & 1) ? __builtin_amdgcn_alignbit(sg[par][dq + j + 1], sg[par][dq + j], 16) : sg[par][dq + j];
+          acc[pt][s] = __builtin_amdgcn_mfma_f32_16x16x32_bf16(af, __builtin_bit_cast(nv_bf8, f), acc[pt][s], 0, 0, 0);
+        }
+      }
+    }
+  }
+}
+template <int KW, int NPT>
+__device__ __forceinline__ void ncv_wg_leave(float* red, const nv_f4 (&acc)[NPT][KW], const NcvWGeom& q, float* __restrict__ partial, float* __restrict__ partial2,
+                                             int tid, int lane, int wid) {
+  constexpr int NCOLT = NPT * KW * 16;
+#pragma unroll
+  for (int pt = 0; pt < NPT; pt++)
+#pragma unroll
+    for (int s = 0; s < KW; s++)
+#pragma unroll
+      for (int rr = 0; rr < 4; rr++) red[(wid * 16 + (lane >> 4) * 4 + rr) * NCOLT + (pt * KW + s) * 16 + (lane & 15)] = acc[pt][s][rr];
+  __syncthreads();
+  const int O = q.Cout * q.ncol;
+  for (int i = tid; i < O; i += 256) {
+    const int co = i / q.ncol, cidx = i - co * q.ncol;
+    const int pair = cidx / KW, s = cidx - pair * KW;
+    const int col = ((pair >> 4) * KW + s) * 16 + (pair & 15);
+    float a = 0.f;
+#pragma unroll
+    for (int w = 0; w < 4; w++) a += red[(w * 16 + co) * NCOLT + col];
+    partial[(int64_t)blockIdx.x * O + i] = a;
+  }
+  const int O2 = q.Cout2 * q.Cin;
+  for (int i = tid; i < O2; i += 256) {
+    const int co2 = i / q.Cin, ci = i - co2 * q.Cin;
+    const int pair = ci * q.kh + (q.kh >> 1), s = KW >> 1;
+    const int col = ((pair >> 4) * KW + s) * 16 + (pair & 15);
+    float a = 0.f;
+#pragma unroll
+    for (int w = 0; w < 4; w++) a += red[(w * 16 + q.Cout + co2) * NCOLT + col];
+    partial2[(int64_t)blockIdx.x * O2 + i] = a;
+  }
+}
+
 template <int KW, int PW, int SW, int NPT>
 __global__ __launch_bounds__(256) void ncv_wgrad2_kernel(const bf16_t* __restrict__ dy, const bf16_t* __restrict__ x, float* __restrict__ partial, NcvWGeom q,
                                                          int images_per_block, const bf16_t* __restrict__ dy2, float* __restrict__ partial2) {
@@ -588,21 +699,13 @@
   const int ximg = q.Cin * q.Hs * q.Ws * (SW == 2 ? 2 : 1);
   unsigned short* xs = reinterpret_cast<unsigned short*>(smem);
   unsigned short* ds = xs + q.IG * ximg;
-  constexpr int NCOLT = NPT * KW * 16;
   float* red = reinterpret_cast<float*>(ds + q.IG * 16 * HoWo);
   {
     const int tot = q.IG * (ximg + 16 * HoWo);
     for (int o = tid * 8; o < tot; o += 256 * 8) *reinterpret_cast<uint4*>(xs + o) = make_uint4(0, 0, 0, 0);
   }
-  const int npairs = q.Cin * q.kh;
   int poff[NPT];
-#pragma unroll
-  for (int pt = 0; pt < NPT; pt++) {
-    int pair = pt * 16 + (lane & 15);
-    if (pair >= npairs) pair = 0;
-    const int ci = pair / q.kh, r = pair - ci * q.kh;
-    poff[pt] = (SW == 1 ? (ci * q.Hs + r) * q.Ws : (ci * q.Hs + r) * 2 * q.Ws) * 2;
-  }
+  ncv_wg_pair_rows<SW, NPT>(q, lane, poff);
   nv_f4 acc[NPT][KW];
 #pragma unroll
   for (int pt = 0; pt < NPT; pt++)
@@ -612,7 +715,6 @@
   const int64_t n0 = (int64_t)blockIdx.x * images_per_block, n1 = min<int64_t>(n0 + images_per_block, q.N);
   const int chunks_per_img = HoWo >> 5;
   const int xpk = (q.Cin * q.H * q.W) >> 3, dpk = (q.Cout * HoWo) >> 3, dpk2 = (q.Cout2 * HoWo) >> 3, per = xpk + dpk + dpk2;
-  const int rc = q.W >> 3;
   const bool pf = q.IG * per <= NCV_WPF * 256;
   uint4 pre[NCV_WPF];
   int p_src[NCV_WPF], p_dst[NCV_WPF], p_im[NCV_WPF];
@@ -622,9 +724,8 @@
     const int im = idx / per, j = idx - im * per;
     p_im[k] = (pf && im < q.IG) ? im : -1;
     if (j < xpk) {
-      const int b = j % rc, a = (j / rc) % q.H, c = j / (rc * q.H);
       p_src[k] = im * q.Cin * q.H * q.W + j * 8;
-      p_dst[k] = im * ximg + (SW == 1 ? (c * q.Hs + q.ph + a) * q.Ws + NCV_OFFA + b * 8 : ((c * q.Hs + q.ph + a) * 2) * q.Ws + NCV_OFFA + b * 4);
+      p_dst[k] = im * ximg + ncv_wg_x_dst<SW>(q, j);
     } else if (j < xpk + dpk) {
       p_src[k] = -(im * q.Cout * HoWo + (j - xpk) * 8) - 1;
       p_dst[k] = q.IG * ximg + im * 16 * HoWo + (j - xpk) * 8;
@@ -664,10 +765,6 @@
       else stage_x(xs + p_dst[k], v);
     }
   };
-  auto x_dst = [&](unsigned short* xi, int j) {
-    const int b = j % rc, a = (j / rc) % q.H, c = j / (rc * q.H);
-    return xi + (SW == 1 ? (c * q.Hs + q.ph + a) * q.Ws + NCV_OFFA + b * 8 : ((c * q.Hs + q.ph + a) * 2) * q.Ws + NCV_OFFA + b * 4);
-  };
 
   if (pf && n0 < n1) pre_load(n0, (int)min<int64_t>(q.IG, n1 - n0));
   for (int64_t nb = n0; nb < n1; nb += q.IG) {
@@ -680,7 +777,7 @@
     else for (int im = 0; im < ig; im++) {
       const bf16_t* xp = x + (nb + im) * q.Cin * q.H * q.W;
       unsigned short* xi = xs + im * ximg;
-      for (int i = tid; i < xpk; i += 256) stage_x(x_dst(xi, i), *reinterpret_cast<const uint4*>(xp + i * 8));
+      for (int i = tid; i < xpk; i += 256) stage_x(xi + ncv_wg_x_dst<SW>(q, i), *reinterpret_cast<const uint4*>(xp + i * 8));
       const bf16_t* dp = dy + (nb + im) * q.Cout * HoWo;
       unsigned short* di = ds + im * 16 * HoWo;
       for (int i = tid; i < dpk; i += 256) *reinterpret_cast<uint4*>(di + i * 8) = *reinterpret_cast<const uint4*>(dp + i * 8);
@@ -696,86 +793,64 @@
 #if defined(NCV_WSKIP) && (NCV_WSKIP & 1)
     if (nb < 0)
 #endif
-    for (int ch = wid; ch < nchunks; ch += 4) {
-      const int pg = ch * 32 + (lane >> 4) * 8;
-      const int im = pg / HoWo, pp = pg - im * HoWo;
-      const int ho = pp / q.Wo, wo0 = pp - ho * q.Wo;
-      const nv_s8 a = *reinterpret_cast<const nv_s8*>(ds + (im * 16 + (lane & 15)) * HoWo + pp);
-      const nv_bf8 af = __builtin_bit_cast(nv_bf8, a);
-      const char* xb = reinterpret_cast<const char*>(xs + im * ximg) +
-                       (SW == 1 ? (ho * q.Ws + wo0 + NCV_OFFA - 8) * 2 : ((ho * 2) * 2 * q.Ws + wo0 + NCV_OFFA - 8) * 2);
-#pragma unroll
-      for (int pt = 0; pt < NPT; pt++) {
-        const char* rowp = xb + poff[pt];
-        if (SW == 1) {
-          constexpr bool need_m = PW > 0, need_p = (KW - 1 - PW) > 0;
-          unsigned int sg[13];
-          const uint4 z = make_uint4(0, 0, 0, 0);
-          const uint4 v0 = need_m ? *reinterpret_cast<const uint4*>(rowp) : z;
-          const uint4 v1 = *reinterpret_cast<const uint4*>(rowp + 16);
-          const uint4 v2 = need_p ? *reinterpret_cast<const uint4*>(rowp + 32) : z;
-          sg[0] = v0.x; sg[1] = v0.y; sg[2] = v0.z; sg[3] = v0.w; sg[4] = v1.x; sg[5] = v1.y; sg[6] = v1.z; sg[7] = v1.w;
-          sg[8] = v2.x; sg[9] = v2.y; sg[10] = v2.z; sg[11] = v2.w; sg[12] = 0;
-#pragma unroll
-          for (int s = 0; s < KW; s++) {
-            const int o = 8 + s - PW;
-            const int dq = o >> 1;
-            typedef unsigned int u4v __attribute__((ext_vector_type(4)));
-            u4v f;
-#pragma unroll
-            for (int j = 0; j < 4; j++) f[j] = (o & 1) ? __builtin_amdgcn_alignbit(sg[dq + j + 1], sg[dq + j], 16) : sg[dq + j];
-            acc[pt][s] = __builtin_amdgcn_mfma_f32_16x16x32_bf16(af, __builtin_bit_cast(nv_bf8, f), acc[pt][s], 0, 0, 0);
-          }
-        } else {
-          unsigned int sg[2][9];
-#pragma unroll
-          for (int par = 0; par < 2; par++) {
-            const uint4 v0 = *reinterpret_cast<const uint4*>(rowp + par * q.Ws * 2);
-            const uint4 v1 = *reinterpret_cast<const uint4*>(rowp + par * q.Ws * 2 + 16);
-            sg[par][0] = v0.x; sg[par][1] = v0.y; sg[par][2] = v0.z; sg[par][3] = v0.w;
-            sg[par][4] = v1.x; sg[par][5] = v1.y; sg[par][6] = v1.z; sg[par][7] = v1.w; sg[par][8] = 0;
-          }
-#pragma unroll
-          for (int s = 0; s < KW; s++) {
-            const int t = s - PW, par = t & 1, half = (t - par) >> 1;
-            const int o = 8 + half, dq = o >> 1;
-            typedef unsigned int u4v __attribute__((ext_vector_type(4)));
-            u4v f;
-#pragma unroll
-            for (int j = 0; j < 4; j++) f[j] = (o & 1) ? __builtin_amdgcn_alignbit(sg[par][dq + j + 1], sg[par][dq + j], 16) : sg[par][dq + j];
-            acc[pt][s] = __builtin_amdgcn_mfma_f32_16x16x32_bf16(af, __builtin_bit_cast(nv_bf8, f), acc[pt][s], 0, 0, 0);
-          }
-        }
-      }
-    }
-  }
-#pragma unroll
-  for (int pt = 0; pt < NPT; pt++)
-#pragma unroll
-    for (int s = 0; s < KW; s++)
-#pragma unroll
-      for (int rr = 0; rr < 4; rr++) red[(wid * 16 + (lane >> 4) * 4 + rr) * NCOLT + (pt * KW + s) * 16 + (lane & 15)] = acc[pt][s][rr];
+    ncv_wg_chunks<KW, PW, SW, NPT>(xs, ximg, ds + (lane & 15) * HoWo, 16 * HoWo, q, poff, acc, nchunks, lane, wid);
+  }
+  ncv_wg_leave<KW, NPT>(red, acc, q, partial, partial2, tid, lane, wid);
+}
+
+constexpr int NCV_CB_PF = 2;
+template <int NK, int PH0>
+__global__ __launch_bounds__(256, 2) void ncv_chain_bwd_kernel(const bf16_t* __restrict__ da, const bf16_t* __restrict__ db, const nv_bf8* __restrict__ wpk, NcvGeom q,
+                                                               const bf16_t* __restrict__ x, NcvWGeom wq, float* __restrict__ partial, int images_per_block) {
+  constexpr int KW = 5, PW = 2;
+  extern __shared__ __attribute__((aligned(16))) char smem[];
+  const int tid = threadIdx.x, lane = tid & 63, wid = tid >> 6;
+  const int HoWo = wq.Ho * wq.Wo;
+  const int gimg = q.C * q.Hs * q.Ws, ximg = wq.Cin * wq.Hs * wq.Ws;
+  unsigned short* gs = reinterpret_cast<unsigned short*>(smem);
+  unsigned short* xs = gs + gimg;
+  unsigned short* ds = xs + ximg;
+  unsigned short* zrow = ds + wq.Cout * HoWo;
+  float* red = reinterpret_cast<float*>(smem);
+  const int n0 = blockIdx.x * images_per_block, n1 = min(n0 + images_per_block, q.N);
+  const int64_t img_a = (int64_t)q.C1 * q.H * q.W, img_b = (int64_t)(q.C - q.C1) * q.H * q.W, img_x = (int64_t)wq.Cin * wq.H * wq.W;
+  NcvPreT<NCV_CB_PF> pre, prex;
+  const NcvPlanT<NCV_CB_PF> plan = ncv_stage_plan<NCV_CB_PF>(q, tid, 256);
+  NcvPlanT<NCV_CB_PF> planx;
+#pragma unroll
+  for (int k = 0; k < NCV_CB_PF; k++) {
+    const int j = tid + k * 256;
+    planx.dst[k] = j * 8 < (int)img_x ? ncv_wg_x_dst<1>(wq, j) : -1;
+    planx.src[k] = j * 8;
+  }
+  if (n0 < n1) { ncv_stage_load(pre, plan, da + n0 * img_a, db + n0 * img_b); ncv_stage_load(prex, planx, x + n0 * img_x, x); }
+  nv_bf8 wfr[NK];
+  int koff[NK];
+  ncv_frag_setup<NK, true>(q, wpk, lane, wfr, koff);
+  int poff[1];
+  ncv_wg_pair_rows<1, 1>(wq, lane, poff);
+  for (int o = tid * 8; o < gimg + ximg + (wq.Cout + 1) * HoWo; o += 256 * 8) *reinterpret_cast<uint4*>(gs + o) = make_uint4(0, 0, 0, 0);
+  const int co = lane & 7, ncg = q.Wo / 8;
+  const int a_tr = (lane & 15) / ncg, a_cg = (lane & 15) - a_tr * ncg;
+  const int a_off = (2 * a_tr * q.sh * q.Ws + a_cg * 8 + (q.wx - PH0)) * 2;
+  unsigned short* mc = ds + co * HoWo;
+  const unsigned short* arow = (lane & 15) < wq.Cout ? ds + (lane & 15) * HoWo : zrow;
+  nv_f4 acc[1][KW];
+#pragma unroll
+  for (int s = 0; s < KW; s++) acc[0][s] = nv_f4{0.f, 0.f, 0.f, 0.f};
+  NcvStatAcc none{nv_f4{0.f, 0.f, 0.f, 0.f}, nv_f4{0.f, 0.f, 0.f, 0.f}, 0};
+  for (int n = n0; n < n1; n++) {
+    __syncthreads();
+    ncv_stage_store(gs, pre, plan, q.dil);
+    ncv_stage_store(xs, prex, planx, 1);
+    __syncthreads();
+    if (n + 1 < n1) { ncv_stage_load(pre, plan, da + (n + 1) * img_a, db + (n + 1) * img_b); ncv_stage_load(prex, planx, x + (n + 1) * img_x, x); }
+    ncv_super_tiles<NK, 1, PH0, 2, false, false, true, 2>(smem, q, wfr, koff, a_off, 0.f, co, nullptr, nullptr, none, mc, q.Wo, lane, wid, 4);
+    __syncthreads();
+    ncv_wg_chunks<KW, PW, 1, 1>(xs, ximg, arow, 0, wq, poff, acc, HoWo >> 5, lane, wid);
+  }
   __syncthreads();
-  const int O = q.Cout * q.ncol;
-  for (int i = tid; i < O; i += 256) {
-    const int co = i / q.ncol, cidx = i - co * q.ncol;
-    const int pair = cidx / KW, s = cidx - pair * KW;
-    const int col = ((pair >> 4) * KW + s) * 16 + (pair & 15);
-    float a = 0.f;
-#pragma unroll
-    for (int w = 0; w < 4; w++) a += red[(w * 16 + co) * NCOLT + col];
-    partial[(int64_t)blockIdx.x * O + i] = a;
-  }
-  const int O2 = q.Cout2 * q.Cin;
-  for (int i = tid; i < O2; i += 256) {
-    const int co2 = i / q.Cin, ci = i - co2 * q.Cin;
-    const int pair = ci * q.kh + (q.kh >> 1), s = KW >> 1;
-    const int col = ((pair >> 4) * KW + s) * 16 + (pair & 15);
-    float a = 0.f;
-#pragma unroll
-    for (int w = 0; w < 4; w++) a += red[(w * 16 + q.Cout + co2) * NCOLT + col];
-    partial2[(int64_t)blockIdx.x * O2 + i] = a;
-  }
+  ncv_wg_leave<KW, 1>(red, acc, wq, partial, nullptr, tid, lane, wid);
 }
 
 
@@ -1153,82 +1228,93 @@
   hipLaunchKernelGGL((ncv_wgrad_kernel<NT, SW>), dim3(blocks), dim3(256), lds, st, dy, x, partial, q, ipb);
 }
 
-struct NcvSecondWgrad { const Tensor* dy; Tensor* dw; };
-static bool ncv_wgrad_run(const Tensor* dy, const Tensor* x, Tensor* dw, const ConvGeom& g, hipStream_t st, const NcvSecondWgrad* second) {
-  if (!ncv_common(g, x->dtype)) return false;
+struct NcvWgrad2Plan { NcvWGeom q; const void* kfn; size_t lds; int nblocks, ipb; };
+static bool ncv_wgrad2_plan(const ConvGeom& g, const NcvWGeom& base, NcvWgrad2Plan& wp) {
+  const int SW = g.sh, HoWo = (int)(g.Ho * g.Wo);
+  const int npt = (int)((g.Cin * g.kh + 15) / 16);
+  const bool aligned = g.kh == g.kw && npt <= 3 &&
+                       ((g.kw == 5 && g.pw == 2 && SW == 1) || (g.kw == 3 && g.pw == 1) || (g.kw == 1 && g.pw == 0));
+  if (!aligned) return false;
+  NcvWGeom& q = wp.q;
+  q = base;
+  if (SW == 1) q.Ws = round_up(NCV_OFFA + std::max((int)g.W, (int)g.Wo + 8) + 8, 8);
+  else q.Ws = round_up(NCV_OFFA + std::max((int)g.W / 2, (int)g.Wo) + 8, 8);
+  const int ximg2 = q.Cin * q.Hs * q.Ws * (SW == 2 ? 2 : 1);
+  const int ncolt = npt * g.kw * 16;
+  const size_t lds2 = (size_t)q.IG * (ximg2 + 16 * HoWo) * 2 + (size_t)4 * 16 * ncolt * 4;
+  if (lds2 > 150 * 1024) return false;
+  const void* kfn = nullptr;
+#define NCV_WG2(KWv, PWv, SWv, NPTv) kfn = (const void*)ncv_wgrad2_kernel<KWv, PWv, SWv, NPTv>
+#define NCV_WG2_NPT(KWv, PWv, SWv) do { if (npt == 1) NCV_WG2(KWv, PWv, SWv, 1); else if (npt == 2) NCV_WG2(KWv, PWv, SWv, 2); else NCV_WG2(KWv, PWv, SWv, 3); } while (0)
+  if (g.kw == 5) NCV_WG2_NPT(5, 2, 1);
+  else if (g.kw == 3 && SW == 1) NCV_WG2_NPT(3, 1, 1);
+  else if (g.kw == 3) NCV_WG2_NPT(3, 1, 2);
+  else if (SW == 1) NCV_WG2_NPT(1, 0, 1);
+  else NCV_WG2_NPT(1, 0, 2);
+#undef NCV_WG2_NPT
+#undef NCV_WG2
+  allow_big_lds(kfn);
+  const int per_cu = std::min((int)std::max<size_t>(1, std::min<size_t>(4, (size_t)(150 * 1024) / lds2)), kernel_occupancy(kfn, 256, lds2));
+  const int64_t rounds = (g.N + q.IG - 1) / q.IG;
+  const int nb = (int)std::min<int64_t>(rounds, (int64_t)num_cus() * per_cu);
+  wp.ipb = (int)((rounds + nb - 1) / nb) * q.IG;
+  wp.nblocks = (int)((g.N + wp.ipb - 1) / wp.ipb);
+  wp.kfn = kfn; wp.lds = lds2;
+  return true;
+}
+static void ncv_wgrad_reduce_later(Tensor* partial, Tensor* dw, int O, int nsplit, hipStream_t st) {
+  WgradReduceArgs ra{};
+  ra.kind = 1; ra.O = O; ra.nsplit = nsplit; ra.blocks = (int)(((int64_t)O * 64 + 255) / 256);
+  wgrad_reduce_enqueue(ra, partial, dw, st);
+}
+static bool ncv_wgrad_geom(const ConvGeom& g, int dtype, int cout2, NcvWGeom& q) {
+  if (!ncv_common(g, dtype)) return false;
   if (g.W % 8 != 0 || g.Wo % 8 != 0 || (g.Ho * g.Wo) % 32 != 0) return false;
-  const int cout2 = second ? (int)second->dy->sizes[1] : 0;
-  if (second && (g.Cout + cout2 > 16 || g.kh != 3 || g.kw != 3 || g.ph != 1 || g.pw != 1)) return false;
-  NcvWGeom q;
   q.N = (int)g.N; q.Cin = (int)g.Cin; q.Cout = (int)g.Cout; q.H = (int)g.H; q.W = (int)g.W; q.Ho = (int)g.Ho; q.Wo = (int)g.Wo;
   q.kh = g.kh; q.kw = g.kw; q.ph = g.ph; q.pw = g.pw; q.Cout2 = cout2;
   q.ncol = (int)g.Cin * g.kh * g.kw;
-  const int SW = g.sh;
   q.Hs = std::max((int)g.H + 2 * g.ph, ((int)g.Ho - 1) * g.sh + g.kh);
-  if (SW == 1) q.Ws = round_up(std::max(NCV_LEFT + (int)g.W, (int)g.Wo - 1 + g.kw - 1 - g.pw + NCV_LEFT + 1), 8);
+  if (g.sh == 1) q.Ws = round_up(std::max(NCV_LEFT + (int)g.W, (int)g.Wo - 1 + g.kw - 1 - g.pw + NCV_LEFT + 1), 8);
   else {
     const int half_max = (g.kw - 1 - g.pw) >> 1;
     q.Ws = round_up(std::max((int)g.W / 2, (int)g.Wo + half_max) + NCV_OFF2 + 1, 8);
   }
+  q.IG = std::max(1, 256 / (int)(g.Ho * g.Wo));
+  return true;
+}
+struct NcvSecondWgrad { const Tensor* dy; Tensor* dw; };
+static bool ncv_wgrad_run(const Tensor* dy, const Tensor* x, Tensor* dw, const ConvGeom& g, hipStream_t st, const NcvSecondWgrad* second) {
+  const int cout2 = second ? (int)second->dy->sizes[1] : 0;
+  NcvWGeom q;
+  if (!ncv_wgrad_geom(g, x->dtype, cout2, q)) return false;
+  if (second && (g.Cout + cout2 > 16 || g.kh != 3 || g.kw != 3 || g.ph != 1 || g.pw != 1)) return false;
+  const int SW = g.sh;
   const int HoWo = (int)(g.Ho * g.Wo);
-  q.IG = std::max(1, 256 / HoWo);
-  const int npt = (int)((g.Cin * g.kh + 15) / 16);
-  const bool aligned = g.kh == g.kw && npt <= 3 &&
-                       ((g.kw == 5 && g.pw == 2 && SW == 1) || (g.kw == 3 && g.pw == 1) || (g.kw == 1 && g.pw == 0));
-  if (aligned) {
-    if (SW == 1) q.Ws = round_up(NCV_OFFA + std::max((int)g.W, (int)g.Wo + 8) + 8, 8);
-    else q.Ws = round_up(NCV_OFFA + std::max((int)g.W / 2, (int)g.Wo) + 8, 8);
-    const int ximg2 = q.Cin * q.Hs * q.Ws * (SW == 2 ? 2 : 1);
-    const int ncolt = npt * g.kw * 16;
-    const size_t lds2 = (size_t)q.IG * (ximg2 + 16 * HoWo) * 2 + (size_t)4 * 16 * ncolt * 4;
-    if (lds2 <= 150 * 1024) {
-      const int O = q.Cout * q.ncol;
-      const void* kfn = nullptr;
-#define NCV_WG2(KWv, PWv, SWv, NPTv) kfn = (const void*)ncv_wgrad2_kernel<KWv, PWv, SWv, NPTv>
-#define NCV_WG2_NPT(KWv, PWv, SWv) do { if (npt == 1) NCV_WG2(KWv, PWv, SWv, 1); else if (npt == 2) NCV_WG2(KWv, PWv, SWv, 2); else NCV_WG2(KWv, PWv, SWv, 3); } while (0)
-      if (g.kw == 5) NCV_WG2_NPT(5, 2, 1);
-      else if (g.kw == 3 && SW == 1) NCV_WG2_NPT(3, 1, 1);
-      else if (g.kw == 3) NCV_WG2_NPT(3, 1, 2);
-      else if (SW == 1) NCV_WG2_NPT(1, 0, 1);
-      else NCV_WG2_NPT(1, 0, 2);
-#undef NCV_WG2_NPT
-#undef NCV_WG2
-      allow_big_lds(kfn);
-      const int per_cu = std::min((int)std::max<size_t>(1, std::min<size_t>(4, (size_t)(150 * 1024) / lds2)), kernel_occupancy(kfn, 256, lds2));
-      const int64_t rounds = (g.N + q.IG - 1) / q.IG;
-      const int nb = (int)std::min<int64_t>(rounds, (int64_t)num_cus() * per_cu);
-      const int ipb = (int)((rounds + nb - 1) / nb) * q.IG;
-      const int nblocks = (int)((g.N + ipb - 1) / ipb);
-      int64_t ps[1] = {(int64_t)nblocks * O};
-      Hold partial(new_tensor(ps, 1, kF32, dy->device()));
-      const int O2 = cout2 * q.Cin;
-      Hold partial2;
-      if (second) { int64_t ps2[1] = {(int64_t)nblocks * O2}; partial2 = Hold(new_tensor(ps2, 1, kF32, dy->device())); }
-      {
-        const double sec_fl = second ? 2.0 * (double)g.N * cout2 * (double)g.Ho * g.Wo * (double)g.Cin : 0.0;
-        const double sec_by = second ? ((double)g.N * cout2 * g.Ho * g.Wo + (double)cout2 * g.Cin) * 2.0 : 0.0;
-        KernelTimer kt("conv_wgrad_narrow", conv_flops(g) + sec_fl, conv_bytes(g, 2) + sec_by, st);
-        const bf16_t* dp = dy->ptr<bf16_t>(); const bf16_t* xp = x->ptr<bf16_t>(); float* pp = partial->ptr<float>();
-        const bf16_t* dp2 = second ? second->dy->ptr<bf16_t>() : (const bf16_t*)nullptr;
-        float* pp2 = second ? partial2->ptr<float>() : (float*)nullptr;
-        int ipb_arg = ipb;
-        void* args[] = {(void*)&dp, (void*)&xp, (void*)&pp, (void*)&q, (void*)&ipb_arg, (void*)&dp2, (void*)&pp2};
-        HIP_CHECK(hipLaunchKernel(kfn, dim3(nblocks), dim3(256), args, lds2, st));
-        LAMP_LAUNCH_CHECK();
-      }
-      WgradReduceArgs ra{};
-      ra.kind = 1; ra.O = O; ra.nsplit = nblocks; ra.blocks = (int)(((int64_t)O * 64 + 255) / 256);
-      wgrad_reduce_enqueue(ra, partial.get(), dw, st);
-      if (second) {
-        WgradReduceArgs rb{};
-        rb.kind = 1; rb.O = O2; rb.nsplit = nblocks; rb.blocks = (int)(((int64_t)O2 * 64 + 255) / 256);
-        wgrad_reduce_enqueue(rb, partial2.get(), second->dw, st);
-      }
-      return true;
-    }
-    if (second) return false;
-    if (SW == 1) q.Ws = round_up(std::max(NCV_LEFT + (int)g.W, (int)g.Wo - 1 + g.kw - 1 - g.pw + NCV_LEFT + 1), 8);
-    else { const int half_max = (g.kw - 1 - g.pw) >> 1; q.Ws = round_up(std::max((int)g.W / 2, (int)g.Wo + half_max) + NCV_OFF2 + 1, 8); }
+  NcvWgrad2Plan wp;
+  if (ncv_wgrad2_plan(g, q, wp)) {
+    const NcvWGeom& qa = wp.q;
+    const int O = qa.Cout * qa.ncol, nblocks = wp.nblocks;
+    int64_t ps[1] = {(int64_t)nblocks * O};
+    Hold partial(new_tensor(ps, 1, kF32, dy->device()));
+    const int O2 = cout2 * qa.Cin;
+    Hold partial2;
+    if (second) { int64_t ps2[1] = {(int64_t)nblocks * O2}; partial2 = Hold(new_tensor(ps2, 1, kF32, dy->device())); }
+    {
+      const double sec_fl = second ? 2.0 * (double)g.N * cout2 * (double)g.Ho * g.Wo * (double)g.Cin : 0.0;
+      const double sec_by = second ? ((double)g.N * cout2 * g.Ho * g.Wo + (double)cout2 * g.Cin) * 2.0 : 0.0;
+      KernelTimer kt("conv_wgrad_narrow", conv_flops(g) + sec_fl, conv_bytes(g, 2) + sec_by, st);
+      const bf16_t* dp = dy->ptr<bf16_t>(); const bf16_t* xp = x->ptr<bf16_t>(); float* pp = partial->ptr<float>();
+      const bf16_t* dp2 = second ? second->dy->ptr<bf16_t>() : (const bf16_t*)nullptr;
+      float* pp2 = second ? partial2->ptr<float>() : (float*)nullptr;
+      int ipb_arg = wp.ipb;
+      NcvWGeom qarg = qa;
+      void* args[] = {(void*)&dp, (void*)&xp, (void*)&pp, (void*)&qarg, (void*)&ipb_arg, (void*)&dp2, (void*)&pp2};
+      HIP_CHECK(hipLaunchKernel(wp.kfn, dim3(nblocks), dim3(256), args, wp.lds, st));
+      LAMP_LAUNCH_CHECK();
+    }
+    ncv_wgrad_reduce_later(partial.get(), dw, O, nblocks, st);
+    if (second) ncv_wgrad_reduce_later(partial2.get(), second->dw, O2, nblocks, st);
+    return true;
   }
   if (second) return false;
   const int nt_real = (q.ncol + 15) / 16;
@@ -1283,4 +1369,51 @@
   return ncv_wgrad_run(dy, x, dw, g, st, &sw);
 }
 
-}
+bool narrow_conv_chain_bwd(const Tensor* x, const ConvGeom& g0, const Tensor* dy, const Tensor* w, const ConvGeom& g, const Tensor* dy1, const Tensor* w1,
+                           const ConvGeom& g1, Tensor* dw0, hipStream_t st) {
+  if (!sw().conv_dgrad_pair || x->dtype != kBF16 || dy->dtype != kBF16 || dy1->dtype != kBF16) return false;
+  if (g.kh != 3 || g.kw != 3 || g.ph != 1 || g.pw != 1 || g1.kh != 1 || g1.kw != 1 || g1.ph != 0 || g1.pw != 0) return false;
+  if (g.sh != g1.sh || g.sw != g1.sw || g.Ho != g1.Ho || g.Wo != g1.Wo || g.H != g1.H || g.W != g1.W || g.Cin != g1.Cin || g.N != g1.N) return false;
+  if (g.groups != 1 || g1.groups != 1 || g.dh != 1 || g.dw != 1 || g1.dh != 1 || g1.dw != 1 || g1.Cout > 16) return false;
+  if (g0.groups != 1 || g0.sh != 1 || g0.sw != 1 || g0.N != g.N || g0.Cout != g.Cin || g0.Ho != g.H || g0.Wo != g.W) return false;
+  const int cout2 = (int)g1.Cout;
+  NcvLaunchPlan lp;
+  if (!ncv_plan(g, dy->dtype, true, false, true, cout2, lp)) return false;
+  const NcvGeom& q = lp.q;
+  if (!lp.aligned || lp.threads != 256 || lp.nke == 0 || lp.NS != 2 || lp.ph0 != 7 || !(lp.NK2 == 6 || lp.NK2 == 8)) return false;
+  if (!q.pf || (int64_t)q.C * q.H * q.W > (int64_t)NCV_CB_PF * 256 * 8) return false;
+  NcvWGeom wbase;
+  NcvWgrad2Plan wp;
+  if (!ncv_wgrad_geom(g0, x->dtype, 0, wbase) || !ncv_wgrad2_plan(g0, wbase, wp)) return false;
+  const NcvWGeom& wq = wp.q;
+  if (g0.kw != 5 || g0.Cin * g0.kh > 16 || wq.IG != 1 || (int64_t)wq.Cin * wq.H * wq.W > (int64_t)NCV_CB_PF * 256 * 8) return false;
+  const int HoWo = wq.Ho * wq.Wo;
+  const size_t lds = ((size_t)q.C * q.Hs * q.Ws + (size_t)wq.Cin * wq.Hs * wq.Ws + (size_t)(wq.Cout + 1) * HoWo) * 2;
+  if (lds > 150 * 1024 || lds < (size_t)4 * 16 * 5 * 16 * 4) return false;
+  const void* kfn = lp.NK2 == 6 ? (const void*)ncv_chain_bwd_kernel<6, 7> : (const void*)ncv_chain_bwd_kernel<8, 7>;
+  if (lds > 64 * 1024) allow_big_lds(kfn);
+  const NcvW wqp = ncv_weights_of(w, g, true, lp, w1, cout2);
+  Hold wpk_h(ncv_packed_weights(w, wqp, st, w1));
+  const nv_bf8* wpk = reinterpret_cast<const nv_bf8*>(static_cast<const Tensor*>(wpk_h.get())->ptr<bf16_t>());
+  const int O = wq.Cout * wq.ncol;
+  int64_t ps[1] = {(int64_t)wp.nblocks * O};
+  Hold partial(new_tensor(ps, 1, kF32, x->device()));
+  {
+    const double fl = conv_flops(g) + 2.0 * (double)g.N * cout2 * (double)g.Ho * g.Wo * (double)g.Cin + conv_flops(g0);
+    const double by = conv_bytes(g, 2) + ((double)g.N * cout2 * g.Ho * g.Wo + (double)cout2 * g.Cin) * 2.0 + conv_bytes(g0, 2) -
+                      2.0 * (double)g.N * g.Cin * g.H * g.W * 2.0;
+    KernelTimer kt("conv_dgrad_wgrad_narrow", fl, by, st);
+    const bf16_t* dap = dy->ptr<bf16_t>(); const bf16_t* dbp = dy1->ptr<bf16_t>(); const bf16_t* xp = x->ptr<bf16_t>();
+    float* pp = partial->ptr<float>();
+    NcvGeom qarg = q;
+    NcvWGeom wqarg = wq;
+    int ipb = wp.ipb;
+    void* args[] = {(void*)&dap, (void*)&dbp, (void*)&wpk, (void*)&qarg, (void*)&xp, (void*)&wqarg, (void*)&pp, (void*)&ipb};
+    HIP_CHECK(hipLaunchKernel(kfn, dim3(wp.nblocks), dim3(256), args, lds, st));
+    LAMP_LAUNCH_CHECK();
+  }
+  ncv_wgrad_reduce_later(partial.get(), dw0, O, wp.nblocks, st);
+  return true;
+}
+
+}
```

Result: no change. 2.259 million samples/s, median of 6 (+0.9%).
